# alpapad/java-rsync

Measured on AMD Instinct MI355X. Metric: GiB/s device-resident rolling+MD5 scan (Generator block sums + Sender match scan; bytes read), higher is better.
Workload: dtype u8

## Files before the change

include/rsync_hip_debug.h:

```cpp
#ifndef RSYNC_HIP_DEBUG_H
#define RSYNC_HIP_DEBUG_H

#include <stdint.h>

#include "rsync_hip.h"

#ifdef __cplusplus
extern "C" {
#endif

int rsh_debug_set_option(const char* name, int64_t value);
int rsh_debug_get_option(const char* name, int64_t* value);
void rsh_debug_reset_options(void);

int rsh_debug_kernel_ms(rsh_ctx* ctx, int32_t which, double* ms);

int rsh_debug_generation(rsh_ctx* ctx, int32_t set, int32_t* gen);

int rsh_debug_streams_busy(rsh_ctx* ctx, int32_t* mask);

int rsh_debug_k1_clock(rsh_ctx* ctx, const void* d_data, int64_t n, int32_t block_length, int32_t reps,
                       double* clock_ghz);

int rsh_debug_multi_selftest(const int64_t* bytes, int32_t njobs, int32_t nparts, int32_t fail_part, int32_t* part_out,
                             int32_t* order_out, int32_t* status_out);

int rsh_debug_tokens_selftest(const uint8_t* src, int64_t n, const rsh_event* ev, int64_t n_ev,
                              const uint8_t file_md5[16], int64_t from, uint8_t* out, int64_t len, int64_t span,
                              int64_t* n_desc);

int rsh_debug_sums_selftest(int32_t unframe, const rsh_header* h, int32_t* weak, uint8_t* strong, uint8_t* wire,
                            int64_t len, int64_t span, int64_t* n_desc);

typedef struct {
    int64_t pos;
    int32_t kind;
    int32_t value;
    int64_t count;
} rsh_token_run;
int rsh_debug_tokens_scan_selftest(rsh_ctx* ctx, const uint8_t* tokens, int64_t tokens_len, int64_t from,
                                   rsh_token_run* runs, int64_t cap, int64_t* n_runs, int64_t* pos, int32_t* status);

int rsh_debug_untokens_selftest(rsh_ctx* ctx, const uint8_t* tokens, int64_t tokens_len, int64_t pos, int32_t T,
                                int64_t count, uint8_t* out, int64_t span, int64_t* n_desc, int64_t* lo, int64_t* hi);

#ifdef __cplusplus
}
#endif
#endif
```

java-rsync_amd/csrc/batch.cpp:

```cpp
#include "batch.h"

namespace rsh {

void destroy_batch_state(BatchState* b) { delete b; }
hipError_t clear_batch_abort_words(BatchState* b) {
    if (!b) return hipSuccess;
    hipError_t e = b->file_abort ? hipMemset(b->file_abort, 0, (size_t)b->file_abort_cap * 4) : hipSuccess;
    if (e == hipSuccess && b->chain_map.p) e = hipMemset(b->chain_map.p, 0, b->chain_map.cap);
    return e;
}

namespace batch {
namespace {

#define RSH_HTRY(call) do { const hipError_t e_ = (call); if (e_ != hipSuccess) return e_; } while (0)
#define RSH_STEP(call) do { const int rc_ = (call); if (rc_ != RSH_OK) return rc_; } while (0)

struct K1Set {
    std::vector<K1Plan> plans;
    std::vector<K1Lane> lanes;
    int lane_align = 16;
    bool partial = tail_gather_on();
    uint32_t ngroups = 0;
    void plan(const std::vector<K1File>& kf) {
        ngroups = plan_block_sums_files(kf.data(), (int32_t)kf.size(), &plans, &lanes, &lane_align, &partial);
    }
};

hipError_t stage_k1(K1Staging& k, std::initializer_list<const K1Set*> sets, hipStream_t st) {
    if (!k.ev) RSH_HTRY(hipEventCreateWithFlags(&k.ev, hipEventDisableTiming));
    if (k.pending) RSH_HTRY(hipEventSynchronize(k.ev));
    k.pending = false;
    size_t np = 0, nl = 0, ng = 0;
    for (const K1Set* s : sets) np += s->plans.size(), nl += s->lanes.size(), ng += s->ngroups;
    RSH_HTRY(k.ensure(np, ng, nl));
    K1Plan* hp = k.h_plans.as<K1Plan>();
    K1Lane* hl = k.h_lanes.as<K1Lane>();
    for (const K1Set* s : sets) {
        hp = std::copy(s->plans.begin(), s->plans.end(), hp);
        hl = std::copy(s->lanes.begin(), s->lanes.end(), hl);
    }
    if (np > 0) RSH_HTRY(hipMemcpyAsync(k.plans.p, k.h_plans.p, np * sizeof(K1Plan), hipMemcpyHostToDevice, st));
    size_t p0 = 0, g0 = 0;
    for (const K1Set* s : sets) {
        RSH_HTRY(launch_expand_groups(k.plans.as<K1Plan>() + p0, (uint32_t)s->plans.size(), s->ngroups,
                                      k.groups.as<K1Group>() + g0, st));
        p0 += s->plans.size(), g0 += s->ngroups;
    }
    if (nl > 0) RSH_HTRY(hipMemcpyAsync(k.lanes.p, k.h_lanes.p, nl * sizeof(K1Lane), hipMemcpyHostToDevice, st));
    RSH_HTRY(hipEventRecord(k.ev, st));
    k.pending = true;
    return hipSuccess;
}

struct SegmentLayout {
    int32_t NF = 0;
    int64_t tw = 0, ts = 0, tna = 0, tas = 0, tnf = 0, tns = 0, thit = 0, tw0 = 0, maxC = 0;
    bool chain_on = false;
    bool two_phase = false;
    bool map_on = false;
    int32_t chain_events = 0;
    K1Set whole, a, b;
    std::vector<int64_t> lead_at;
    int64_t nlead_all = 0;
    size_t lead_ents_at = 0;
    std::vector<int64_t> map_off;
    int64_t map_end(const FileLayout& fs) const { return std::min<int64_t>(fs.na_a * fs.B, fs.n - fs.B + 1); }
    hipError_t plan(BatchState* S, const std::vector<FileLayout*>& file, hipStream_t st);
};

hipError_t SegmentLayout::plan(BatchState* S, const std::vector<FileLayout*>& file, hipStream_t st) {
    NF = (int32_t)file.size();
    for (FileLayout* p : file) {
        FileLayout& fs = *p;
        fs.na = (fs.n + fs.B - 1) / fs.B;
        fs.nf = std::min<int64_t>(fs.na, fs.C);
        fs.ns = pow2_at_least(2 * (uint64_t)fs.C + 2);
        fs.off_tw = tw, tw += fs.C;
        fs.off_ts = ts, ts += (int64_t)fs.C * fs.dl;
        fs.off_na = tna, tna += fs.na;
        fs.off_as = tas, tas += fs.na * fs.dl;
        fs.off_nf = tnf, tnf += fs.nf;
        fs.off_ns = tns, tns += fs.ns;
        fs.off_hit = thit, thit += pad16(16 + fs.B);
        fs.off_w0 = tw0, tw0 += pad16(std::min<int64_t>(fs.B, fs.n));
        maxC = std::max<int64_t>(maxC, fs.C);
    }
    const size_t nf = (size_t)NF;
    RSH_HTRY(S->h_weak.ensure((size_t)tw * 4 + 4));
    RSH_HTRY(S->h_strong.ensure((size_t)ts + 1));
    RSH_HTRY(S->slots.ensure((size_t)tns * 8));
    RSH_HTRY(S->src_weak.ensure((size_t)tna * 4));
    RSH_HTRY(S->src_strong.ensure((size_t)tas + 1));
    RSH_HTRY(S->flags.ensure((size_t)tnf + 1));
    RSH_HTRY(S->haw.ensure((size_t)tna * 4));
    RSH_HTRY(S->h_aw.ensure((size_t)tna * 4));
    RSH_HTRY(S->h_as.ensure((size_t)tas + 1));
    RSH_HTRY(S->h_fl.ensure((size_t)tnf + 1));
    RSH_HTRY(S->h_files.ensure(nf * sizeof(ScanFile)));
    RSH_HTRY(S->h_hit.ensure((size_t)thit));
    RSH_HTRY(S->h_win0.ensure((size_t)tw0));
    RSH_HTRY(S->first.ensure(nf * sizeof(ProbeOut)));
    RSH_HTRY(S->h_first.ensure(nf * sizeof(ProbeOut)));
    RSH_HTRY(S->bucket.ensure(nf * HIT_BUCKET_INTS * 4));
    RSH_HTRY(S->h_bucket.ensure(nf * HIT_BUCKET_INTS * 4));
    RSH_HTRY(S->h_copies.ensure(2 * nf * sizeof(CopyEnt)));
    RSH_HTRY(S->h_ccopies.ensure(nf * sizeof(CopyEnt) + 3 * nf * sizeof(CopyEnt)));
    RSH_HTRY(S->h_tabents.ensure(nf * sizeof(TableEnt)));
    RSH_HTRY(S->h_flagents.ensure(nf * sizeof(FlagEnt)));
    RSH_HTRY(S->h_flagents_a.ensure(nf * sizeof(FlagEnt)));
    lead_at.assign(nf + 1, 0);
    for (size_t f = 0; f < nf; ++f) lead_at[f + 1] = lead_at[f] + std::min<int64_t>(kLeadWindows, file[f]->nf);
    nlead_all = lead_at[nf];
    lead_ents_at = ((size_t)(nlead_all + 1) * 4 + 63) & ~(size_t)63;
    RSH_HTRY(S->h_lead.ensure(lead_ents_at + (size_t)(nlead_all + 1) * sizeof(GatherEnt)));
    auto k1_file = [&](const FileLayout& fs, int64_t w0, int64_t w1) {
        return K1File{fs.d_src + w0 * fs.B, std::min<int64_t>(fs.n, w1 * fs.B) - w0 * fs.B, (uint32_t)fs.B, (uint32_t)fs.dl,
                      (uint32_t)(w1 - w0), S->src_weak.as<int32_t>() + fs.off_na + w0,
                      S->src_strong.as<uint8_t>() + fs.off_as + w0 * fs.dl};
    };
    std::vector<K1File> k1;
    for (const FileLayout* fs : file) k1.push_back(k1_file(*fs, 0, fs->na));
    whole.plan(k1);
    RSH_HTRY(S->ensure_file_abort(NF));
    for (K1Plan& pl : whole.plans) pl.abort = S->file_abort + pl.file;
    chain_on = opt(OPT_BATCH_CHAIN) != 0;
    chain_events = (int32_t)std::clamp<int64_t>(
        kChainEventBytes / ((int64_t)std::max<int32_t>(NF, 1) * (int64_t)sizeof(rsh_event)), 256, kChainEventsMax);
    for (FileLayout* fs : file) fs->na_a = fs->na;
    if (const int64_t pre = opt(OPT_BATCH_CHAIN_PREFIX); chain_on && pre != 0) {
        const int64_t P = pre > 0 ? pre : 16 * std::max<int64_t>(1, kWaveSlots / std::max<int32_t>(NF, 1));
        for (FileLayout* fs : file) {
            fs->na_a = std::min(fs->na, P);
            two_phase = two_phase || fs->na_a < fs->na;
        }
    }
    if (two_phase) {
        std::vector<K1File> ka, kb;
        std::vector<int32_t> b_file;
        for (int32_t f = 0; f < NF; ++f) {
            const FileLayout& fs = *file[(size_t)f];
            ka.push_back(k1_file(fs, 0, fs.na_a));
            if (fs.na_a == fs.na) continue;
            kb.push_back(k1_file(fs, fs.na_a, fs.na));
            b_file.push_back(f);
        }
        a.plan(ka);
        b.plan(kb);
        for (K1Plan& pl : a.plans) pl.abort = nullptr;
        for (K1Plan& pl : b.plans) pl.abort = S->file_abort + b_file[(size_t)pl.file];
        for (const K1Lane& ln : b.lanes) {
            const int64_t lo = (int64_t)ln.c_first * ln.B, hi = std::min<int64_t>(ln.n, lo + (int64_t)ln.nchunks * ln.B);
            file[(size_t)b_file[(size_t)ln.file]]->lane_b_bytes += std::max<int64_t>(0, hi - lo);
        }
    }
    RSH_HTRY(S->spec_k1.ensure(std::max(whole.plans.size(), a.plans.size() + b.plans.size()),
                               std::max(whole.ngroups, a.ngroups + b.ngroups),
                               std::max(whole.lanes.size(), a.lanes.size() + b.lanes.size())));
    if (!chain_on) return hipSuccess;
    RSH_HTRY(S->kslots.ensure(kslots_bytes(tns, tw)));
    RSH_HTRY(S->h_kents.ensure(nf * sizeof(ChunkIndexEnt)));
    RSH_HTRY(S->h_chain.ensure(nf * sizeof(ChainFile)));
    RSH_HTRY(S->h_chain_out.ensure(nf * sizeof(ChainOut)));
    RSH_HTRY(S->h_chain_ev.ensure(nf * (size_t)chain_events * sizeof(rsh_event)));
    RSH_HTRY(S->h_early.ensure(4096));
    map_off.assign(nf + 1, 0);
    map_on = two_phase && opt(OPT_CHAIN_HELPERS) != 0;
    for (size_t f = 0; map_on && f < nf; ++f) {
        const FileLayout& fs = *file[f];
        const bool wide = fs.B >= 512 && fs.B % 32 == 0 && CHAIN_TILE / fs.B + 2 <= CHAIN_SEGS;
        const int64_t hend = map_end(fs);
        map_off[f + 1] = map_off[f] + (wide && fs.C > 0 && hend > 0 ? (hend + 31) / 32 : 0);
    }
    map_on = map_on && map_off[nf] > 0 && map_off[nf] * 8 <= opt(OPT_CHAIN_MAP_BYTES);
    if (map_on) {
        if ((size_t)map_off[nf] * 8 > S->chain_map.cap) {
            RSH_HTRY(S->chain_map.ensure((size_t)map_off[nf] * 8));
            RSH_HTRY(hipMemsetAsync(S->chain_map.p, 0, S->chain_map.cap, st));
        }
        RSH_HTRY(S->chain_help.ensure(nf * sizeof(ChainHelp)));
        RSH_HTRY(S->h_chain_help.ensure(nf * sizeof(ChainHelp)));
    }
    return hipSuccess;
}

TableEnt table_ent(const DevBuf& slots, const FileScan& fs) {
    return TableEnt{slots.as<unsigned long long>() + fs.off_ns, fs.d_weak, fs.ns - 1, fs.C};
}
FlagEnt flag_ent(BatchState* S, const FileScan& fs, uint32_t nflag) {
    return FlagEnt{S->src_weak.as<int32_t>() + fs.off_na, S->src_strong.as<uint8_t>() + fs.off_as, fs.d_weak, fs.d_strong,
                   S->flags.as<uint8_t>() + fs.off_nf, nflag, (uint32_t)fs.dl};
}
CopyEnt* table_copies(BatchState* S, const FileScan& fs, CopyEnt* out) {
    if (fs.C == 0) return out;
    *out++ = CopyEnt{reinterpret_cast<const uint8_t*>(fs.d_weak), S->h_weak.as<uint8_t>() + 4 * fs.off_tw, (int64_t)fs.C * 4};
    if (fs.dl > 0) *out++ = CopyEnt{fs.d_strong, S->h_strong.as<uint8_t>() + fs.off_ts, (int64_t)fs.C * fs.dl};
    return out;
}
CopyEnt* spec_copies(BatchState* S, const FileScan& fs, int64_t nal, bool flags, bool sums, CopyEnt* out) {
    const int64_t nfl = std::min(fs.nf, nal);
    if (flags && nfl > 0) *out++ = CopyEnt{S->flags.as<uint8_t>() + fs.off_nf, S->h_fl.as<uint8_t>() + fs.off_nf, nfl};
    if (!sums) return out;
    *out++ = CopyEnt{S->src_weak.as<uint8_t>() + 4 * fs.off_na, S->h_aw.as<uint8_t>() + 4 * fs.off_na, nal * 4};
    if (fs.dl > 0)
        *out++ = CopyEnt{S->src_strong.as<uint8_t>() + fs.off_as, S->h_as.as<uint8_t>() + fs.off_as, nal * fs.dl};
    return out;
}

struct Scan {
    rsh_ctx* const c;
    BatchState* const S;
    rsh_scan_job* const jobs;
    const uint8_t* const seed;
    const std::chrono::steady_clock::time_point t0 = std::chrono::steady_clock::now();
    const bool trace = opt(OPT_SCAN_TRACE) != 0;
    const hipStream_t st, aux;
    std::vector<FileScan> files;
    SegmentLayout L;
    std::shared_ptr<Batch> bp = std::make_shared<Batch>();
    Batch& b = *bp;
    RoundCtl ctl;
    int gen = 0;
    bool tentative = false;
    bool k1_launched = false, spec_launched = false;
    bool skip_rest = false;
    std::vector<char> early;
    hipError_t early_err = hipSuccess;
    uint32_t n_help = 0;
    int spec_rc = RSH_OK;
    int32_t nwait = 0, left = 0;
    int rounds = 0;
    double enq_ms = 0, setup_ms = 0, resolve_ms = 0;

    Scan(rsh_ctx* c_, BatchState* S_, rsh_scan_job* jobs_, const uint8_t* seed_)
        : c(c_), S(S_), jobs(jobs_), seed(seed_), st(c_->stream), aux(c_->aux) {}
    int32_t NF() const { return L.NF; }
    ChainOut* chain_out() const { return S->h_chain_out.as<ChainOut>(); }
    rsh_event* chain_ev(int32_t f) const { return S->h_chain_ev.as<rsh_event>() + (int64_t)f * L.chain_events; }

    int lay_out(const std::vector<int32_t>& which);
    void prepare_files();
    int enqueue_prep();
    int begin_speculation();
    int launch_spec_k1();
    int launch_spec();
    int enqueue_walks();
    void prepare_walks();
    int walk_phase0();
    int walk_rest();
    hipError_t await_walks();
    hipError_t early_resolve(int32_t f);
    void take_walk(int32_t f, bool prefix_only);
    int await_setup();
    int take_walks();
    int hand_over();
    void report_walks();
    int lead_check();
    hipError_t run_rounds();
    int cancel_unlanded();
    void return_events();
    void add_stats(rsh_scan_stats* agg);
};

int Scan::lay_out(const std::vector<int32_t>& which) {
    files.resize(which.size());
    std::vector<FileLayout*> lay;
    for (size_t f = 0; f < which.size(); ++f) {
        FileScan& fs = files[f];
        const rsh_scan_job& j = jobs[which[f]];
        fs.job = which[f];
        fs.d_src = static_cast<const uint8_t*>(j.d_src);
        fs.d_weak = static_cast<const int32_t*>(j.d_weak);
        fs.d_strong = static_cast<const uint8_t*>(j.d_strong);
        fs.n = j.n;
        fs.B = j.h.block_length;
        fs.C = j.h.chunk_count;
        fs.dl = j.h.digest_length;
        lay.push_back(&fs);
    }
    RSH_BHIP(L.plan(S, lay, st));
    early.assign(files.size(), 0);
    return RSH_OK;
}

void Scan::prepare_files() {
    ScanFile* F = S->h_files.as<ScanFile>();
    b.files = &files;
    for (int32_t f = 0; f < NF(); ++f) {
        FileScan& fs = files[(size_t)f];
        const rsh_scan_job& j = jobs[fs.job];
        fs.table.chunk_count = fs.C;
        fs.table.block_length = (int32_t)fs.B;
        fs.table.remainder = j.h.remainder;
        fs.table.digest_length = fs.dl;
        fs.table.weak = S->h_weak.as<int32_t>() + fs.off_tw;
        fs.table.strong = S->h_strong.as<uint8_t>() + fs.off_ts;
        BatchBackend& be = fs.be;
        be.b = &b;
        be.f = f;
        be.na = fs.na;
        be.aw = S->h_aw.as<int32_t>() + fs.off_na;
        be.as = S->h_as.as<uint8_t>() + fs.off_as;
        be.fl = S->h_fl.as<uint8_t>() + fs.off_nf;
        be.win0 = S->h_win0.as<uint8_t>() + fs.off_w0;
        be.w0 = std::min<int64_t>(fs.B, fs.n);
        be.hit = S->h_hit.as<uint8_t>() + fs.off_hit;
        be.bucket = S->h_bucket.as<int32_t>() + (int64_t)f * HIT_BUCKET_INTS;
        be.n = fs.n;
        be.B = fs.B;
        memcpy(be.seed, seed, 4);
        be.table = &fs.table;
        be.haw_ready.assign((size_t)fs.na, 0);
        F[f] = ScanFile{};
        F[f].data = fs.d_src;
        F[f].n = fs.n;
        F[f].B = (uint32_t)fs.B;
        F[f].out = S->first.as<ProbeOut>() + f;
        F[f].table_weak = fs.d_weak;
        F[f].C = fs.C;
        F[f].bucket = S->bucket.as<int32_t>() + (int64_t)f * HIT_BUCKET_INTS;
        F[f].hit = S->h_hit.as<uint8_t>() + fs.off_hit;
        F[f].nwin = 1;
        F[f].aligned_weak = S->haw.as<int32_t>() + fs.off_na;
    }
}

int Scan::enqueue_prep() {
    ScanFile* F = S->h_files.as<ScanFile>();
    RSH_BHIP(hipEventRecord(c->ev_in, st));
    CopyEnt* wc = S->h_ccopies.as<CopyEnt>();
    int64_t max_w0 = 0;
    for (int32_t f = 0; f < NF(); ++f) {
        FileScan& fs = files[(size_t)f];
        const int64_t w0 = std::min<int64_t>(fs.B, fs.n);
        wc[f] = CopyEnt{fs.d_src, S->h_win0.as<uint8_t>() + fs.off_w0, w0};
        max_w0 = std::max(max_w0, w0);
    }
    RSH_BHIP(launch_copy_many(wc, (uint32_t)NF(), max_w0, st));
    if (L.nlead_all > 0 && !L.chain_on) {
        auto* ents = reinterpret_cast<GatherEnt*>(S->h_lead.as<uint8_t>() + L.lead_ents_at);
        for (int32_t f = 0; f < NF(); ++f)
            for (int64_t k = 0; k < L.lead_at[(size_t)f + 1] - L.lead_at[(size_t)f]; ++k)
                ents[L.lead_at[(size_t)f] + k] = GatherEnt{k * files[(size_t)f].B, f, 0};
        RSH_BHIP(launch_window_weak(F, ents, (uint32_t)L.nlead_all, S->h_lead.as<int32_t>(), st));
    }
    RSH_BHIP(hipEventRecord(c->ev_prep, st));
    constexpr bool bg = true;
    if (!L.chain_on) {
        CopyEnt* tc = S->h_copies.as<CopyEnt>();
        CopyEnt* tc_end = tc;
        for (const FileScan& fs : files) tc_end = table_copies(S, fs, tc_end);
        RSH_BHIP(launch_copy_many(tc, (uint32_t)(tc_end - tc), L.maxC * 4, st, bg));
    }
    RSH_BHIP(hipEventRecord(c->ev_tab, st));
    if (!L.chain_on) {
        TableEnt* te = S->h_tabents.as<TableEnt>();
        RSH_BHIP(launch_table_clear(S->slots.as<unsigned long long>(), (uint64_t)L.tns, st, bg));
        for (int32_t f = 0; f < NF(); ++f) te[f] = table_ent(S->slots, files[(size_t)f]);
        RSH_BHIP(launch_table_insert_many(te, (uint32_t)NF(), (int32_t)L.maxC, st, bg));
        return RSH_OK;
    }
    if (!S->ev_fk) RSH_BHIP(hipEventCreateWithFlags(&S->ev_fk, hipEventDisableTiming));
    RSH_BHIP(hipMemsetAsync(S->kslots.p, 0, (size_t)L.tns * 8 + (size_t)L.tw, st));
    ChunkIndexEnt* ke = S->h_kents.as<ChunkIndexEnt>();
    for (int32_t f = 0; f < NF(); ++f) {
        const FileScan& fs = files[(size_t)f];
        ke[f] = ChunkIndexEnt{table_ent(S->kslots, fs), kslots_dup(S, L.tns) + fs.off_tw};
    }
    RSH_BHIP(launch_chunk_index(ke, (uint32_t)NF(), (int32_t)L.maxC, st, bg));
    return RSH_OK;
}

int Scan::begin_speculation() {
    gen = c->next_gen();
    tentative = L.nlead_all > 0 && !L.chain_on;
    return tentative ? launch_spec_k1() : RSH_OK;
}

int Scan::launch_spec_k1() {
    k1_launched = true;
    K1Set& k = L.whole;
    size_t kept = 0;
    k.ngroups = 0;
    for (const K1Plan& pl : k.plans)
        if (!files[(size_t)pl.file].done) {
            k.plans[kept] = pl;
            k.plans[kept++].g0 = k.ngroups;
            k.ngroups += pl.ng;
        }
    k.plans.resize(kept);
    kept = 0;
    for (const K1Lane& ln : k.lanes)
        if (!files[(size_t)ln.file].done) k.lanes[kept++] = ln;
    k.lanes.resize(kept);
    int32_t dropped = 0;
    for (FileScan& fs : files)
        if (fs.done) fs.cancelled = true, ++dropped;
    if (trace)
        fprintf(stderr, "[rsh-batch] speculation launched: %u groups, %d resolved files dropped\n", k.ngroups, dropped);
    RSH_BHIP(stage_k1(S->spec_k1, {&k}, aux));
    RSH_BHIP(hipStreamWaitEvent(aux, L.chain_on ? c->ev_in : c->ev_prep, 0));
    RSH_BHIP(launch_block_sums_batch(S->spec_k1.groups.as<K1Group>(), k.ngroups, S->spec_k1.lanes.as<K1Lane>(),
                                     (uint32_t)k.lanes.size(), k.lane_align, seed_word(seed), aux, c->abort_word, gen,
                                     k.partial));
    return RSH_OK;
}

int Scan::launch_spec() {
    if (!k1_launched) RSH_STEP(launch_spec_k1());
    RSH_BHIP(hipStreamWaitEvent(aux, c->ev_in, 0));
    FlagEnt* fe = S->h_flagents.as<FlagEnt>();
    CopyEnt* const fc = S->h_ccopies.as<CopyEnt>() + NF();
    CopyEnt *fc_end = fc, *const sc = fc + NF(), *sc_end = sc;
    uint32_t max_nf = 0;
    int64_t max_len = 0, max_fl = 0;
    for (int32_t f = 0; f < NF(); ++f) {
        const FileScan& fs = files[(size_t)f];
        const uint32_t nflag = fs.cancelled ? 0u : (uint32_t)fs.nf;
        fe[f] = flag_ent(S, fs, nflag);
        max_nf = std::max<uint32_t>(max_nf, nflag);
        if (fs.cancelled) continue;
        fc_end = spec_copies(S, fs, fs.na, true, false, fc_end);
        sc_end = spec_copies(S, fs, fs.na, false, true, sc_end);
        max_fl = std::max<int64_t>(max_fl, fs.nf);
        max_len = std::max<int64_t>(max_len, fs.na * 4);
    }
    RSH_BHIP(launch_chain_flags_many(fe, (uint32_t)NF(), max_nf, aux));
    if (L.chain_on) RSH_BHIP(hipEventRecord(S->ev_fk, aux));
    if (!L.chain_on) RSH_BHIP(launch_copy_many(fc, (uint32_t)(fc_end - fc), max_fl, aux));
    RSH_BHIP(hipEventRecord(c->ev_flags, aux));
    if (!L.chain_on) RSH_BHIP(launch_copy_many(sc, (uint32_t)(sc_end - sc), max_len, aux));
    RSH_BHIP(hipEventRecord(c->ev_spec, aux));
    return RSH_OK;
}

void Scan::take_walk(int32_t f, bool prefix_only) {
    FileScan& fs = files[(size_t)f];
    const ChainOut& o = chain_out()[f];
    if (o.status == CHAIN_DONE) {
        fs.dev_ev = chain_ev(f);
        fs.dev_n = o.n_ev;
    } else {
        fs.res.ev.assign(chain_ev(f), chain_ev(f) + o.n_ev);
    }
    fs.res.literal = o.literal;
    fs.res.matched = o.matched;
    fs.res.stats.chain_matches += o.chain_matches;
    fs.res.stats.events += o.events;
    fs.res.stats.flushes += o.flushes;
    fs.rs.s = o.s;
    fs.rs.m = o.m;
    fs.rs.pref = o.pref;
    fs.rs.anchor = o.s;
    fs.rs.elo = o.elo;
    fs.rs.ehi = o.ehi;
    fs.rs.clear_from = o.clear_to >= 0 ? o.s : -1;
    fs.rs.clear_to = o.clear_to;
    fs.be.na = (o.aborted || prefix_only) ? fs.na_a : fs.na;
    if (o.md5c_valid) {
        fs.rs.md5c.assign(o.md5c, o.md5c + fs.dl);
        fs.rs.md5c_valid = true;
        fs.rs.dkeys_ready = false;
    }
    if (o.status == CHAIN_DONE) fs.rs.done = fs.done = true;
}

hipError_t Scan::early_resolve(int32_t f) {
    FileScan& fs = files[(size_t)f];
    take_walk(f, true);
    if (fs.done) return hipSuccess;
    const auto te0 = std::chrono::steady_clock::now();
    hipStream_t es = c->phase;
    CopyEnt* ec = S->h_early.as<CopyEnt>();
    TableEnt* et = reinterpret_cast<TableEnt*>(ec + 8);
    const int64_t nal = fs.na_a;
    CopyEnt* ec_end = spec_copies(S, fs, nal, true, true, table_copies(S, fs, ec));
    et[0] = table_ent(S->slots, fs);
    RSH_HTRY(hipStreamWaitEvent(es, S->ev_fa, 0));
    RSH_HTRY(launch_copy_many(ec, (uint32_t)(ec_end - ec), std::max<int64_t>((int64_t)fs.C * 4, nal * 4), es));
    RSH_HTRY(launch_table_clear(S->slots.as<unsigned long long>() + fs.off_ns, fs.ns, es));
    RSH_HTRY(launch_table_insert_many(et, 1, fs.C, es));
    RSH_HTRY(spin_sync(S, es));
    fs.be.head = false;
    b.landed.store(true);
    b.aligned.store(true);
    b.direct = [this, f, es](FileScan&) {
        const hipError_t x = serve_round(c, S, files, std::vector<int32_t>{f}, es);
        if (x != hipSuccess && early_err == hipSuccess) early_err = x;
    };
    resolve_run(fs.n, fs.table, fs.be, &fs.rs, &fs.res, nullptr);
    b.direct = nullptr;
    fs.rs.done = fs.done = true;
    early[(size_t)f] = 1;
    if (trace)
        fprintf(stderr, "[rsh-batch] file %d resolved while the walks ran: %.3f ms, done at %.3f ms\n", f, ms_since(te0),
                ms_since(t0));
    return early_err;
}

hipError_t Scan::await_walks() {
    const ChainOut* co = chain_out();
    std::vector<char> seen((size_t)NF(), 0);
    for (;;) {
        const hipError_t q = hipEventQuery(S->ev_wa);
        if (q != hipErrorNotReady) return q;
        for (int32_t f = 0; f < NF(); ++f) {
            if (seen[(size_t)f] || *reinterpret_cast<const volatile int32_t*>(&co[f].fin) == 0) continue;
            seen[(size_t)f] = 1;
            std::atomic_thread_fence(std::memory_order_acquire);
            if (co[f].status == CHAIN_STOP && co[f].why == CHAIN_WHY_FLUSHED) RSH_HTRY(early_resolve(f));
        }
        _mm_pause();
    }
}

void Scan::prepare_walks() {
    ChainFile* cf = S->h_chain.as<ChainFile>();
    ChainOut* co = chain_out();
    ChainHelp* chh = L.map_on ? S->h_chain_help.as<ChainHelp>() : nullptr;
    for (int32_t f = 0; f < NF(); ++f) {
        const FileScan& fs = files[(size_t)f];
        co[f] = ChainOut{};
        co[f].clear_to = -1;
        const int64_t mw = L.map_on ? L.map_off[(size_t)f + 1] - L.map_off[(size_t)f] : 0;
        const int64_t hend = mw > 0 ? L.map_end(fs) : 0;
        cf[f] = ChainFile{fs.d_src, fs.n, (uint32_t)fs.B, fs.C, fs.dl, jobs[fs.job].h.remainder,
                          fs.ns - 1, S->kslots.as<unsigned long long>() + fs.off_ns, fs.d_weak, fs.d_strong,
                          S->src_weak.as<int32_t>() + fs.off_na, S->src_strong.as<uint8_t>() + fs.off_as,
                          S->flags.as<uint8_t>() + fs.off_nf, fs.na, fs.na_a,
                          L.two_phase ? S->file_abort + f : nullptr, chain_ev(f), L.chain_events,
                          seed_word(seed), co + f,
                          mw > 0 ? S->chain_map.as<unsigned long long>() + L.map_off[(size_t)f] : nullptr, hend,
                          kslots_dup(S, L.tns) + fs.off_tw};
        if (chh) chh[f] = ChainHelp{(int32_t)((hend + CHAIN_MAP_SEG - 1) / CHAIN_MAP_SEG), 0, 1, 0, 0, 0, 0, 0, INT64_MAX, 0, 0, 0,
                                    kChainHelpTiles};
    }
    const int64_t helpers_opt = opt(OPT_CHAIN_HELPERS);
    n_help = !L.map_on ? 0u
             : helpers_opt > 0 ? (uint32_t)helpers_opt
                               : (uint32_t)std::max<int64_t>(0, (int64_t)c->n_cu - NF());
}

int Scan::enqueue_walks() {
    if (!L.chain_on) return RSH_OK;
    prepare_walks();
    if (trace) {
        for (hipEvent_t* e : {&S->ev_ch0, &S->ev_ch1})
            if (!*e) RSH_BHIP(hipEventCreate(e));
    }
    if (L.two_phase) RSH_STEP(walk_phase0());
    RSH_STEP(walk_rest());
    if (trace) RSH_BHIP(hipEventRecord(S->ev_ch1, st));
    return RSH_OK;
}

int Scan::walk_phase0() {
    const ChainFile* cf = S->h_chain.as<ChainFile>();
    const K1Staging& k = S->spec_k1;
    if (!S->ev_fa) RSH_BHIP(hipEventCreateWithFlags(&S->ev_fa, hipEventDisableTiming));
    if (!S->ev_wa) RSH_BHIP(hipEventCreate(&S->ev_wa));
    RSH_BHIP(stage_k1(S->spec_k1, {&L.a, &L.b}, aux));
    RSH_BHIP(hipStreamWaitEvent(aux, c->ev_in, 0));
    RSH_BHIP(launch_block_sums_batch(k.groups.as<K1Group>(), L.a.ngroups, k.lanes.as<K1Lane>(), (uint32_t)L.a.lanes.size(),
                                     L.a.lane_align, seed_word(seed), aux, c->abort_word, gen, L.a.partial));
    RSH_BHIP(hipStreamWaitEvent(aux, c->ev_in, 0));
    FlagEnt* fa = S->h_flagents_a.as<FlagEnt>();
    uint32_t max_na = 0;
    for (int32_t f = 0; f < NF(); ++f) {
        const FileScan& fs = files[(size_t)f];
        const uint32_t nflag = (uint32_t)std::min(fs.na_a, fs.nf);
        fa[f] = flag_ent(S, fs, nflag);
        max_na = std::max(max_na, nflag);
    }
    RSH_BHIP(launch_chain_flags_many(fa, (uint32_t)NF(), max_na, aux));
    RSH_BHIP(hipEventRecord(S->ev_fa, aux));
    if (L.map_on)
        RSH_BHIP(hipMemcpyAsync(S->chain_help.p, S->h_chain_help.p, (size_t)NF() * sizeof(ChainHelp), hipMemcpyHostToDevice, st));
    RSH_BHIP(hipStreamWaitEvent(st, S->ev_fa, 0));
    const int gen_b = c->next_gen();
    if (trace) RSH_BHIP(hipEventRecord(S->ev_ch0, st));
    RSH_BHIP(launch_chain_advance(cf, (uint32_t)NF(), st, 0, gen_b, L.map_on ? S->chain_help.as<ChainHelp>() : nullptr,
                                  n_help, trace));
    RSH_BHIP(hipEventRecord(S->ev_wa, st));
    RSH_BHIP(await_walks());
    const ChainOut* co = chain_out();
    skip_rest = true;
    for (int32_t f = 0; f < NF() && skip_rest; ++f)
        skip_rest = co[f].status == CHAIN_DONE || co[f].aborted || (co[f].status == CHAIN_STOP && co[f].md5c_valid);
    if (!skip_rest) {
        RSH_BHIP(hipStreamWaitEvent(aux, S->ev_wa, 0));
        RSH_BHIP(launch_block_sums_batch(k.groups.as<K1Group>() + L.a.ngroups, L.b.ngroups,
                                         k.lanes.as<K1Lane>() + L.a.lanes.size(), (uint32_t)L.b.lanes.size(), L.b.lane_align,
                                         seed_word(seed), aux, c->abort_word, gen_b, L.b.partial));
        k1_launched = true;
    }
    if (trace)
        fprintf(stderr, "[rsh-batch] two-phase speculation: prefix %u groups, rest %u groups%s\n", L.a.ngroups, L.b.ngroups,
                skip_rest ? " (skipped: no walk reached the prefix's end)" : "");
    return RSH_OK;
}

int Scan::walk_rest() {
    if (!skip_rest) {
        RSH_STEP(launch_spec());
        spec_launched = true;
        RSH_BHIP(hipStreamWaitEvent(st, S->ev_fk, 0));
        if (trace && !L.two_phase) RSH_BHIP(hipEventRecord(S->ev_ch0, st));
        RSH_BHIP(launch_chain_advance(S->h_chain.as<ChainFile>(), (uint32_t)NF(), st, L.two_phase ? 1 : 0, 0, nullptr, 0, trace));
    } else {
        RSH_BHIP(hipEventRecord(c->ev_flags, st));
        RSH_BHIP(hipEventRecord(c->ev_spec, st));
        RSH_BHIP(hipEventRecord(S->ev_fk, st));
        spec_launched = true;
    }
    return RSH_OK;
}

int Scan::await_setup() {
    enq_ms = ms_since(t0);
    RSH_BHIP(hipEventSynchronize(c->ev_tab));
    RSH_BHIP(spin_sync(S, st));
    setup_ms = ms_since(t0);
    return RSH_OK;
}

int Scan::take_walks() {
    if (!L.chain_on) return RSH_OK;
    for (int32_t f = 0; f < NF(); ++f) {
        if (early[(size_t)f]) continue;
        take_walk(f, skip_rest);
        if (!files[(size_t)f].done) ++left;
    }
    b.landed.store(true);
    if (left > 0) RSH_STEP(hand_over());
    if (trace) report_walks();
    return RSH_OK;
}

int Scan::hand_over() {
    CopyEnt* tc = S->h_copies.as<CopyEnt>();
    CopyEnt* tc_end = tc;
    TableEnt* te = S->h_tabents.as<TableEnt>();
    uint32_t ntl = 0;
    int64_t mt = 0;
    for (const FileScan& fs : files) {
        if (fs.done || fs.C == 0) continue;
        tc_end = table_copies(S, fs, tc_end);
        mt = std::max<int64_t>(mt, (int64_t)fs.C * 4);
        te[ntl++] = table_ent(S->slots, fs);
    }
    RSH_BHIP(launch_copy_many(tc, (uint32_t)(tc_end - tc), mt, st));
    RSH_BHIP(launch_table_clear(S->slots.as<unsigned long long>(), (uint64_t)L.tns, st));
    RSH_BHIP(launch_table_insert_many(te, ntl, (int32_t)L.maxC, st));
    CopyEnt* lc = S->h_ccopies.as<CopyEnt>() + NF();
    CopyEnt* lc_end = lc;
    int64_t mx = 0;
    for (const FileScan& fs : files) {
        if (fs.done) continue;
        lc_end = spec_copies(S, fs, fs.be.na, true, true, lc_end);
        mx = std::max(mx, fs.be.na * 4);
    }
    RSH_BHIP(hipStreamWaitEvent(st, c->ev_spec, 0));
    RSH_BHIP(launch_copy_many(lc, (uint32_t)(lc_end - lc), mx, st));
    RSH_BHIP(spin_sync(S, st));
    b.aligned.store(true);
    for (FileScan& fs : files) fs.be.head = false;
    return RSH_OK;
}

void Scan::report_walks() {
    const ChainOut* co = chain_out();
    float kms = 0.f, wams = 0.f;
    if (S->ev_ch0 && S->ev_ch1) (void)hipEventElapsedTime(&kms, S->ev_ch0, S->ev_ch1);
    if (L.two_phase && S->ev_ch0 && S->ev_wa) (void)hipEventElapsedTime(&wams, S->ev_ch0, S->ev_wa);
    int64_t tsum = 0, esum = 0, dsum = 0, psum = 0, asum = 0, msum = 0;
    int32_t tmax = 0, emax = 0, fmax = 0;
    for (int32_t f = 0; f < NF(); ++f) {
        tsum += co[f].tiles;
        msum += co[f].mapped;
        if (co[f].tiles > tmax) tmax = co[f].tiles, fmax = f;
        esum += co[f].events;
        dsum += co[f].digests;
        psum += co[f].md5c_valid;
        asum += co[f].aborted;
        emax = std::max<int32_t>(emax, (int32_t)co[f].events);
    }
    fprintf(stderr, "[rsh-batch] chain walks done at %.3f ms (walks %.3f ms, phase 0 %.3f ms; tiles %lld (%lld from the hit "
            "map), max %d per file; events %lld, max %d; %lld windows digested, %lld files poisoned, %lld speculations "
            "stopped at the prefix): %d of %d files left to the resolvers\n", ms_since(t0), kms, wams, (long long)tsum,
            (long long)msum, tmax, (long long)esum, emax,
            (long long)dsum, (long long)psum, (long long)asum, left, NF());
    const ChainOut& x = co[fmax];
    for (int32_t f = 0; f < NF(); ++f)
        if (co[f].status != CHAIN_DONE)
            fprintf(stderr, "[rsh-batch]   file %d: left at s %lld (why %d, events %lld, tiles %d, poisoned %d, searched to "
                    "%lld, phase 1 %d, walk %.1f us)\n", f, (long long)co[f].s, co[f].why, (long long)co[f].events,
                    co[f].tiles, co[f].md5c_valid, (long long)co[f].clear_to, co[f].spec_full, co[f].t_total / 100.0);
    fprintf(stderr, "[rsh-batch]   file %d: walk %.1f us = tiles %.1f (table checks %.1f; %d of %d tiles from the hit map,"
            " the first at tile %d) + events %.1f (buckets %.1f; %d digests: %.1f) + key set %.1f + steps (1)/(1') %.1f +"
            " event drains %.1f + other\n", fmax, x.t_total / 100.0,
            x.t_tiles / 100.0, x.t_check / 100.0, x.mapped, x.tiles, x.first_mapped, x.t_event / 100.0,
            x.t_evb / 100.0, x.digests, x.t_digest / 100.0, x.t_kset / 100.0, x.t_chain / 100.0, x.t_drain / 100.0);
    if (!S->chain_help.p || !L.two_phase) return;
    std::vector<ChainHelp> hh((size_t)NF());
    if (hipMemcpy(hh.data(), S->chain_help.p, (size_t)NF() * sizeof(ChainHelp), hipMemcpyDeviceToHost) != hipSuccess) return;
    int64_t segs = 0, joins = 0, files_helped = 0;
    for (const ChainHelp& q : hh) {
        segs += q.mapped;
        joins += q.joins;
        files_helped += q.joins > 0;
    }
    const ChainHelp& q = hh[(size_t)fmax];
    fprintf(stderr, "[rsh-batch]   hit map: %lld segments mapped over %lld files (%lld key sets built); file %d: %d "
            "segments (%d whole), %d key sets (%.1f us each), claims %d of %d, first whole segment %.1f us after "
            "the walk's start\n", (long long)segs, (long long)files_helped, (long long)joins, fmax, q.mapped,
            q.whole, q.joins, q.joins ? q.t_kset / 100.0 / q.joins : 0.0, q.claim, q.nseg,
            q.t_first == INT64_MAX ? -1.0 : (q.t_first - q.t_start) / 100.0);
}

int Scan::lead_check() {
    if (!tentative) return RSH_OK;
    const int32_t* lead_w = S->h_lead.as<int32_t>();
    for (int32_t f = 0; f < NF(); ++f) {
        FileScan& fs = files[(size_t)f];
        const int64_t a = L.lead_at[(size_t)f], nl = L.lead_at[(size_t)f + 1] - a;
        int64_t lead = 0;
        while (lead < nl && lead_w[a + lead] == fs.table.weak[lead]) ++lead;
        fs.wait_spec = nl > 0 && lead == nl && (nl >= kLeadWindows || nl == fs.nf);
        nwait += fs.wait_spec;
    }
    if (nwait > 0) {
        spec_rc = launch_spec();
        if (spec_rc != RSH_OK) return spec_rc;
        spec_launched = true;
    } else {
        RSH_BHIP(hipMemsetD32Async(reinterpret_cast<hipDeviceptr_t>(S->file_abort), gen, (size_t)NF(), st));
        RSH_BHIP(hipStreamWaitEvent(st, S->spec_k1.ev, 0));
        gen = c->next_gen();
        k1_launched = false;
    }
    if (trace) fprintf(stderr, "[rsh-batch] lead check: %d of %d files wait for the speculation\n", nwait, NF());
    return RSH_OK;
}

hipError_t Scan::run_rounds() {
    ctl.launch_spec = [this] { return launch_spec(); };
    ctl.spec_launched = &spec_launched;
    ctl.spec_rc = &spec_rc;
    ctl.k1_launched = k1_launched;
    ctl.gen = gen;
    ctl.trace = trace;
    ctl.t0 = t0;
    const hipError_t err = run_resolvers(c, S, bp, files, st, ctl, &rounds);
    const double rounds_end_ms = ms_since(t0);
    resolve_ms = ms_since(t0) - setup_ms;
    if (trace) {
        HostTimes tt;
        for (const HostTimes& x : b.times) {
            tt.bucket_ms += x.bucket_ms;
            tt.sort_ms += x.sort_ms;
            tt.dkeys_ms += x.dkeys_ms;
            tt.md5_ms += x.md5_ms;
        }
        fprintf(stderr, "[rsh-batch] host totals (cumulative per thread): bucket %.3f sort %.3f dkeys %.3f md5 %.3f ms\n",
                tt.bucket_ms, tt.sort_ms, tt.dkeys_ms, tt.md5_ms);
        fprintf(stderr, "[rsh-batch] %d files: enqueued %.3f, tables+hashes ready %.3f, rounds done %.3f, joined %.3f ms\n",
                NF(), enq_ms, setup_ms, rounds_end_ms, ms_since(t0));
    }
    return err;
}

int Scan::cancel_unlanded() {
    if (!spec_launched) return RSH_OK;
    if (!b.landed.load() && hipEventQuery(c->ev_flags) == hipSuccess) b.landed.store(true);
    if (b.landed.load()) return RSH_OK;
    for (int32_t f = 0; f < NF(); ++f) {
        FileScan& fs = files[(size_t)f];
        if (fs.cancelled) continue;
        fs.cancelled = true;
        RSH_BHIP(hipStreamWriteValue32(st, S->file_abort + f, (uint32_t)gen, 0));
    }
    if (trace) fprintf(stderr, "[rsh-batch] scan done before the speculation landed: stopped\n");
    RSH_BHIP(hipStreamWriteValue32(st, c->abort_word, (uint32_t)gen, 0));
    RSH_BHIP(hipStreamWaitEvent(st, c->ev_spec, 0));
    return RSH_OK;
}

void Scan::return_events() {
    std::vector<int32_t> copy_files;
    int64_t copy_bytes = 0;
    for (int32_t f = 0; f < NF(); ++f) {
        FileScan& fs = files[(size_t)f];
        rsh_scan_job& j = jobs[fs.job];
        j.literal = fs.res.literal;
        j.matched = fs.res.matched;
        j.n_ev = fs.dev_ev ? fs.dev_n : (int64_t)fs.res.ev.size();
        if (j.n_ev > j.ev_cap || (!j.ev && j.n_ev > 0)) {
            j.status = RSH_E_NOSPACE;
        } else {
            if (j.n_ev > 0) {
                copy_files.push_back(f);
                copy_bytes += j.n_ev * (int64_t)sizeof(rsh_event);
            }
            j.status = RSH_OK;
        }
    }
    auto copy_range = [&](size_t i0, size_t i1) {
        for (size_t i = i0; i < i1; ++i) {
            FileScan& fs = files[(size_t)copy_files[i]];
            rsh_scan_job& j = jobs[fs.job];
            memcpy(j.ev, fs.dev_ev ? fs.dev_ev : fs.res.ev.data(), (size_t)j.n_ev * sizeof(rsh_event));
        }
    };
    const int nct = copy_bytes > (1 << 20) ? std::min<int>(8, std::max(1, call_cores())) : 1;
    if (nct > 1 && copy_files.size() > 1) {
        const size_t per = (copy_files.size() + (size_t)nct - 1) / (size_t)nct;
        const int parts = (int)((copy_files.size() + per - 1) / per);
        S->pool.ensure(parts - 1);
        const std::function<void(int)> part = [&](int k) {
            copy_range((size_t)k * per, std::min(copy_files.size(), (size_t)(k + 1) * per));
        };
        S->pool.run(parts, part);
    } else {
        copy_range(0, copy_files.size());
    }
}

void Scan::add_stats(rsh_scan_stats* agg) {
    for (const FileScan& fs : files) {
        const rsh_scan_stats& s = fs.res.stats;
        agg->chain_matches += s.chain_matches;
        agg->events += s.events;
        agg->host_md5_windows += s.host_md5_windows;
        agg->flushes += s.flushes;
        agg->table_ms += s.table_ms + fs.table.sort_ms;
        int64_t spec_bytes = (spec_launched && b.landed.load() && !fs.cancelled) ? fs.n : 0;
        if (spec_bytes > 0 && fs.be.na < fs.na)
            spec_bytes = std::min<int64_t>(fs.n, fs.be.na * fs.B) + (skip_rest ? 0 : fs.lane_b_bytes);
        agg->device_bytes += fs.be.bytes_read + spec_bytes;
        agg->phase_matches += s.phase_matches;
    }
    agg->probe_launches += rounds;
    agg->device_ms += setup_ms;
    agg->resolver_ms += resolve_ms;
    agg->speculation_aborted = spec_launched ? (b.landed.load() ? 0 : 1) : 2;
}

int scan_batch(rsh_ctx* c, rsh_scan_job* jobs, const std::vector<int32_t>& which, const uint8_t seed[4],
               rsh_scan_stats* agg) {
    BatchState* S = state_of(c);
    if (!S) return RSH_E_NOMEM;
    Scan s(c, S, jobs, seed);
    RSH_STEP(s.lay_out(which));
    s.prepare_files();
    RSH_STEP(s.enqueue_prep());
    RSH_STEP(s.begin_speculation());
    RSH_STEP(s.enqueue_walks());
    RSH_STEP(s.await_setup());
    RSH_STEP(s.take_walks());
    RSH_STEP(s.lead_check());
    const hipError_t err = s.run_rounds();
    RSH_STEP(s.cancel_unlanded());
    if (s.spec_rc != RSH_OK) return s.spec_rc;
    if (err != hipSuccess) return RSH_E_DEVICE;
    s.return_events();
    if (agg) s.add_stats(agg);
    return RSH_OK;
}

}
}
}

using namespace rsh;

namespace rsh {
using namespace batch;

hipError_t batch_warm(rsh_ctx* c, int32_t nfiles, int64_t n, int64_t B, int32_t dl) {
    if (nfiles <= 0) return hipSuccess;
    BatchState* S = state_of(c);
    if (!S) return hipErrorOutOfMemory;
    FileLayout shape;
    shape.d_src = reinterpret_cast<const uint8_t*>(uintptr_t{4096});
    shape.n = n, shape.B = B, shape.C = (int32_t)((n + B - 1) / B), shape.dl = dl;
    std::vector<FileLayout> shapes((size_t)std::min<int32_t>(nfiles, kMaxLive), shape);
    std::vector<FileLayout*> lay;
    for (FileLayout& sh : shapes) lay.push_back(&sh);
    SegmentLayout L;
    RSH_HTRY(L.plan(S, lay, c->stream));
    hipError_t e = hipSuccess;
    auto ok = [&](hipError_t x) {
        if (e == hipSuccess) e = x;
    };
    S->pool.ensure(7);
    for (PinnedBuf* pb : {&S->h_fjobs, &S->h_fout, &S->h_rcp, &S->h_req, &S->h_gw, &S->h_gb, &S->h_ow, &S->h_ob, &S->h_win,
                          &S->h_dkeys})
        ok(pb->ensure(64 << 10));
    for (PinnedBuf* pb : {&S->h_fgw, &S->h_iv, &S->h_tiles, &S->h_segs, &S->h_ptiles}) ok(pb->ensure(512 << 10));
    for (DevBuf* db : {&S->fc_dev, &S->partials, &S->dslots, &S->d_probe}) ok(db->ensure(64 << 10));
    for (hipEvent_t* ev : {&S->ev_fk, &S->ev_fa, &S->spec_k1.ev, &S->ev_sync, &S->gen_k1.ev})
        if (!*ev) ok(hipEventCreateWithFlags(ev, hipEventDisableTiming));
    if (!S->ev_wa) ok(hipEventCreate(&S->ev_wa));
    ok(S->gen_k1.ensure(L.whole.plans.size(), L.whole.ngroups, L.whole.lanes.size()));
    return e;
}

int block_sums_batch_claimed(rsh_ctx* ctx, const rsh_block_job* jobs, int32_t njobs, const uint8_t seed[4]) {
    if (!ctx || !seed || njobs < 0 || (njobs > 0 && !jobs)) return RSH_E_INVAL;
    std::vector<K1File> files;
    for (int32_t i = 0; i < njobs; ++i) {
        const rsh_block_job& j = jobs[i];
        const int rc = check_generator_header(j.n, &j.h);
        if (rc != RSH_OK) return rc;
        if (j.h.chunk_count == 0) continue;
        if (!j.d_data || !j.d_weak || (!j.d_strong && j.h.digest_length > 0)) return RSH_E_INVAL;
        files.push_back(K1File{static_cast<const uint8_t*>(j.d_data), j.n, (uint32_t)j.h.block_length,
                               (uint32_t)j.h.digest_length, (uint32_t)j.h.chunk_count, static_cast<int32_t*>(j.d_weak),
                               static_cast<uint8_t*>(j.d_strong)});
    }
    if (files.empty()) return RSH_OK;
    BatchState* S = state_of(ctx);
    if (!S) return RSH_E_NOMEM;
    RSH_BHIP(hipSetDevice(ctx->device));
    K1Set k;
    k.plan(files);
    RSH_BHIP(stage_k1(S->gen_k1, {&k}, ctx->stream));
    RSH_BHIP(launch_block_sums_batch(S->gen_k1.groups.as<K1Group>(), k.ngroups, S->gen_k1.lanes.as<K1Lane>(),
                                     (uint32_t)k.lanes.size(), k.lane_align, seed_word(seed), ctx->stream, nullptr, 0,
                                     k.partial));
    return RSH_OK;
}

int match_scan_batch_claimed(rsh_ctx* ctx, rsh_scan_job* jobs, int32_t njobs, const uint8_t seed[4],
                             rsh_scan_stats* stats) {
    if (!ctx || !seed || njobs < 0 || (njobs > 0 && !jobs)) return RSH_E_INVAL;
    if (stats) *stats = rsh_scan_stats{};
    std::vector<int32_t> scan;
    for (int32_t i = 0; i < njobs; ++i) {
        rsh_scan_job& j = jobs[i];
        j.n_ev = j.literal = j.matched = 0;
        j.status = RSH_OK;
        if (j.n < 0) {
            j.status = RSH_E_INVAL;
            continue;
        }
        const int v = rsh_header_validate(&j.h);
        if (v != RSH_OK) {
            j.status = v;
            continue;
        }
        if (j.h.block_length == 0 || j.n == 0) {
            ResolveResult r;
            if (j.h.block_length == 0) skip_events(j.n, &r);
            j.literal = r.literal;
            j.n_ev = (int64_t)r.ev.size();
            if (j.n_ev > j.ev_cap || (!j.ev && j.n_ev > 0)) j.status = RSH_E_NOSPACE;
            else if (j.n_ev > 0) memcpy(j.ev, r.ev.data(), r.ev.size() * sizeof(rsh_event));
            continue;
        }
        if (!j.d_src || (j.h.chunk_count > 0 && (!j.d_weak || (!j.d_strong && j.h.digest_length > 0)))) {
            j.status = RSH_E_INVAL;
            continue;
        }
        if ((j.n + j.h.block_length - 1) / j.h.block_length > 2147483647LL) {
            j.status = RSH_E_OVERFLOW;
            continue;
        }
        scan.push_back(i);
    }
    if (!scan.empty()) {
        auto fail_from = [&](size_t k, int rc) {
            for (size_t q = k; q < scan.size(); ++q) jobs[scan[q]].status = rc;
            return rc;
        };
        if (hipSetDevice(ctx->device) != hipSuccess) return fail_from(0, RSH_E_DEVICE);
        for (size_t k = 0; k < scan.size(); k += kMaxLive) {
            const std::vector<int32_t> part(scan.begin() + (ptrdiff_t)k,
                                            scan.begin() + (ptrdiff_t)std::min(scan.size(), k + kMaxLive));
            const int rc = scan_batch(ctx, jobs, part, seed, stats);
            if (rc != RSH_OK) return fail_from(k, rc);
        }
    }
    for (int32_t i = 0; i < njobs; ++i)
        if (jobs[i].status != RSH_OK) return jobs[i].status;
    return RSH_OK;
}

}

extern "C" {

int rsh_block_sums_batch_device(rsh_ctx* ctx, const rsh_block_job* jobs, int32_t njobs, const uint8_t seed[4]) {
    if (!ctx) return RSH_E_INVAL;
    RSH_CLAIM(ctx);
    return rsh::block_sums_batch_claimed(ctx, jobs, njobs, seed);
}

int rsh_match_scan_batch_device(rsh_ctx* ctx, rsh_scan_job* jobs, int32_t njobs, const uint8_t seed[4],
                                rsh_scan_stats* stats) {
    if (!ctx) return RSH_E_INVAL;
    RSH_CLAIM(ctx);
    return rsh::match_scan_batch_claimed(ctx, jobs, njobs, seed, stats);
}

}
```

java-rsync_amd/csrc/batch.h:

```cpp
#pragma once
#include <sched.h>
#include <ucontext.h>

#include <condition_variable>
#include <functional>
#include <memory>
#include <mutex>
#include <thread>

#include <immintrin.h>

#include "ctx.h"
#include "host_md5.h"
#include "options.h"
#include "resolver.h"

namespace rsh {

struct HostPool {
    std::mutex mu;
    std::condition_variable cv_work, cv_done;
    std::vector<std::thread> th;
    const std::function<void(int)>* job = nullptr;
    int njobs = 0, next = 0, done = 0;
    uint64_t gen = 0;
    bool quit = false;
    void ensure(int n) {
        while ((int)th.size() < n) th.emplace_back([this] { work(); });
    }
    void work() {
        uint64_t seen = 0;
        std::unique_lock<std::mutex> l(mu);
        for (;;) {
            cv_work.wait(l, [&] { return quit || gen != seen; });
            if (quit) return;
            seen = gen;
            while (next < njobs) {
                const int i = next++;
                l.unlock();
                (*job)(i);
                l.lock();
                if (++done == njobs) cv_done.notify_one();
            }
        }
    }
    void run(int n, const std::function<void(int)>& f) {
        if (n <= 0) return;
        std::unique_lock<std::mutex> l(mu);
        job = &f;
        njobs = n, next = 0, done = 0;
        ++gen;
        cv_work.notify_all();
        while (next < njobs) {
            const int i = next++;
            l.unlock();
            f(i);
            l.lock();
            ++done;
        }
        cv_done.wait(l, [&] { return done == njobs; });
        job = nullptr;
    }
    ~HostPool() {
        {
            std::lock_guard<std::mutex> l(mu);
            quit = true;
        }
        cv_work.notify_all();
        for (std::thread& t : th) t.join();
    }
};

struct K1Staging {
    DevBuf plans, groups, lanes;
    PinnedBuf h_plans, h_lanes;
    hipEvent_t ev = nullptr;
    bool pending = false;
    hipError_t ensure(size_t nplans, size_t ngroups, size_t nlanes) {
        hipError_t e = hipSuccess;
        if (pending && ((nplans + 1) * sizeof(K1Plan) > h_plans.cap || (nlanes + 1) * sizeof(K1Lane) > h_lanes.cap)) {
            e = hipEventSynchronize(ev);
            pending = false;
        }
        if (e == hipSuccess) e = groups.ensure((ngroups + 1) * sizeof(K1Group));
        if (e == hipSuccess) e = plans.ensure((nplans + 1) * sizeof(K1Plan));
        if (e == hipSuccess) e = lanes.ensure((nlanes + 1) * sizeof(K1Lane));
        if (e == hipSuccess) e = h_plans.ensure((nplans + 1) * sizeof(K1Plan));
        if (e == hipSuccess) e = h_lanes.ensure((nlanes + 1) * sizeof(K1Lane));
        return e;
    }
    ~K1Staging() {
        if (ev) {
            if (pending) (void)hipEventSynchronize(ev);
            (void)hipEventDestroy(ev);
        }
        for (DevBuf* b : {&plans, &groups, &lanes}) b->release();
        for (PinnedBuf* b : {&h_plans, &h_lanes}) b->release();
    }
};

struct BatchState {
    HostPool pool;
    K1Staging gen_k1, spec_k1;
    DevBuf slots, dslots, src_weak, src_strong, flags, haw, partials, bucket, first;
    DevBuf d_probe;
    DevBuf fc_dev;
    PinnedBuf h_fgw, h_fjobs, h_fout;
    PinnedBuf h_early;
    PinnedBuf h_rcp;
    PinnedBuf h_weak, h_strong, h_aw, h_as, h_fl, h_files, h_hit, h_win0, h_bucket, h_first, h_iv, h_tiles, h_segs,
        h_ptiles, h_req, h_gw, h_gb, h_ow, h_ob, h_win, h_copies, h_tabents, h_flagents, h_flagents_a, h_dkeys, h_ccopies,
        h_lead;
    int* file_abort = nullptr;
    int64_t file_abort_cap = 0;
    DevBuf kslots;
    PinnedBuf h_kents, h_chain, h_chain_out, h_chain_ev;
    DevBuf chain_help, chain_map;
    PinnedBuf h_chain_help;
    std::vector<std::unique_ptr<char[]>> fiber_stacks;
    hipEvent_t ev_fk = nullptr;
    hipEvent_t ev_sync = nullptr;
    hipEvent_t ev_ch0 = nullptr, ev_ch1 = nullptr;
    hipEvent_t ev_fa = nullptr, ev_wa = nullptr;
    hipError_t ensure_file_abort(int64_t nf) {
        if (nf <= file_abort_cap) return hipSuccess;
        if (file_abort) (void)hipFree(file_abort);
        file_abort = nullptr;
        file_abort_cap = 0;
        const int64_t cap = std::max<int64_t>(nf, 256);
        hipError_t e = hipExtMallocWithFlags(reinterpret_cast<void**>(&file_abort), (size_t)cap * 4,
                                             hipDeviceMallocUncached);
        if (e == hipSuccess) e = hipMemset(file_abort, 0, (size_t)cap * 4);
        if (e == hipSuccess) file_abort_cap = cap;
        return e;
    }
    ~BatchState() {
        if (file_abort) (void)hipFree(file_abort);
        for (hipEvent_t e : {ev_fk, ev_ch0, ev_ch1, ev_fa, ev_wa, ev_sync})
            if (e) (void)hipEventDestroy(e);
        kslots.release();
        for (PinnedBuf* b : {&h_kents, &h_chain, &h_chain_out, &h_chain_ev, &h_chain_help}) b->release();
        chain_help.release();
        chain_map.release();
        for (DevBuf* b : {&d_probe, &fc_dev, &slots, &dslots, &src_weak, &src_strong, &flags, &haw, &partials, &bucket, &first})
            b->release();
        for (PinnedBuf* b : {&h_weak, &h_strong, &h_aw, &h_as, &h_fl, &h_files, &h_hit, &h_win0, &h_bucket, &h_first,
                             &h_iv, &h_tiles, &h_segs, &h_ptiles, &h_req, &h_gw, &h_gb, &h_ow, &h_ob, &h_win, &h_copies,
                             &h_tabents, &h_flagents, &h_flagents_a, &h_dkeys, &h_ccopies, &h_lead, &h_fgw, &h_fjobs,
                             &h_fout, &h_early, &h_rcp})
            b->release();
    }
};
inline size_t kslots_bytes(int64_t tns, int64_t tw) { return (size_t)tns * 8 + (size_t)tw + 8; }
inline uint8_t* kslots_dup(BatchState* S, int64_t tns) {
    return reinterpret_cast<uint8_t*>(S->kslots.as<unsigned long long>() + tns);
}

namespace batch {

constexpr int32_t kMaxLive = 256;
constexpr int kDeferRounds = 2;
constexpr int32_t kChainHelpTiles = 1;
constexpr int kSpinUs = 200;
constexpr int32_t kMaxWorkers = 32;
constexpr size_t kFiberStack = 512 * 1024;
constexpr int32_t kEagerSortChunks = 1 << 16;
constexpr int64_t kPad = 16;
constexpr int64_t kWaveSlots = 2 * 4 * 256;
constexpr size_t kProbeUpload = 2048;
constexpr int32_t kChainEventsMax = 4096;
constexpr int64_t kChainEventBytes = 64ll << 20;

inline int64_t pad16(int64_t v) { return (v + kPad - 1) / kPad * kPad; }

inline BatchState* state_of(rsh_ctx* c) {
    if (!c->batch) c->batch = new (std::nothrow) BatchState();
    return c->batch;
}

template <class T>
hipError_t pin(PinnedBuf& b, int64_t count, T** out) {
    const hipError_t e = b.ensure((size_t)std::max<int64_t>(count, 1) * sizeof(T));
    *out = b.as<T>();
    return e;
}

#define RSH_BHIP(call)                                  \
    do {                                                \
        hipError_t e_ = (call);                         \
        if (e_ != hipSuccess) {                         \
            note_error(e_, __LINE__, __FILE__);         \
            return RSH_E_DEVICE;                        \
        }                                               \
    } while (0)

struct Req {
    enum Kind { WEAK, BYTES, WIN, PROBE, WAIT, FLUSH, FCHAIN } kind = WEAK;
    const int64_t* pos = nullptr;
    int64_t count = 0;
    const int64_t* pos2 = nullptr;
    int64_t count2 = 0;
    uint8_t* out_b2 = nullptr;
    int32_t* out_w = nullptr;
    uint8_t* out_b = nullptr;
    int64_t p = 0, w = 0;
    const uint8_t* win = nullptr;
    const ProbeInterval* iv = nullptr;
    int64_t niv = 0;
    const std::vector<int32_t>* keys = nullptr;
    bool head = false;
    int64_t result = -1;
    const ProbeOut* out = nullptr;
    FlushChain fchain;
    int64_t npre = 0;
    uint32_t* chain_out = nullptr;
};

struct Batch;

class BatchBackend : public ScanBackend {
  public:
    Batch* b = nullptr;
    int32_t f = 0;
    bool head = true;
    int64_t na = 0;
    const int32_t* aw = nullptr;
    const uint8_t* as = nullptr;
    const uint8_t* fl = nullptr;
    const uint8_t* win0 = nullptr;
    int64_t w0 = 0;
    const uint8_t* hit = nullptr;
    const int32_t* bucket = nullptr;
    int64_t n = 0, B = 0;
    uint8_t seed[4];
    ChunkTable* table = nullptr;
    std::vector<uint8_t> haw_ready;
    int64_t win_pos[HIT_WINDOWS] = {-1, -1, -1, -1};
    int64_t t_pos = -1;
    int32_t t_val = 0;
    HitCache cache;

    int64_t aligned_count() override;
    int64_t flags_count() override { return head ? 0 : na; }
    int64_t max_batch() override { return head ? 4 : 4096; }
    const int32_t* aligned_weak() override { return aw; }
    const uint8_t* aligned_strong() override { return as; }
    const uint8_t* chain_flags() override { return fl; }
    void weak_many(const int64_t* pos, int64_t count, int32_t* out) override;
    void bytes_many(const int64_t* pos, int64_t count, uint8_t* out) override;
    void flush_gather(const int64_t* tpos, int64_t nt, int32_t* tv, const int64_t* bpos, int64_t nb,
                      uint8_t* bv) override;
    void md5_at(int64_t p, uint8_t out[16]) override;
    int64_t first_hit(const ProbeInterval* iv, int64_t count, const std::vector<int32_t>* keys) override;
    int64_t flush_probe(const ProbeInterval* pre, int64_t npre, const FlushChain& q, std::vector<FlushStep>* steps,
                        std::vector<ProbeInterval>* ivs, const std::vector<int32_t>* keys) override;
  private:
    int64_t probe_answer(const ProbeInterval* iv, int64_t count, const std::vector<int32_t>* keys);
};

struct FileLayout {
    const uint8_t* d_src = nullptr;
    int64_t n = 0, B = 0, na = 0, nf = 0;
    int64_t na_a = 0;
    int64_t lane_b_bytes = 0;
    int32_t C = 0, dl = 0;
    uint32_t ns = 0;
    int64_t off_tw = 0, off_ts = 0, off_na = 0, off_as = 0, off_nf = 0, off_ns = 0, off_hit = 0, off_w0 = 0;
};

struct FileScan : FileLayout {
    int32_t job = 0;
    const int32_t* d_weak = nullptr;
    const uint8_t* d_strong = nullptr;
    const rsh_event* dev_ev = nullptr;
    int64_t dev_n = 0;
    ChunkTable table;
    ResolveState rs;
    ResolveResult res;
    BatchBackend be;
    Req req;
    bool pending = false;
    bool done = false;
    bool started = false;
    bool cancelled = false;
    bool wait_spec = false;
    int32_t worker = 0;
    ucontext_t uc;
    char* stack = nullptr;
};

struct Batch {
    std::mutex mu;
    std::condition_variable cv_coord, cv_work;
    std::atomic<int32_t> idle{0};
    std::atomic<int32_t> nworkers{0};
    std::atomic<uint64_t> gen{0};
    std::atomic<bool> quit{false};
    std::atomic<bool> landed{false};
    std::atomic<bool> aligned{false};
    std::vector<FileScan>* files = nullptr;
    std::vector<ucontext_t> worker_uc;
    std::vector<double> busy_ms, max_fiber_ms;
    std::vector<HostTimes> times;

    std::function<void(FileScan&)> direct;
    void post(FileScan& fs) {
        if (direct) {
            direct(fs);
            return;
        }
        fs.pending = true;
        swapcontext(&fs.uc, &worker_uc[(size_t)fs.worker]);
    }
};
// ... 40 lines not shown
```

java-rsync_amd/csrc/capi.cpp:

```cpp
#include <hip/hip_runtime.h>
#include <immintrin.h>
#include <stdio.h>
#include <stdlib.h>
#include <string.h>

#include <algorithm>
#include <atomic>
#include <chrono>
#include <functional>
#include <thread>
#include <vector>

#include "device.h"
#include "host_md5.h"
#include "resolver.h"
#include "rsync_hip.h"

#include "ctx.h"
#include "options.h"
#include "rsync_hip_debug.h"

namespace {
int warm_calls(rsh_ctx* c) {
    const uint8_t seed[4] = {1, 2, 3, 4};
    constexpr int64_t n5 = 8 << 20, B5 = 131072, n4 = 1 << 20, B4 = 8192;
    const int64_t bytes = 2 * n5 + 4 * n4;
    void* d = nullptr;
    if (hipMalloc(&d, (size_t)bytes + 4096) != hipSuccess) return RSH_E_DEVICE;
    uint8_t* src5 = static_cast<uint8_t*>(d);
    uint8_t* bas5 = src5 + n5;
    uint8_t* src4 = bas5 + n5;
    uint8_t* bas4 = src4 + 2 * n4;
    int rc = RSH_OK;
    auto fill_pair = [&](uint8_t* src, uint8_t* bas, int64_t n, int64_t B, uint64_t key) {
        if (rc == RSH_OK && (rsh_fill_splitmix_device(c, src, n, key, 0) != RSH_OK ||
                             rsh_fill_splitmix_device(c, bas, n, key ^ 0xED17, 0) != RSH_OK ||
                             hipMemcpy2DAsync(bas, (size_t)(2 * B), src, (size_t)(2 * B), (size_t)B, (size_t)(n / (2 * B)),
                                              hipMemcpyDeviceToDevice, c->stream) != hipSuccess))
            rc = RSH_E_DEVICE;
    };
    fill_pair(src5, bas5, n5, B5, 0x5EED5EED00000005ull);
    fill_pair(src4, bas4, 2 * n4, B4, 0x5EED5EED00000004ull);
    rsh_header h5{}, h4{};
    if (rc == RSH_OK) rc = rsh_header_make((int32_t)B5, 4, n5, &h5);
    if (rc == RSH_OK) rc = rsh_header_make((int32_t)B4, 3, n4, &h4);
    const int64_t C5 = h5.chunk_count, C4 = h4.chunk_count;
    void* t = nullptr;
    if (rc == RSH_OK && hipMalloc(&t, (size_t)(C5 * 8 + 2 * C4 * 8) + 256) != hipSuccess) rc = RSH_E_DEVICE;
    int32_t* w5 = static_cast<int32_t*>(t);
    uint8_t* s5 = reinterpret_cast<uint8_t*>(w5 + C5);
    int32_t* w4 = reinterpret_cast<int32_t*>(s5 + C5 * 4);
    uint8_t* s4 = reinterpret_cast<uint8_t*>(w4 + 2 * C4);
    std::vector<rsh_event> ev((size_t)(4 * (C5 + C4) + 64));
    int64_t n_ev = 0, lit = 0, mat = 0;
    if (rc == RSH_OK) rc = rsh_block_sums_device(c, bas5, n5, &h5, seed, w5, s5);
    if (rc == RSH_OK)
        rc = rsh_match_scan_device(c, src5, n5, &h5, w5, s5, seed, ev.data(), (int64_t)ev.size(), &n_ev, &lit, &mat,
                                   nullptr);
    if (rc == RSH_OK) {
        rsh_block_job bj[2];
        rsh_scan_job sj[2];
        for (int f = 0; f < 2; ++f) {
            bj[f] = rsh_block_job{bas4 + f * n4, n4, h4, w4 + f * C4, s4 + f * C4 * 3};
            sj[f] = rsh_scan_job{};
            sj[f].d_src = src4 + f * n4;
            sj[f].n = n4;
            sj[f].h = h4;
            sj[f].d_weak = bj[f].d_weak;
            sj[f].d_strong = bj[f].d_strong;
            sj[f].ev = ev.data() + (size_t)f * (ev.size() / 2);
            sj[f].ev_cap = (int64_t)ev.size() / 2;
        }
        rc = rsh_block_sums_batch_device(c, bj, 2, seed);
        if (rc == RSH_OK) rc = rsh_match_scan_batch_device(c, sj, 2, seed, nullptr);
    }
    if (rsh_ctx_sync(c) != RSH_OK && rc == RSH_OK) rc = RSH_E_DEVICE;
    if (t) (void)hipFree(t);
    (void)hipFree(d);
    return rc;
}
}

int rsh_ctx::next_gen() {
    if (gen >= kGenWrapAt) {
        bool ok = hipDeviceSynchronize() == hipSuccess;
        ok = ok && hipMemset(abort_word, 0, 256) == hipSuccess;
        ok = ok && rsh::clear_batch_abort_words(batch) == hipSuccess;
        if (ok) gen = 0;
    }
    return ++gen;
}

extern "C" {

int rsh_abi_version(void) { return RSH_ABI_VERSION; }

const char* rsh_last_error(void) { return g_last_err; }

const char* rsh_strerror(int status) {
    switch (status) {
        case RSH_OK: return "ok";
        case RSH_E_INVAL: return "invalid argument";
        case RSH_E_PROTOCOL: return "checksum header rejected (RsyncProtocolException)";
        case RSH_E_OVERFLOW: return "chunk count is negative or greater than int max (ChunkOverflow)";
        case RSH_E_NOSPACE: return "event buffer too small";
        case RSH_E_DEVICE: return "HIP device error or no gfx950 device";
        case RSH_E_NOMEM: return "out of memory";
        case RSH_E_BUSY: return "context in use by another thread";
        case RSH_E_NOTFOUND: return "file not found (FileViewNotFound)";
        case RSH_E_OPEN: return "file cannot be opened (FileViewOpenFailed)";
        case RSH_E_NOSOURCE: return "the context holds no source from its last scan";
        default: return "unknown status";
    }
}

int rsh_device_count(int* count) {
    int c = 0;
    if (hipGetDeviceCount(&c) != hipSuccess) c = 0;
    if (count) *count = c;
    return c > 0 ? RSH_OK : RSH_E_DEVICE;
}

int rsh_ctx_create(int device, rsh_ctx** out) {
    if (!out) return RSH_E_INVAL;
    *out = nullptr;
    int count = 0;
    if (hipGetDeviceCount(&count) != hipSuccess || device < 0 || device >= count) return RSH_E_DEVICE;
    hipDeviceProp_t prop;
    if (hipGetDeviceProperties(&prop, device) != hipSuccess) return RSH_E_DEVICE;
    if (strncmp(prop.gcnArchName, "gfx950", 6) != 0) return RSH_E_DEVICE;
    RSH_HIP(hipSetDevice(device));
    rsh_ctx* c = new (std::nothrow) rsh_ctx();
    if (!c) return RSH_E_NOMEM;
    c->device = device;
    c->n_cu = prop.multiProcessorCount > 0 ? prop.multiProcessorCount : 256;
    c->abort_word = nullptr;
    if (hipStreamCreateWithFlags(&c->stream, hipStreamNonBlocking) != hipSuccess ||
        hipStreamCreateWithFlags(&c->aux, hipStreamNonBlocking) != hipSuccess ||
        hipStreamCreateWithFlags(&c->phase, hipStreamNonBlocking) != hipSuccess ||
        hipEventCreateWithFlags(&c->ev_in, hipEventDisableTiming) != hipSuccess ||
        hipEventCreateWithFlags(&c->ev_tab, hipEventDisableTiming) != hipSuccess ||
        hipEventCreateWithFlags(&c->ev_spec, hipEventDisableTiming) != hipSuccess ||
        hipEventCreateWithFlags(&c->ev_phase[0], hipEventDisableTiming) != hipSuccess ||
        hipEventCreateWithFlags(&c->ev_phase[1], hipEventDisableTiming) != hipSuccess ||
        hipEventCreateWithFlags(&c->ev_flags, hipEventDisableTiming) != hipSuccess ||
        hipEventCreateWithFlags(&c->ev_prep, hipEventDisableTiming) != hipSuccess ||
        hipEventCreate(&c->ev_k1a) != hipSuccess || hipEventCreate(&c->ev_k1b) != hipSuccess ||
        hipEventCreate(&c->ev_gen_a) != hipSuccess || hipEventCreate(&c->ev_gen_b) != hipSuccess ||
        hipEventCreateWithFlags(&c->ev_rs_tail, hipEventDisableTiming) != hipSuccess ||
        hipEventCreate(&c->ev_pha[0]) != hipSuccess || hipEventCreate(&c->ev_phb[0]) != hipSuccess ||
        hipEventCreate(&c->ev_pha[1]) != hipSuccess || hipEventCreate(&c->ev_phb[1]) != hipSuccess ||
        hipExtMallocWithFlags(reinterpret_cast<void**>(&c->abort_word), 256, hipDeviceMallocUncached) != hipSuccess ||
        hipMemset(c->abort_word, 0, 256) != hipSuccess ||
        hipEventRecord(c->ev_phase[0], c->stream) != hipSuccess || hipEventRecord(c->ev_phase[1], c->stream) != hipSuccess) {
        delete c;
        return RSH_E_DEVICE;
    }
    if (ctx_warm(c) != hipSuccess || warm_calls(c) != RSH_OK) {
        (void)hipStreamSynchronize(c->stream);
        delete c;
        return RSH_E_DEVICE;
    }
    *out = c;
    return RSH_OK;
}
// ... 259 lines not shown
    return o + 4;
}

int rsh_tokens_write(const uint8_t* src, const rsh_event* ev, int64_t n_ev, const uint8_t file_md5[16], uint8_t* out,
                     int64_t cap) {
    if (!out || !file_md5 || (n_ev > 0 && !ev)) return RSH_E_INVAL;
    if (rsh_tokens_size(ev, n_ev) > cap) return RSH_E_NOSPACE;
    uint8_t* o = out;
    for (int64_t i = 0; i < n_ev; ++i) {
        if (ev[i].kind == RSH_EV_LITERAL) {
            if (!src) return RSH_E_INVAL;
            for (int64_t cur = ev[i].offset, end = ev[i].offset + ev[i].length; cur < end;) {
                const int64_t len = std::min<int64_t>(kChunkSize, end - cur);
                o = put_int(o, (int32_t)len);
                memcpy(o, src + cur, (size_t)len);
                o += len;
                cur += len;
            }
        } else {
            for (int32_t j = 0; j < ev[i].count; ++j) o = put_int(o, -(ev[i].index + j + 1));
        }
    }
    o = put_int(o, 0);
    memcpy(o, file_md5, 16);
    return RSH_OK;
}

int64_t rsh_generator_bytes(const rsh_header* h, const int32_t* weak, const uint8_t* strong, uint8_t* out, int64_t cap) {
    if (!h) return RSH_E_INVAL;
    const int64_t size = 16 + (int64_t)h->chunk_count * (4 + h->digest_length);
    if (!out) return size;
    if (cap < size || (h->chunk_count > 0 && (!weak || (!strong && h->digest_length > 0)))) return RSH_E_NOSPACE;
    uint8_t* o = out;
    o = put_int(o, h->chunk_count);
    o = put_int(o, h->block_length);
    o = put_int(o, h->digest_length);
    o = put_int(o, h->remainder);
    for (int32_t i = 0; i < h->chunk_count; ++i) {
        o = put_int(o, weak[i]);
        memcpy(o, strong + (int64_t)i * h->digest_length, (size_t)h->digest_length);
        o += h->digest_length;
    }
    return size;
}

int rsh_dev_alloc(rsh_ctx* ctx, int64_t bytes, void** out) {
    if (!ctx || !out || bytes < 0) return RSH_E_INVAL;
    RSH_HIP(hipSetDevice(ctx->device));
    return hipMalloc(out, (size_t)(bytes ? bytes : 1)) == hipSuccess ? RSH_OK : RSH_E_NOMEM;
}

int rsh_dev_free(rsh_ctx* ctx, void* p) {
    if (!ctx) return RSH_E_INVAL;
    RSH_HIP(hipSetDevice(ctx->device));
    if (p) RSH_HIP(hipFree(p));
    return RSH_OK;
}

int rsh_memcpy_h2d(rsh_ctx* ctx, void* dst, const void* src, int64_t bytes) {
    if (!ctx || bytes < 0 || (bytes > 0 && (!dst || !src))) return RSH_E_INVAL;
    RSH_HIP(hipSetDevice(ctx->device));
    RSH_HIP(hipMemcpyAsync(dst, src, (size_t)bytes, hipMemcpyHostToDevice, ctx->stream));
    RSH_HIP(hipStreamSynchronize(ctx->stream));
    return RSH_OK;
}

int rsh_memcpy_d2h(rsh_ctx* ctx, void* dst, const void* src, int64_t bytes) {
    if (!ctx || bytes < 0 || (bytes > 0 && (!dst || !src))) return RSH_E_INVAL;
    RSH_HIP(hipSetDevice(ctx->device));
    RSH_HIP(hipMemcpyAsync(dst, src, (size_t)bytes, hipMemcpyDeviceToHost, ctx->stream));
    RSH_HIP(hipStreamSynchronize(ctx->stream));
    return RSH_OK;
}

int rsh_debug_set_option(const char* name, int64_t value) {
    const int i = rsh::opt_index(name);
    if (i < 0) return RSH_E_INVAL;
    rsh::opt_table()[i].store(value, std::memory_order_relaxed);
    return RSH_OK;
}

int rsh_debug_get_option(const char* name, int64_t* value) {
    const int i = rsh::opt_index(name);
    if (i < 0 || !value) return RSH_E_INVAL;
    *value = rsh::opt((rsh::Opt)i);
    return RSH_OK;
}

void rsh_debug_reset_options(void) {
    for (int i = 0; i < rsh::OPT_COUNT; ++i) rsh::opt_table()[i].store(rsh::opt_info()[i].def, std::memory_order_relaxed);
}

int rsh_debug_kernel_ms(rsh_ctx* ctx, int32_t which, double* ms) {
    if (!ctx || !ms || which < 0 || which > 2) return RSH_E_INVAL;
    *ms = -1.0;
    const bool timed = which == 0 ? ctx->gen_timed : which == 1 ? ctx->spec_timed : ctx->sums_timed;
    if (!timed) return RSH_OK;
    const hipEvent_t a = which == 0 ? ctx->ev_gen_a : which == 1 ? ctx->ev_k1a : ctx->ev_sums_a;
    const hipEvent_t b = which == 0 ? ctx->ev_gen_b : which == 1 ? ctx->ev_k1b : ctx->ev_sums_b;
    RSH_HIP(hipSetDevice(ctx->device));
    RSH_HIP(hipEventSynchronize(b));
    float f = 0.f;
    RSH_HIP(hipEventElapsedTime(&f, a, b));
    *ms = f;
    return RSH_OK;
}

int rsh_debug_generation(rsh_ctx* ctx, int32_t set, int32_t* gen) {
    if (!ctx || set < -1 || set > rsh_ctx::kGenWrapAt) return RSH_E_INVAL;
    if (set >= 0) ctx->gen = set;
    if (gen) *gen = ctx->gen;
    return RSH_OK;
}

int rsh_debug_streams_busy(rsh_ctx* ctx, int32_t* mask) {
    if (!ctx || !mask) return RSH_E_INVAL;
    RSH_HIP(hipSetDevice(ctx->device));
    *mask = 0;
    const hipStream_t st[3] = {ctx->stream, ctx->aux, ctx->phase};
    for (int i = 0; i < 3; ++i) {
        const hipError_t e = hipStreamQuery(st[i]);
        if (e == hipErrorNotReady) *mask |= 1 << i;
        else if (e != hipSuccess) RSH_HIP(e);
    }
    return RSH_OK;
}

int rsh_debug_k1_clock(rsh_ctx* ctx, const void* d_data, int64_t n, int32_t block_length, int32_t reps,
                       double* clock_ghz) {
    if (!ctx || !d_data || !clock_ghz || reps <= 0 || block_length <= 0 || n <= 0 || block_length % 128 != 0 ||
        n % (64 * (int64_t)block_length) != 0)
        return RSH_E_INVAL;
    RSH_HIP(hipSetDevice(ctx->device));
    const int64_t C = n / block_length;
    void *w = nullptr, *st = nullptr, *clk = nullptr;
    hipError_t e = hipMalloc(&w, (size_t)C * 4);
    if (e == hipSuccess) e = hipMalloc(&st, (size_t)C * 16);
    if (e == hipSuccess) e = hipMalloc(&clk, 16);
    if (e == hipSuccess) e = hipMemsetAsync(clk, 0, 16, ctx->stream);
    for (int32_t r = 0; e == hipSuccess && r < reps; ++r)
        e = rsh::launch_k1_clock(static_cast<const uint8_t*>(d_data), n, (uint32_t)block_length, 16, 0x04030201u,
                                 static_cast<int32_t*>(w), static_cast<uint8_t*>(st),
                                 static_cast<unsigned long long*>(clk), ctx->stream);
    unsigned long long h[2] = {0, 0};
    if (e == hipSuccess) e = hipMemcpyAsync(h, clk, 16, hipMemcpyDeviceToHost, ctx->stream);
    if (e == hipSuccess) e = hipStreamSynchronize(ctx->stream);
    for (void* p : {w, st, clk})
        if (p) (void)hipFree(p);
    RSH_HIP(e);
    *clock_ghz = h[1] ? 0.1 * (double)h[0] / (double)h[1] : 0.0;
    return RSH_OK;
}

int rsh_fill_splitmix_device(rsh_ctx* ctx, void* d_out, int64_t n, uint64_t key, int64_t byte_offset) {
    if (!ctx || (n > 0 && !d_out) || n < 0 || byte_offset < 0) return RSH_E_INVAL;
    RSH_HIP(hipSetDevice(ctx->device));
    RSH_HIP(rsh::launch_fill_splitmix(static_cast<uint8_t*>(d_out), n, key, byte_offset, ctx->stream));
    return RSH_OK;
}

}
```

java-rsync_amd/csrc/device.h:

```cpp
#pragma once
#include <hip/hip_runtime.h>
#include <stdint.h>

#include <vector>

#include "hit_cache.h"
#include "rsync_hip.h"

namespace rsh {

hipError_t launch_block_sums(const uint8_t* d_data, int64_t n, uint32_t B, uint32_t nchunks, uint32_t dl,
                             uint32_t seed_word, int32_t* d_weak, uint8_t* d_strong, hipStream_t s,
                             const int* abort_flag = nullptr, int abort_gen = 0);
void k1_timing_next(hipEvent_t start, hipEvent_t stop);
bool k1_timing_taken();

#ifdef RSH_KBENCH
hipError_t launch_block_sums_variant(int variant, const uint8_t* d_data, int64_t n, uint32_t B, uint32_t nchunks,
                                     uint32_t dl, uint32_t seed_word, int32_t* d_weak, uint8_t* d_strong,
                                     hipStream_t s, const int* abort_flag = nullptr, int abort_gen = 0);
#endif

struct K1File {
    const uint8_t* data;
// ... 111 lines not shown
    uint32_t B;
    uint32_t mask;
    const unsigned long long* slots;
    int32_t* aligned_weak;
    ProbeOut* out;
    const int32_t* table_weak;
    int32_t C;
    int32_t iv0, niv;
    int32_t nwin;
    int32_t* bucket;
    uint8_t* hit;
    int32_t next_sums;
    int32_t nsmall;
    uint32_t small[PROBE_SMALL_KEYS];
};
struct ProbeIv {
    int64_t a, b, anchor;
    uint32_t e_lo, e_hi;
    int32_t file;
    int32_t pad;
};
struct FlushChainJob {
    const int32_t* tv;
    const uint8_t* bv;
    ProbeIv* iv;
    uint32_t* out;
    int64_t f, B, n, last;
    int32_t K, niv;
    uint32_t el, eh;
};
hipError_t launch_flush_chain(const FlushChainJob* jobs, uint32_t njobs, hipStream_t s);
struct ProbeTile {
    int64_t q0;
    int32_t iv;
    int32_t pbase;
};
struct PartialTile {
    int64_t q0;
    int32_t file;
    int32_t pad;
};
struct ProbeArgs {
    const ScanFile* files;
    const ProbeIv* ivs;
    const ProbeTile* tiles;
    int4* partials;
};
constexpr int PROBE_LONG_PPL = 64;
constexpr int64_t PROBE_LONG_SUB = 256 * PROBE_LONG_PPL;
constexpr int64_t PROBE_LONG_PASSES = 8;
constexpr int64_t PROBE_LONG_MIN = 2 * PROBE_LONG_SUB;
constexpr int64_t PROBE_LONG_BIG = 256 * PROBE_LONG_SUB;
constexpr int64_t PROBE_LONG_MAX_B = 16384;
struct ProbeSeg {
    int64_t q0;
    int32_t iv;
    int32_t len;
};
void probe_tiles(int64_t a, int64_t b, int64_t B, int32_t iv, std::vector<ProbeTile>* out);
int64_t probe_seg_len(int64_t full_positions, int64_t B);
int64_t probe_full_positions(int64_t a, int64_t b, int64_t n, int64_t B);
void probe_plan(int64_t a, int64_t b, int64_t n, int64_t B, int32_t iv, int64_t seg_len, std::vector<ProbeTile>* tiles,
                std::vector<ProbeSeg>* segs);
hipError_t launch_probe_long(const ProbeArgs& args, const ProbeSeg* segs, uint32_t nsegs, hipStream_t s);
void probe_partials(std::vector<ProbeTile>* tiles, size_t t0, int64_t B, int32_t file, std::vector<PartialTile>* out);
hipError_t launch_probe_first(const ProbeArgs& args, uint32_t ntiles, const PartialTile* ptiles, uint32_t nptiles,
                              hipStream_t s);
hipError_t launch_hit_window(const ScanFile* files, const ProbeIv* ivs, const int32_t* req, int32_t nreq, int32_t max_C,
                             hipStream_t s);

hipError_t launch_probe_out_reset(ProbeOut* d_out, uint32_t n, hipStream_t s);

struct GatherEnt {
    int64_t p;
    int32_t file;
    int32_t by_block;
};
hipError_t launch_gather_bytes(const ScanFile* files, const GatherEnt* ents, uint32_t n, uint8_t* out, hipStream_t s);
hipError_t launch_window_weak(const ScanFile* files, const GatherEnt* ents, uint32_t n, int32_t* out, hipStream_t s);
struct CopyEnt {
    const uint8_t* src;
    uint8_t* dst;
    int64_t len;
};
hipError_t launch_copy_many(const CopyEnt* ents, uint32_t n, int64_t max_len, hipStream_t s, bool bg = false);
struct CopyFew {
    CopyEnt e[4];
    uint32_t n;
};
hipError_t launch_copy_few(const CopyFew& f, hipStream_t s);
hipError_t launch_copy_few_stamped(const CopyFew& f, int* stamp, int gen, hipStream_t s);
hipError_t launch_copy_to_host(const uint8_t* d_src, int64_t n, uint8_t* h_dst, hipStream_t s);
struct GatherOp {
    const uint8_t* src;
    uint8_t* dst;
    int64_t len;
};
hipError_t launch_gather_ops(const GatherOp* ops, uint32_t n, hipStream_t s, int64_t avg_len = 1 << 20);
#ifdef RSH_KBENCH
hipError_t launch_gather_ops_variant(int v, const GatherOp* ops, uint32_t n, hipStream_t s);
#endif
struct TokSpan;
hipError_t launch_token_frame(const TokSpan* spans, uint32_t n, uint32_t max_len, bool dst_on_host, hipStream_t s);
struct TokRun;
struct TokScanOut;
struct UntokSpan;
hipError_t launch_token_scan(const uint8_t* tokens, int64_t len, int64_t from, TokRun* runs, int64_t cap, TokScanOut* out,
                             hipStream_t s);
hipError_t launch_token_unframe(const UntokSpan* spans, uint32_t n, uint32_t max_len, hipStream_t s);
hipError_t launch_warm_tokens(hipStream_t s);
struct SumsSpan;
hipError_t launch_sums_frame(const SumsSpan* spans, uint32_t n, uint32_t max_len, hipStream_t s);
hipError_t launch_sums_unframe(const SumsSpan* spans, uint32_t n, uint32_t max_len, hipStream_t s);
hipError_t launch_warm_sums(hipStream_t s);
struct TableEnt {
    unsigned long long* slots;
    const int32_t* keys;
    uint32_t mask;
    int32_t nkeys;
};
hipError_t launch_table_insert_many(const TableEnt* ents, uint32_t n, int32_t max_keys, hipStream_t s,
                                    bool bg = false);
struct FlagEnt {
    const int32_t* wsrc;
    const uint8_t* ssrc;
    const int32_t* wbas;
    const uint8_t* sbas;
    uint8_t* flags;
    uint32_t count, dl;
};
hipError_t launch_chain_flags_many(const FlagEnt* ents, uint32_t n, uint32_t max_count, hipStream_t s);
inline uint32_t slot_hash_host(uint32_t key) {
    const uint32_t h = key * 0x9E3779B1u;
    return h ^ (h >> 15);
}

enum { CHAIN_STOP = 0, CHAIN_DONE = 1, CHAIN_MORE = 2 };
constexpr int CHAIN_BUCKET_CAP = 64;
struct ChainOut {
    int64_t s, m;
    int32_t pref, status;
    int32_t n_ev, tiles;
    int64_t literal, matched, chain_matches, events;
    uint8_t md5c[16];
    int32_t md5c_valid, digests;
    int64_t flushes;
    int64_t t_total, t_tiles, t_check, t_event, t_digest;
    int64_t t_kset, t_chain, t_drain;
    int64_t t_evb;
    int32_t spec_full;
    int32_t aborted;
    int32_t mapped, first_mapped;
    int64_t clear_to;
    int32_t why, pad2;
    uint32_t elo, ehi;
    int32_t fin, pad3;
};
enum { CHAIN_WHY_NONE = 0, CHAIN_WHY_EVCAP, CHAIN_WHY_END, CHAIN_WHY_PHASE, CHAIN_WHY_TAIL, CHAIN_WHY_NOKSET,
       CHAIN_WHY_CUT, CHAIN_WHY_FLUSH, CHAIN_WHY_BUCKET, CHAIN_WHY_FLUSHHIT, CHAIN_WHY_DEADCAP, CHAIN_WHY_CLOSED,
       CHAIN_WHY_FLUSHED };
struct ChainHelp {
    int32_t nseg;
    int32_t claim;
    int32_t live;
    int32_t tiles;
    int64_t pos;
    int32_t mapped;
    int32_t joins;
    int64_t t_start, t_first;
    int64_t t_kset;
    int32_t whole;
    int32_t nhelp;
    int32_t help_tiles;
};
constexpr int CHAIN_THREADS = 512;
constexpr int CHAIN_PPT = 32;
constexpr int64_t CHAIN_TILE = (int64_t)CHAIN_THREADS * CHAIN_PPT;
constexpr int CHAIN_SEGS = 64;
constexpr int64_t CHAIN_MAP_SEG = 2 * CHAIN_TILE;

struct ChainFile {
    const uint8_t* data;
    int64_t n;
    uint32_t B;
    int32_t C, dl, rem;
    uint32_t kmask;
    const unsigned long long* kslots;
    const int32_t* table_weak;
    const uint8_t* table_strong;
    const int32_t* aw;
    const uint8_t* as;
    const uint8_t* flags;
    int64_t na;
    int64_t na_a;
    int* abort;
    rsh_event* ev;
    int32_t ev_cap;
    uint32_t seed;
    ChainOut* out;
    unsigned long long* hmap;
    int64_t hend;
    const uint8_t* dup;
};
hipError_t launch_k1_clock(const uint8_t* d_data, int64_t n, uint32_t B, uint32_t dl, uint32_t seed_word,
                           int32_t* d_weak, uint8_t* d_strong, unsigned long long* d_clk, hipStream_t s);
hipError_t launch_chain_advance(const ChainFile* files, uint32_t nfiles, hipStream_t s, int phase = 1,
                                int abort_gen = 0, ChainHelp* help = nullptr, uint32_t helpers = 0, bool timed = false);
struct ChunkIndexEnt {
    TableEnt t;
    uint8_t* dup;
};
hipError_t launch_chunk_index(const ChunkIndexEnt* ents, uint32_t nfiles, int32_t max_keys, hipStream_t s,
                              bool bg = false);

hipError_t launch_fill_splitmix(uint8_t* d_out, int64_t n, uint64_t key, int64_t byte_offset, hipStream_t s);

}
```

java-rsync_amd/csrc/device_chain.hip:

```cpp
#include <hip/hip_runtime.h>

#include "device.h"
#include "device_common.h"
#include "device_roll.h"
#include "md5_core.h"
#include "options.h"

#include <algorithm>
#include <type_traits>

namespace rsh {

constexpr int CHAIN_EV_LDS = 64;
__device__ __forceinline__ int64_t chain_clock(bool timed) {
#ifdef RSH_CHAIN_TIMERS_ALWAYS
    timed = true;
#endif
    return timed ? (int64_t)wall_clock64() : 0;
}

__device__ __forceinline__ bool kslots_has(const unsigned long long* __restrict__ ks, uint32_t mask, uint32_t key) {
    uint32_t h = slot_hash(key) & mask;
    for (;;) {
        const unsigned long long v = ks[h];
        if (v == 0ull) return false;
        if ((uint32_t)(v >> 32) == key) return true;
        h = (h + 1) & mask;
    }
}

constexpr int CHAIN_CK_BUCKETS = 8192;
__host__ __device__ constexpr uint32_t chain_ck_h1(uint32_t k) {
    return (((k ^ (k >> 15)) & 0xFFFFFFu) * 0x9E3779u) >> 19;
}
__host__ __device__ constexpr uint32_t chain_ck_h2(uint32_t k) {
    return CHAIN_CK_BUCKETS + ((((k ^ (k >> 8)) & 0xFFFFFFu) * 0x85EBCBu) >> 19);
}
__host__ __device__ constexpr uint32_t chain_ck_empty(uint32_t i) {
    return (i == chain_ck_h1(0u) || i == chain_ck_h2(0u)) ? 1u : 0u;
}
static_assert(chain_ck_h1(1u) != chain_ck_h1(0u) && chain_ck_h2(1u) != chain_ck_h2(0u), "empty values");
struct ChainKeySet {
    uint2* b;
    int32_t* full;
};
__device__ __forceinline__ void chain_ck_insert(const ChainKeySet& ks, uint32_t k) {
    uint32_t cur = k;
    int w = 0;
    for (int it = 0; it < 128; ++it) {
        const uint32_t bi = w == 0 ? chain_ck_h1(cur) : chain_ck_h2(cur), e = chain_ck_empty(bi);
        uint32_t* slot = reinterpret_cast<uint32_t*>(&ks.b[bi]);
#pragma unroll
        for (int j = 0; j < 2; ++j) {
            const uint32_t old = atomicCAS(slot + j, e, cur);
            if (old == e || old == cur) return;
        }
        const uint32_t old = atomicExch(slot + (it & 1), cur);
        if (old == cur) return;
        cur = old;
        w ^= 1;
    }
    *ks.full = 1;
}
__device__ __forceinline__ bool chain_ck_has(const ChainKeySet& ks, uint32_t k) {
    const uint2 a = ks.b[chain_ck_h1(k)], c = ks.b[chain_ck_h2(k)];
    return a.x == k || a.y == k || c.x == k || c.y == k;
}

__device__ __forceinline__ uint32_t chain_mask16(const ChainKeySet& set, const uint32_t (&keys)[16]) {
    uint32_t m = 0;
#pragma unroll
    for (int i = 0; i < 16; ++i) {
        const uint32_t k = keys[i];
        const uint2 x = set.b[chain_ck_h1(k)], y = set.b[chain_ck_h2(k)];
        m |= (uint32_t)((x.x == k) | (x.y == k) | (y.x == k) | (y.y == k)) << i;
        if ((i & 3) == 3) asm volatile("" ::: "memory");
    }
    return m;
}

__device__ __forceinline__ int chain_first_hit16(const unsigned long long* __restrict__ ks, uint32_t kmask,
                                                 const ChainKeySet& set, const uint32_t (&keys)[PROBE_PPT],
                                                 uint32_t valid) {
    if (*set.full == 0) {
        const uint32_t m = chain_mask16(set, keys) & valid;
        return m ? __builtin_ctz(m) : -1;
    }
    uint32_t hit = 0, need = 0;
    {
        unsigned long long sl[PROBE_PPT];
#pragma unroll
        for (int i = 0; i < PROBE_PPT; ++i) sl[i] = (valid >> i) & 1u ? ks[slot_hash(keys[i]) & kmask] : 0ull;
#pragma unroll
        for (int i = 0; i < PROBE_PPT; ++i) {
            if (sl[i] == 0ull) continue;
            if ((uint32_t)(sl[i] >> 32) == keys[i]) hit |= 1u << i;
            else need |= 1u << i;
        }
    }
    hit &= valid;
    need &= valid & (hit ? (hit & (0u - hit)) - 1u : 0xFFFFFFFFu);
    while (need) {
        const int i = __builtin_ctz(need);
        uint32_t kk = 0;
#pragma unroll
        for (int j = 0; j < PROBE_PPT; ++j)
            if (j == i) kk = keys[j];
        if (kslots_has(ks, kmask, kk)) return i;
        need &= need - 1u;
    }
    return hit ? __builtin_ctz(hit) : -1;
}

constexpr int CHAIN_WIN_BUF = 16384;
__device__ __forceinline__ uint32_t chain_window_stage(const uint8_t* x, uint32_t L, uint32_t seed, uint8_t* buf,
                                                       uint32_t c0) {
    const int t = threadIdx.x;
    const uint32_t len = L - c0 < (uint32_t)CHAIN_WIN_BUF ? L - c0 : (uint32_t)CHAIN_WIN_BUF;
    const bool last = c0 + len == L;
    const uintptr_t xa = reinterpret_cast<uintptr_t>(x) + c0, a0 = xa & ~(uintptr_t)15;
    const int32_t shift = (int32_t)(xa - a0);
    for (int32_t g = 16 * t; g < shift + (int32_t)len; g += 16 * CHAIN_THREADS) {
        const uint4 q = *reinterpret_cast<const uint4*>(a0 + (uintptr_t)g);
        const uint32_t w[4] = {q.x, q.y, q.z, q.w};
#pragma unroll
        for (int k = 0; k < 16; ++k) {
            const int32_t o = g + k - shift;
            if (o >= 0 && o < (int32_t)len) buf[o] = (uint8_t)(w[k >> 2] >> (8 * (k & 3)));
        }
    }
    const uint32_t plen = last ? ((len + 4 + 1 + 8 + 63) & ~63u) : len;
    if (last && (uint32_t)t < plen - len) {
        const uint32_t i = len + (uint32_t)t;
        const uint64_t bits = ((uint64_t)L + 4) * 8;
        uint32_t v = 0;
        if (t < 4) v = (seed >> (8 * t)) & 0xFFu;
        else if (t == 4) v = 0x80u;
        else if (i >= plen - 8) v = (uint32_t)(bits >> (8 * (i - (plen - 8)))) & 0xFFu;
        buf[i] = (uint8_t)v;
    }
    __syncthreads();
    return plen;
}
__device__ __attribute__((noinline)) void chain_window_digest(const uint8_t* x, uint32_t L, uint32_t dl, uint32_t seed,
                                                              uint8_t* buf, uint8_t* dig) {
    const int t = threadIdx.x;
    Md5State st = md5_init();
    for (uint32_t c0 = 0; c0 < L; c0 += CHAIN_WIN_BUF) {
        const uint32_t plen = chain_window_stage(x, L, seed, buf, c0);
        if (t == 0) {
            const uint4* bq = reinterpret_cast<const uint4*>(buf);
            for (uint32_t b = 0; b < plen / 64; ++b) {
                uint32_t m[16];
#pragma unroll
                for (int i = 0; i < 4; ++i) {
                    const uint4 v = bq[4 * b + i];
                    m[4 * i] = v.x, m[4 * i + 1] = v.y, m[4 * i + 2] = v.z, m[4 * i + 3] = v.w;
                }
                md5_compress(st, m);
            }
        }
        __syncthreads();
    }
    if (t == 0) store_digest(dig, st, dl);
    __syncthreads();
}

template <int NB>
__device__ __forceinline__ void chain_digest_load_n(const uint8_t* __restrict__ a, int dl, uint32_t (&w)[4]) {
#pragma unroll
    for (int k = 0; k < 4; ++k) w[k] = 0u;
#pragma unroll
    for (int j = 0; j < NB; ++j) {
        const uint32_t v = a[j < dl ? j : dl - 1];
        w[j >> 2] |= (j < dl ? v : 0u) << (8 * (j & 3));
    }
}
__device__ __forceinline__ void chain_digest_load(const uint8_t* __restrict__ a, int dl, uint32_t (&w)[4]) {
    if (dl <= 4) chain_digest_load_n<4>(a, dl, w);
    else if (dl <= 8) chain_digest_load_n<8>(a, dl, w);
    else chain_digest_load_n<16>(a, dl, w);
}
__device__ __forceinline__ bool chain_digest_eq_reg(const uint32_t (&a)[4], const uint8_t* __restrict__ b, int dl) {
    uint32_t w[4];
    chain_digest_load(b, dl, w);
    return ((a[0] ^ w[0]) | (a[1] ^ w[1]) | (a[2] ^ w[2]) | (a[3] ^ w[3])) == 0u;
}
__device__ __forceinline__ bool chain_digest_eq(const uint8_t* __restrict__ a, const uint8_t* __restrict__ b, int dl) {
    uint32_t w[4];
    chain_digest_load(a, dl, w);
    return chain_digest_eq_reg(w, b, dl);
}

__device__ __forceinline__ void chain_lane_sums(const uint32_t (&xa)[2][4], const uint32_t (&xb)[2][4], uint32_t base,
                                                uint32_t B, int32_t (&pre)[4]) {
    int32_t sa = 0, ja = 0, sb = 0, jb = 0;
#pragma unroll
    for (int hh = 0; hh < 2; ++hh)
#pragma unroll
        for (int d = 0; d < 4; ++d) {
            const int wt = 0x03020100 + 0x04040404 * d + 0x10101010 * hh;
            sa = __builtin_amdgcn_sdot4((int)xa[hh][d], 0x01010101, sa, false);
            ja = __builtin_amdgcn_sdot4((int)xa[hh][d], wt, ja, false);
            sb = __builtin_amdgcn_sdot4((int)xb[hh][d], 0x01010101, sb, false);
            jb = __builtin_amdgcn_sdot4((int)xb[hh][d], wt, jb, false);
        }
    pre[0] = sa;
    pre[1] = (int32_t)(base * (uint32_t)sa) + ja;
    pre[2] = sb;
    pre[3] = (int32_t)((base + B) * (uint32_t)sb) + jb;
}

__device__ __forceinline__ void chain_kset_build(const ChainKeySet& ks, const int32_t* __restrict__ weak, int64_t C) {
    const int t = threadIdx.x;
    for (int i = t; i < 2 * CHAIN_CK_BUCKETS; i += CHAIN_THREADS) {
        const uint32_t e = chain_ck_empty((uint32_t)i);
        ks.b[i] = make_uint2(e, e);
    }
    if (t == 0) *ks.full = 0;
    __syncthreads();
    for (int64_t c = t; c < C; c += CHAIN_THREADS) chain_ck_insert(ks, (uint32_t)weak[c]);
    __syncthreads();
}

__device__ __forceinline__ int32_t chain_ld(const int32_t* p) {
    return __hip_atomic_load(const_cast<int32_t*>(p), __ATOMIC_RELAXED, __HIP_MEMORY_SCOPE_AGENT);
}
__device__ __forceinline__ int64_t chain_ld64(const int64_t* p) {
    return __hip_atomic_load(const_cast<int64_t*>(p), __ATOMIC_RELAXED, __HIP_MEMORY_SCOPE_AGENT);
}
__device__ __forceinline__ void chain_st(int32_t* p, int32_t v) {
    __hip_atomic_store(p, v, __ATOMIC_RELAXED, __HIP_MEMORY_SCOPE_AGENT);
}
__device__ __forceinline__ void chain_st64(int64_t* p, int64_t v) {
    __hip_atomic_store(p, v, __ATOMIC_RELAXED, __HIP_MEMORY_SCOPE_AGENT);
}

struct ChainLds {
    ChainKeySet kset;
    int32_t* sh;
    int32_t (*seg)[4];
    int32_t* hit;
    uint32_t* key;
    int32_t* bk;
    int32_t* nbk;
    int64_t* zero;
    unsigned long long* best;
    int32_t* word;
    int32_t* live;
};

struct ChainTileKeys {
    int64_t p0, kb, o, kb0;
    uint32_t xa[2][4], xb[2][4];
    int32_t head[4], pre[4], To;
};
__device__ __forceinline__ void chain_tile_sums(ChainTileKeys& K, const ChainFile& F, int64_t q0, bool live,
                                                const ChainLds& L) {
    const int64_t n = F.n, B = F.B;
    K.kb0 = q0 / B;
    const int64_t o0 = K.kb0 * B;
#pragma unroll
    for (int v = 0; v < 4; ++v) K.head[v] = 0;
    if (q0 > o0) {
        range_sums(F.data, n, o0, q0, o0, K.head[0], K.head[1]);
        range_sums(F.data, n, o0 + B, q0 + B, o0, K.head[2], K.head[3]);
        block_reduce<4>(K.head, L.sh);
    }
    K.p0 = q0 + (int64_t)threadIdx.x * CHAIN_PPT;
    K.kb = K.p0 / B;
    K.o = K.kb * B;
    load16(F.data, n, K.p0, K.xa[0]);
    load16(F.data, n, K.p0 + 16, K.xa[1]);
    load16(F.data, n, K.p0 + B, K.xb[0]);
    load16(F.data, n, K.p0 + B + 16, K.xb[1]);
    K.To = live ? F.aw[K.kb] : 0;
    chain_lane_sums(K.xa, K.xb, (uint32_t)(K.p0 - q0), (uint32_t)B, K.pre);
    block_exscan<4>(K.pre, L.sh);
    if (K.p0 == K.o) {
#pragma unroll
        for (int v = 0; v < 4; ++v) L.seg[K.kb - K.kb0][v] = K.pre[v];
    }
}
__device__ __forceinline__ void chain_tile_start(const ChainTileKeys& K, int64_t q0, uint32_t B,
                                                 const int32_t (*seg)[4], uint32_t& u1, uint32_t& u2) {
    uint32_t pa, pa2, pb, pb2;
    if (K.o < q0) {
        const uint32_t d = (uint32_t)(q0 - K.o);
        pa = (uint32_t)K.head[0] + (uint32_t)K.pre[0];
        pa2 = (uint32_t)K.head[1] + (uint32_t)K.pre[1] + d * (uint32_t)K.pre[0];
        pb = (uint32_t)K.head[2] + (uint32_t)K.pre[2];
        pb2 = (uint32_t)K.head[3] + (uint32_t)K.pre[3] + d * (uint32_t)K.pre[2];
    } else {
        const int32_t* R = seg[K.kb - K.kb0];
        const uint32_t d = (uint32_t)(K.o - q0);
        pa = (uint32_t)(K.pre[0] - R[0]);
        pa2 = (uint32_t)(K.pre[1] - R[1]) - d * pa;
        pb = (uint32_t)(K.pre[2] - R[2]);
        pb2 = (uint32_t)(K.pre[3] - R[3]) - d * pb;
    }
    const uint32_t s1o = (uint32_t)K.To & 0xFFFFu, s2o = (uint32_t)K.To >> 16;
    const uint32_t P1e = s1o + pb;
    const uint32_t P2e = B * s1o - s2o + pb2;
    u1 = P1e - pa;
    u2 = (uint32_t)(K.p0 + B - K.o) * u1 - (P2e - pa2);
}
__device__ __forceinline__ void chain_tile_half(const ChainTileKeys& K, int hh, uint32_t B, uint32_t& u1, uint32_t& u2,
                                                uint32_t (&keys)[16]) {
    uint32_t wa[4], wb[4];
#pragma unroll
    for (int j = 0; j < 4; ++j) {
        wa[j] = hh ? K.xa[1][j] : K.xa[0][j];
        wb[j] = hh ? K.xb[1][j] : K.xb[0][j];
    }
#pragma unroll
    for (int i = 0; i < 16; ++i) {
        keys[i] = (u1 & 0xFFFFu) | (u2 << 16);
        const int32_t xo = sbyte_of(wa, i), xi = sbyte_of(wb, i);
        u1 += (uint32_t)(xi - xo);
        u2 += u1 - (uint32_t)__mul24((int)B, xo);
    }
}

__device__ void chain_map_tile(const ChainFile& F, int64_t q0, uint32_t gen, const ChainLds& L) {
    const int64_t p0 = q0 + (int64_t)threadIdx.x * CHAIN_PPT, hend = F.hend;
    const bool live = p0 < hend;
    ChainTileKeys K;
    chain_tile_sums(K, F, q0, live, L);
    __syncthreads();
    if (live) {
        uint32_t u1, u2;
        chain_tile_start(K, q0, F.B, L.seg, u1, u2);
        uint32_t bits = 0;
#pragma unroll 1
        for (int hh = 0; hh < 2; ++hh) {
            uint32_t keys[16];
            chain_tile_half(K, hh, F.B, u1, u2, keys);
            bits |= chain_mask16(L.kset, keys) << (16 * hh);
        }
        if (hend - p0 < 32) bits &= (1u << (uint32_t)(hend - p0)) - 1u;
        __hip_atomic_store(&F.hmap[p0 >> 5], ((unsigned long long)gen << 32) | bits, __ATOMIC_RELAXED,
                           __HIP_MEMORY_SCOPE_AGENT);
    }
    __syncthreads();
}

template <bool EARLY>
__device__ __forceinline__ int64_t chain_first_unset_flag(const uint8_t* __restrict__ flags, int64_t k, int64_t nflags,
                                                          int64_t* zero) {
    const int t = threadIdx.x;
    if (t == 0) *zero = nflags;
    __syncthreads();
    const uintptr_t fa = reinterpret_cast<uintptr_t>(flags);
    for (uintptr_t l0 = (fa + (uintptr_t)k) & ~(uintptr_t)15; l0 < fa + (uintptr_t)nflags; l0 += 16u * CHAIN_THREADS) {
        const uintptr_t la = l0 + 16u * (uintptr_t)t;
        const int64_t jb = (int64_t)la - (int64_t)fa;
        int64_t z = -1;
        if (la < fa + (uintptr_t)nflags) {
            uint32_t w[4] = {0x01010101u, 0x01010101u, 0x01010101u, 0x01010101u};
            if (la + 16 <= fa + (uintptr_t)nflags) {
                const uint4 q = *reinterpret_cast<const uint4*>(la);
                w[0] = q.x, w[1] = q.y, w[2] = q.z, w[3] = q.w;
            } else {
                for (int i = 0; i < 16; ++i)
                    if (jb + i >= 0 && jb + i < nflags && flags[jb + i] == 0) w[i >> 2] &= ~(0xFFu << (8 * (i & 3)));
            }
#pragma unroll
            for (int i = 15; i >= 0; --i)
                if (jb + i >= k && jb + i < nflags && ((w[i >> 2] >> (8 * (i & 3))) & 0xFFu) == 0u) z = jb + i;
        }
        if (z >= 0) atomicMin((unsigned long long*)zero, (unsigned long long)z);
        if (EARLY) {
            __syncthreads();
            if (*zero < nflags) break;
        }
    }
    if (!EARLY) __syncthreads();
    const int64_t first = *zero;
    __syncthreads();
    return first;
}

__device__ __forceinline__ bool chain_narrow_search(const ChainFile& F, int64_t a, int64_t stop, int64_t na,
                                                    const ChainLds& L, int32_t& tiles, int64_t& p, uint32_t& key) {
    const int t = threadIdx.x;
    const int64_t n = F.n, B = F.B;
    for (int64_t q0 = (a / B) * B + ((a % B) / PROBE_TILE) * PROBE_TILE; p < 0 && q0 <= stop;) {
        const int64_t kb = q0 / B, o = kb * B;
        if (kb >= na) return true;
        int64_t qend = q0 + PROBE_TILE;
        if (qend > o + B) qend = o + B;
        ++tiles;
        int32_t head[4] = {0, 0, 0, 0};
        if (q0 > o) {
            range_sums(F.data, n, o, q0, o, head[0], head[1]);
            range_sums(F.data, n, o + B, q0 + B, o, head[2], head[3]);
            block_reduce<4>(head, L.sh);
        }
        const int64_t p0 = q0 + (int64_t)t * PROBE_PPT;
        uint32_t xa[4], xb[4];
        load16(F.data, n, p0, xa);
        load16(F.data, n, p0 + B, xb);
        int32_t part[4] = {0, 0, 0, 0};
#pragma unroll
        for (int i = 0; i < PROBE_PPT; ++i) {
            const int32_t va = sbyte_of(xa, i), vb = sbyte_of(xb, i);
            part[0] += va;
            part[1] += (int32_t)((uint32_t)(p0 + i - o) * (uint32_t)va);
            part[2] += vb;
            part[3] += (int32_t)((uint32_t)(p0 + B + i - o) * (uint32_t)vb);
        }
        int32_t pre[4] = {part[0], part[1], part[2], part[3]};
        block_exscan<4>(pre, L.sh);
        if (t == 0) *L.hit = 0x7FFFFFFF;
        __syncthreads();
        uint32_t keys[PROBE_PPT];
        if (t < PROBE_THREADS && p0 < qend && p0 <= stop && p0 + PROBE_PPT > a) {
            const uint32_t pa = (uint32_t)(head[0] + pre[0]), pa2 = (uint32_t)(head[1] + pre[1]);
            const uint32_t pb = (uint32_t)(head[2] + pre[2]), pb2 = (uint32_t)(head[3] + pre[3]);
            const int32_t To = F.aw[kb];
            const uint32_t s1o = (uint32_t)To & 0xFFFFu, s2o = (uint32_t)To >> 16;
            const uint32_t P1e = s1o + pb;
            const uint32_t P2e = (uint32_t)B * s1o - s2o + pb2;
            const uint32_t s1 = P1e - pa;
            const uint32_t s2 = (uint32_t)(p0 + B - o) * s1 - (P2e - pa2);
            int32_t R = (int32_t)((s1 & 0xFFFFu) | (s2 << 16));
#pragma unroll
            for (int i = 0; i < PROBE_PPT; ++i) {
                keys[i] = (uint32_t)R;
                R = roll_add(roll_sub(R, (int32_t)B, sbyte_of(xa, i)), sbyte_of(xb, i));
            }
            uint32_t valid = 0;
#pragma unroll
            for (int i = 0; i < PROBE_PPT; ++i) {
                const int64_t pp = p0 + i;
                if (pp >= a && pp <= stop && pp < qend) valid |= 1u << i;
            }
            const int h = chain_first_hit16(F.kslots, F.kmask, L.kset, keys, valid);
            if (h >= 0) atomicMin(L.hit, (int32_t)(p0 + h - q0));
        }
        __syncthreads();
        const int32_t hoff = *L.hit;
        if (hoff != 0x7FFFFFFF && (hoff >> 4) == t) {
#pragma unroll
            for (int i = 0; i < PROBE_PPT; ++i)
                if (i == (hoff & 15)) *L.key = keys[i];
        }
        __syncthreads();
        if (hoff != 0x7FFFFFFF) {
            p = q0 + hoff;
            key = *L.key;
        }
        __syncthreads();
        q0 = qend;
    }
    return false;
}

__device__ __forceinline__ void chain_bucket_gather(const ChainFile& F, uint32_t key, const ChainLds& L) {
    const int t = threadIdx.x;
    if (t >= 64) return;
    int32_t cnt = 0;
    const unsigned long long* ks = F.kslots;
    uint32_t h = slot_hash(key) & F.kmask;
    for (bool more = true; more; h = (h + 64u) & F.kmask) {
        const unsigned long long v = ks[(h + (uint32_t)t) & F.kmask];
        const unsigned long long empty = __ballot(v == 0ull);
        const int lim = empty ? __builtin_ctzll(empty) : 64;
        const bool mine = t < lim && (uint32_t)(v >> 32) == key;
        const unsigned long long hits = __ballot(mine);
        const int at = cnt + __popcll(hits & ((1ull << t) - 1ull));
        if (mine && at < CHAIN_BUCKET_CAP) L.bk[at] = (int32_t)((uint32_t)v - 1u);
        cnt += __popcll(hits);
        more = empty == 0ull;
    }
    if (t == 0) {
        *L.nbk = cnt;
        for (int i = 1; i < cnt && i < CHAIN_BUCKET_CAP; ++i)
            for (int j = i; j > 0 && L.bk[j - 1] > L.bk[j]; --j) {
                const int32_t x = L.bk[j];
                L.bk[j] = L.bk[j - 1];
                L.bk[j - 1] = x;
            }
    }
}
__device__ __forceinline__ int32_t chain_close_index(const int32_t* bk, int32_t size, int32_t pref) {
    int32_t l = 0, r = size - 1;
    while (l <= r) {
        const int32_t mid = l + (r - l) / 2;
        if (bk[mid] == pref) return mid;
        if (bk[mid] < pref) l = mid + 1;
        else r = mid - 1;
    }
    return l < size - 1 ? l : size - 1;
}

struct ChainTally {
    int64_t lit, mat, chain_matches, events, flushes;
    int32_t tiles, digests, mapped, first_mapped;
    int64_t t_tiles, t_check, t_event, t_digest, t_kset, t_chain, t_drain, t_evb;
};
__device__ __forceinline__ void chain_write_out(const ChainFile& F, int phase, int abort_gen, int64_t s, int64_t m,
                                                int32_t pref, int32_t nev, int32_t status, int32_t why,
                                                int64_t clear_to, uint32_t elo, uint32_t ehi, const uint8_t* stale,
                                                bool dead, const ChainTally& N, int64_t t_total) {
    ChainOut* out = F.out;
    out->s = s;
    out->m = m;
    out->pref = pref;
    out->status = status;
    out->n_ev = nev;
    out->tiles = N.tiles;
    out->digests = N.digests;
    out->flushes = N.flushes;
    out->t_total += t_total;
    out->t_tiles += N.t_tiles;
    out->t_check += N.t_check;
    out->t_event += N.t_event;
    out->t_digest += N.t_digest;
    out->t_kset += N.t_kset;
    out->t_chain += N.t_chain;
    out->t_drain += N.t_drain;
    out->t_evb += N.t_evb;
    out->spec_full = phase == 1;
    out->mapped = N.mapped;
    out->clear_to = clear_to;
    out->why = why;
    out->elo = elo;
    out->ehi = ehi;
    out->first_mapped = N.first_mapped;
    const bool stop_spec = phase == 0 && F.abort && (status == CHAIN_DONE || dead);
    out->aborted = stop_spec;
    if (stop_spec) *(volatile int*)F.abort = abort_gen;
    out->md5c_valid = stale != nullptr;
    if (stale != nullptr)
        for (int j = 0; j < F.dl && j < 16; ++j) out->md5c[j] = stale[j];
    out->literal = N.lit;
    out->matched = N.mat;
    out->chain_matches = N.chain_matches;
    out->events = N.events;
    __threadfence_system();
    *(volatile int32_t*)&out->fin = 1;
}

constexpr int CHAIN_HELP_LEAD = 64;
__device__ __attribute__((noinline)) void chain_help(const ChainFile* __restrict__ files, int nfiles, uint32_t gen,
                                                     ChainHelp* help, const ChainLds L, bool timed) {
    const int t = threadIdx.x;
    int cur = -1;
    ChainFile F = files[0];
    for (;;) {
        if (t == 0) {
            *L.best = 0ull;
            *L.live = 0;
        }
        __syncthreads();
        for (int f = t; f < nfiles; f += CHAIN_THREADS) {
            ChainHelp* h = help + f;
            const int32_t nseg = h->nseg;
            if (nseg == 0) continue;
            const int32_t live = chain_ld(&h->live), tiles = chain_ld(&h->tiles), claim = chain_ld(&h->claim);
            const int32_t nhelp = chain_ld(&h->nhelp);
            const int64_t pos = chain_ld64(&h->pos);
            if (live == 0 || claim >= nseg) continue;
            *L.live = 1;
            if (tiles < h->help_tiles) continue;
            const int64_t lead = (int64_t)claim - pos / CHAIN_MAP_SEG;
            const uint32_t level = lead <= 0 ? 3u : lead <= 4 ? 2u : lead <= 16 ? 1u : 0u;
            const uint32_t few = 255u - (uint32_t)(nhelp < 0 ? 0 : nhelp > 255 ? 255 : nhelp);
            const uint32_t tie = ((uint32_t)f * 0x9E3779B1u) ^ ((uint32_t)blockIdx.x * 0x85EBCA77u);
            const unsigned long long key = ((unsigned long long)(f == cur && lead < CHAIN_HELP_LEAD) << 63) |
                                           ((unsigned long long)level << 61) | ((unsigned long long)few << 53) |
                                           ((unsigned long long)(tie >> 1) << 21) | (uint32_t)f;
            atomicMax(L.best, key);
        }
        __syncthreads();
        const unsigned long long best = *L.best;
        const bool any_live = *L.live != 0;
        __syncthreads();
        if (best == 0ull) {
            if (!any_live) break;
            __builtin_amdgcn_s_sleep(64);
            continue;
        }
        const int f = (int)(best & 0xFFFFFull);
        ChainHelp* h = help + f;
        if (t == 0) {
            atomicMax(&h->claim, (int32_t)(chain_ld64(&h->pos) / CHAIN_MAP_SEG) + 1);
            *L.word = atomicAdd(&h->claim, 1);
        }
        __syncthreads();
        const int32_t seg = *L.word;
        __syncthreads();
        if (seg >= h->nseg) continue;
        if (f != cur) {
            if (t == 0) {
                if (cur >= 0) atomicSub(&help[cur].nhelp, 1);
                atomicAdd(&h->nhelp, 1);
            }
            cur = f;
            const int64_t tb = chain_clock(timed);
            F = files[f];
            chain_kset_build(L.kset, F.table_weak, F.C);
            if (t == 0) {
                atomicAdd((unsigned long long*)&h->t_kset, (unsigned long long)(chain_clock(timed) - tb));
                atomicAdd(&h->joins, 1);
            }
            if (*L.kset.full) {
                if (t == 0) atomicMax(&h->claim, h->nseg);
                __syncthreads();
                continue;
            }
        }
        const int64_t lo = (int64_t)seg * CHAIN_MAP_SEG, hi = lo + CHAIN_MAP_SEG < F.hend ? lo + CHAIN_MAP_SEG : F.hend;
        bool whole = true;
        for (int64_t q0 = lo; q0 < hi; q0 += CHAIN_TILE) {
            if (t == 0) *L.word = chain_ld(&h->live) != 0 && chain_ld64(&h->pos) < q0 + CHAIN_TILE;
            __syncthreads();
            const bool go = *L.word != 0;
            __syncthreads();
            if (!go) {
                whole = false;
                break;
            }
            chain_map_tile(F, q0, gen, L);
        }
        if (t == 0) {
            atomicAdd(&h->mapped, 1);
            if (whole) {
                atomicAdd(&h->whole, 1);
                atomicMin((unsigned long long*)&h->t_first, (unsigned long long)chain_clock(timed));
            }
        }
    }
    if (t == 0 && cur >= 0) atomicSub(&help[cur].nhelp, 1);
}

__global__ __launch_bounds__(CHAIN_THREADS) void chain_advance_kernel(const ChainFile* __restrict__ files, int phase,
                                                                      int abort_gen, ChainHelp* help, int nfiles,
                                                                      int timed) {
    __builtin_amdgcn_s_setprio(3);
    __shared__ int32_t sh[4 * CHAIN_THREADS / 64];
    __shared__ int32_t s_hit;
    __shared__ uint32_t s_key;
    __shared__ int32_t s_sc[4];
    __shared__ int32_t s_bk[CHAIN_BUCKET_CAP];
    __shared__ int32_t s_nbk;
    __shared__ int64_t s_zero;
    __shared__ __attribute__((aligned(16))) uint8_t s_win[CHAIN_WIN_BUF + 128];
    __shared__ int32_t s_any;
    __shared__ int32_t s_seg[CHAIN_SEGS][4];
    __shared__ uint2 s_ck[2 * CHAIN_CK_BUCKETS];
    __shared__ int32_t s_ck_full;
    __shared__ __attribute__((aligned(16))) uint8_t s_dig[16];
    __shared__ rsh_event s_ev[CHAIN_EV_LDS];
    __shared__ unsigned long long s_best;
    __shared__ int32_t s_word, s_live;
    const ChainKeySet kset{s_ck, &s_ck_full};
    ChainLds L;
    L.kset = kset, L.sh = sh, L.seg = s_seg, L.hit = &s_hit, L.key = &s_key, L.bk = s_bk, L.nbk = &s_nbk;
    L.zero = &s_zero, L.best = &s_best, L.word = &s_word, L.live = &s_live;
    if ((int)blockIdx.x >= nfiles) {
        chain_help(files, nfiles, (uint32_t)abort_gen, help, L, timed != 0);
        return;
    }
    const ChainFile F = files[blockIdx.x];
    ChainHelp* const H = (phase == 0 && help != nullptr) ? help + blockIdx.x : nullptr;
    if (H != nullptr && threadIdx.x == 0) chain_st64(&H->t_start, chain_clock(timed));
    const uint32_t map_gen = (H != nullptr && F.hmap != nullptr) ? (uint32_t)abort_gen : 0u;
    ChainOut* out = F.out;
    if (phase == 1 && out->status != CHAIN_MORE) return;
    const int t = threadIdx.x;
    const int64_t n = F.n, B = F.B, C = F.C;
    const int dl = F.dl;
    const int64_t S = F.rem > 0 ? F.rem : B;
    const int64_t last = n - S, nB = n - B;
    const int64_t na = phase == 0 ? F.na_a : F.na, nflags = na < C ? na : C;
    const bool wide = (B % CHAIN_PPT) == 0 && B >= 512 && CHAIN_TILE / B + 2 <= CHAIN_SEGS;
    int64_t s = out->s, m = out->m;
    bool kset_built = true;
    if (s % B == 0 && nflags >= na)
        kset_built = chain_first_unset_flag<false>(F.flags, s / B, nflags, &s_zero) < nflags;
    const int64_t tks0 = chain_clock(timed);
    if (kset_built) chain_kset_build(kset, F.table_weak, C);
    ChainTally N{out->literal, out->matched, out->chain_matches, out->events, out->flushes, out->tiles, out->digests,
                 out->mapped, out->first_mapped, 0, 0, 0, 0, chain_clock(timed) - tks0, 0, 0, 0};
    int32_t pref = out->pref;
    int32_t nev = out->n_ev, status = CHAIN_STOP;
    int32_t poisoned = 0, dead = 0;
    const int64_t tk0 = chain_clock(timed);
    const uint8_t* stale = nullptr;
    uint32_t dg[4] = {0u, 0u, 0u, 0u};
    int64_t clear_to = -1;
    int32_t why = CHAIN_WHY_NONE;
    uint32_t desync_lo = 0, desync_hi = 0;
    int64_t pf_s = -1;
    int32_t pf_pref = -1, pf_aw = 0, pf_tw = 0;
    uint8_t pf_flag = 0;
    rsh_event pend{0, 0, 0, 0, 0, 0};
    bool have = false;
    if (nev > 0) {
        pend = F.ev[nev - 1];
        have = true;
        --nev;
    }
    int32_t nev_w = nev;
    auto drain_ev = [&]() {
        const int64_t tdr0 = chain_clock(timed);
        __syncthreads();
        for (int32_t i = t; i < nev - nev_w; i += CHAIN_THREADS) F.ev[nev_w + i] = s_ev[i];
        nev_w = nev;
        __syncthreads();
        N.t_drain += chain_clock(timed) - tdr0;
    };
    auto flush_pend = [&]() {
        if (have) {
            if (t == 0) s_ev[nev - nev_w] = pend;
            ++nev;
        }
        have = false;
    };
    auto emit_lit = [&](int64_t off, int64_t len) {
        if (len <= 0) return;
        flush_pend();
        pend = rsh_event{off, len, RSH_EV_LITERAL, 0, 0, 0};
        have = true;
        N.lit += len;
    };
    auto emit_match = [&](int64_t off, int64_t len, int32_t idx, int32_t cnt) {
        N.mat += len;
        if (have && pend.kind == RSH_EV_MATCH && pend.index + pend.count == idx && pend.offset + pend.length == off) {
            pend.count += cnt;
            pend.length += len;
            return;
        }
        flush_pend();
        pend = rsh_event{off, len, RSH_EV_MATCH, idx, cnt, 0};
        have = true;
    };

    for (;;) {
        if (nev - nev_w >= CHAIN_EV_LDS - 8) drain_ev();
        if (nev + 3 > F.ev_cap) {
            why = CHAIN_WHY_EVCAP;
            break;
        }
        if (s > last) {
            emit_lit(m, n - m);
            status = CHAIN_DONE;
            why = CHAIN_WHY_END;
            break;
        }
        if (s % B != 0 && !poisoned) {
            why = CHAIN_WHY_PHASE;
            break;
        }
        const int64_t k = s / B;
        const bool al = s % B == 0;
        const bool pf_use = pf_s == s && pf_pref == pref && !poisoned;
        const uint8_t flag_k = pf_use ? pf_flag : (!poisoned && k == pref && k < nflags) ? F.flags[k] : (uint8_t)0;
        const int32_t aw_k = pf_use ? pf_aw : (al && k < na) ? F.aw[k] : 0;
        const int32_t tw_pref = pf_use ? pf_tw : (!poisoned && pref < C && k < na) ? F.table_weak[pref] : 0;
        pf_s = -1;
        const int64_t tch0 = chain_clock(timed);
        if (flag_k) {
            const int64_t j_end = chain_first_unset_flag<true>(F.flags, k, nflags, &s_zero);
            const int64_t t_max = (last - s) / B + 1;
            const int64_t tt = (j_end - k < t_max) ? j_end - k : t_max;
            const int64_t j = k + tt, p = (s + tt * B < n) ? s + tt * B : n;
            emit_lit(m, s - m);
            emit_match(s, p - s, (int32_t)k, (int32_t)(j - k));
            N.chain_matches += j - k;
            s = m = p;
            pref = (int32_t)j;
            N.t_chain += chain_clock(timed) - tch0;
            continue;
        }
        if (!poisoned && pref < C && k < na) {
            int64_t lim = na - k;
            if (C - pref < lim) lim = C - pref;
            if ((last - s) / B + 1 < lim) lim = (last - s) / B + 1;
            int64_t tt = 0;
            if (lim > 0 && aw_k == tw_pref && chain_digest_eq(F.as + k * dl, F.table_strong + (int64_t)pref * dl, dl)) {
                tt = 1;
                while (tt < lim && F.aw[k + tt] == F.table_weak[pref + tt] &&
                       chain_digest_eq(F.as + (k + tt) * dl, F.table_strong + (pref + tt) * dl, dl))
                    ++tt;
            }
            if (tt > 0) {
                const int64_t p = (s + tt * B < n) ? s + tt * B : n;
                emit_lit(m, s - m);
                emit_match(s, p - s, pref, (int32_t)tt);
                s = m = p;
                pref += (int32_t)tt;
                N.t_chain += chain_clock(timed) - tch0;
                continue;
            }
        }
        N.t_chain += chain_clock(timed) - tch0;
        const int64_t f = (m + 10 * B <= n) ? m + 9 * B : INT64_MAX;
        const int64_t stop = f < last ? f : last;
        if (stop > nB) {
            why = CHAIN_WHY_TAIL;
            break;
        }
        if (!kset_built && (s / B < na || s <= (stop < na * B - 1 ? stop : na * B - 1))) {
            why = CHAIN_WHY_NOKSET;
            break;
        }
        int64_t p = -1;
        uint32_t key = 0;
        int64_t a = s;
        if (al && k < na) {
            key = (uint32_t)aw_k;
            if (s_ck_full ? kslots_has(F.kslots, F.kmask, key) : chain_ck_has(kset, key)) p = s;
            else a = s + 1;
        }
        bool sc_hit = false;
        bool cut = false;
        if (wide) {
            const int64_t lim_spec = na * B - 1;
            const int64_t qlast = stop < lim_spec ? stop : lim_spec;
            if (H != nullptr && t == 0) {
                chain_st64(&H->pos, a);
                chain_st(&H->tiles, N.tiles);
            }
            for (int64_t q0 = a & ~(int64_t)(CHAIN_PPT - 1); p < 0 && q0 <= qlast;) {
                ++N.tiles;
                const int64_t tt0 = chain_clock(timed);
                if (map_gen != 0u) {
                    const int64_t pm = q0 + (int64_t)t * CHAIN_PPT;
                    const int64_t lo = a > pm ? a - pm : 0, hi = qlast - pm;
                    const bool need = lo <= 31 && hi >= lo;
                    unsigned long long wv = 0ull;
                    if (need) wv = __hip_atomic_load(&F.hmap[pm >> 5], __ATOMIC_RELAXED, __HIP_MEMORY_SCOPE_AGENT);
                    const bool al_lane = need && pm % B == 0;
                    const int32_t awl = al_lane ? F.aw[pm / B] : 0;
                    const int64_t kl = pm / B, kl1 = kl + 1;
                    int32_t scw[4] = {0, 0, 0, 0};
// ... 164 lines not shown
                pos = it;
            }
            const int32_t c = s_bk[pos];
            const bool eq = (diag && c == kp) ? ((dg[0] ^ dgk[0]) | (dg[1] ^ dgk[1]) | (dg[2] ^ dgk[2]) | (dg[3] ^ dgk[3])) == 0u
                                              : chain_digest_eq_reg(dg, F.table_strong + (int64_t)c * dl, dl);
            if (eq) hit = c;
        }
        __syncthreads();
        N.t_event += chain_clock(timed) - te0;
        if (hit < 0) {
            if (p < f) {
                s = p + 1;
                if (poisoned) continue;
                poisoned = 1;
                stale = md5c;
                if (t == 0) s_any = 0;
                __syncthreads();
                {
                    bool any = false;
                    for (int64_t c = t; c < C; c += 2 * CHAIN_THREADS) {
                        const int64_t c2 = c + CHAIN_THREADS < C ? c + CHAIN_THREADS : c;
                        any |= (int)chain_digest_eq_reg(dg, F.table_strong + c * dl, dl) |
                               (int)chain_digest_eq_reg(dg, F.table_strong + c2 * dl, dl);
                    }
                    if (any) s_any = 1;
                }
                __syncthreads();
                dead = s_any == 0;
                if (dead) {
                    const int64_t nfl = s <= last ? (n - m) / (10 * B) : 0;
                    if (nev + nfl + 3 <= F.ev_cap) {
                        flush_pend();
                        drain_ev();
                        for (int64_t i = t; i < nfl; i += CHAIN_THREADS)
                            F.ev[nev + i] = rsh_event{m + 10 * B * i, 10 * B, RSH_EV_LITERAL, 0, 0, 0};
                        nev += (int32_t)nfl;
                        nev_w = nev;
                        N.lit += 10 * B * nfl;
                        m += 10 * B * nfl;
                        N.flushes += nfl;
                        emit_lit(m, n - m);
                        s = n;
                        status = CHAIN_DONE;
                        poisoned = 0;
                    }
                }
                if (!dead) continue;
                why = status == CHAIN_DONE ? CHAIN_WHY_CLOSED : CHAIN_WHY_DEADCAP;
            } else {
                if (!poisoned) {
                    poisoned = 1;
                    stale = md5c;
                }
                emit_lit(m, p + B - m);
                ++N.flushes;
                const int64_t s2 = p + B;
                s = m = s2;
                if (s2 <= last) {
                    const int32_t jx = (int32_t)(int8_t)F.data[p];
                    uint32_t rlo = (key & 0xFFFFu) - (uint32_t)jx, rhi = (key >> 16) - (uint32_t)B * (uint32_t)jx;
                    if (n - s2 >= B) {
                        rlo += (uint32_t)(int32_t)(int8_t)F.data[s2 + B - 1];
                        rhi += rlo;
                    }
                    uint32_t T2;
                    if (s2 % B == 0 && s2 / B < na) {
                        T2 = (uint32_t)F.aw[s2 / B];
                    } else {
                        const int64_t L2 = n - s2 < B ? n - s2 : B;
                        int32_t w2[2] = {0, 0};
                        range_sums(F.data, n, s2, s2 + L2, s2, w2[0], w2[1]);
                        block_reduce<2>(w2, sh);
                        const uint32_t S1 = (uint32_t)w2[0], S2 = (uint32_t)L2 * S1 - (uint32_t)w2[1];
                        T2 = (S1 & 0xFFFFu) | (S2 << 16);
                    }
                    desync_lo = (rlo - T2) & 0xFFFFu;
                    desync_hi = (rhi - (T2 >> 16)) & 0xFFFFu;
                }
                why = CHAIN_WHY_FLUSHED;
            }
            break;
        }
        emit_lit(m, p - m);
        emit_match(p, w, hit, 1);
        pref = hit + 1;
        s = m = p + w;
        poisoned = 0;
    }
    flush_pend();
    drain_ev();
    if (t == 0)
        chain_write_out(F, phase, abort_gen, s, m, pref, nev, status, why, clear_to, desync_lo, desync_hi,
                        poisoned ? stale : nullptr, dead != 0, N, chain_clock(timed) - tk0);
    if (H != nullptr) {
        if (t == 0) chain_st(&H->live, 0);
        __syncthreads();
        chain_help(files, nfiles, (uint32_t)abort_gen, help, L, timed != 0);
    }
}

hipError_t launch_chain_advance(const ChainFile* files, uint32_t nfiles, hipStream_t s, int phase, int abort_gen,
                                ChainHelp* help, uint32_t helpers, bool timed) {
    if (nfiles == 0) return hipSuccess;
    if (phase != 0 || help == nullptr || nfiles >= (1u << 20)) {
        help = nullptr;
        helpers = 0;
    }
    hipLaunchKernelGGL(chain_advance_kernel, dim3(nfiles + helpers), dim3(CHAIN_THREADS), 0, s, files, phase,
                       abort_gen, help, (int)nfiles, timed ? 1 : 0);
    return hipGetLastError();
}

constexpr int CHUNK_INDEX_MLP = 8;
__global__ void chunk_index_kernel(const ChunkIndexEnt* __restrict__ ents, uint32_t nfiles) {
    const TableEnt e = ents[blockIdx.y].t;
    uint8_t* const dup = ents[blockIdx.y].dup;
    const int64_t stride = (int64_t)gridDim.x * blockDim.x;
    for (int64_t i0 = blockIdx.x * (int64_t)blockDim.x + threadIdx.x; i0 < e.nkeys; i0 += CHUNK_INDEX_MLP * stride) {
        unsigned long long v[CHUNK_INDEX_MLP], got[CHUNK_INDEX_MLP];
        uint32_t h[CHUNK_INDEX_MLP];
#pragma unroll
        for (int j = 0; j < CHUNK_INDEX_MLP; ++j) {
            const int64_t i = i0 + j * stride;
            const uint32_t key = i < e.nkeys ? (uint32_t)e.keys[i] : 0u;
            v[j] = ((unsigned long long)key << 32) | (uint32_t)(i + 1);
            h[j] = slot_hash(key) & e.mask;
        }
#pragma unroll
        for (int j = 0; j < CHUNK_INDEX_MLP; ++j)
            got[j] = i0 + j * stride < e.nkeys ? atomicCAS(&e.slots[h[j]], 0ull, v[j]) : 0ull;
#pragma unroll
        for (int j = 0; j < CHUNK_INDEX_MLP; ++j) {
            unsigned long long g = got[j];
            uint32_t hh = h[j];
            while (g != 0ull) {
                if ((g >> 32) == (v[j] >> 32)) {
                    dup[(uint32_t)v[j] - 1] = 1;
                    dup[(uint32_t)g - 1] = 1;
                }
                hh = (hh + 1) & e.mask;
                g = atomicCAS(&e.slots[hh], 0ull, v[j]);
            }
        }
    }
    (void)nfiles;
}

hipError_t launch_chunk_index(const ChunkIndexEnt* ents, uint32_t nfiles, int32_t max_keys, hipStream_t s, bool bg) {
    if (nfiles == 0 || max_keys <= 0) return hipSuccess;
    const uint32_t gx = (uint32_t)std::min<int64_t>((max_keys + 255) / 256, bg ? 2 : 64);
    hipLaunchKernelGGL(chunk_index_kernel, dim3(gx, nfiles), dim3(256), 0, s, ents, nfiles);
    return hipGetLastError();
}
__global__ void warm_chain_kernel() {}
constexpr int kWarmScratchWords = 160;
__global__ __launch_bounds__(CHAIN_THREADS) void warm_scratch_kernel(int32_t sel, int32_t* out) {
    volatile int32_t a[kWarmScratchWords];
    for (int i = 0; i < kWarmScratchWords; ++i) a[i] = i ^ sel;
    const int32_t v = a[(threadIdx.x + (uint32_t)sel) % kWarmScratchWords];
    if (out && v == 0x7FFFFFFF) out[0] = v;
}
hipError_t launch_warm_chain(hipStream_t s) {
    hipLaunchKernelGGL(warm_chain_kernel, dim3(1), dim3(64), 0, s);
    hipLaunchKernelGGL(warm_scratch_kernel, dim3(256), dim3(CHAIN_THREADS), 0, s, 1, nullptr);
    return hipGetLastError();
}

}
```

java-rsync_amd/csrc/options.h:

```cpp
#pragma once
#include <stdint.h>
#include <string.h>

#include <atomic>

namespace rsh {

enum Opt : int {
    OPT_K1_GATHER,
    OPT_K1_SHIFT,
    OPT_K1_UNALIGNED,
    OPT_SCAN_TRACE,
    OPT_SCAN_SEGMENTED,
    OPT_SCAN_SAMPLES,
    OPT_BATCH_CHAIN,
    OPT_BATCH_CHAIN_PREFIX,
    OPT_HOST_CORES,
    OPT_FILE_TILE,
    OPT_FILE_TILE_ABOVE,
    OPT_PROBE_LONG,
    OPT_SEGMENT_BYTES,
    OPT_MD5_WIDTH,
    OPT_CHAIN_HELPERS,
    OPT_CHAIN_MAP_BYTES,
    OPT_TIME_GEN,
    OPT_BATCH_WARM,
    OPT_FAULT_INJECT,
    OPT_TOKENS_SPAN,
    OPT_TOKENS_PIECE,
    OPT_SUMS_PIECE,
    OPT_TOKENS_RUNS,
    OPT_COUNT
};

struct OptInfo {
    const char* name;
    int64_t def;
};

inline constexpr OptInfo kOpts[OPT_COUNT] = {
    {"k1_gather", 1},           {"k1_shift", 1},        {"k1_unaligned", 1},
    {"scan_trace", 0},          {"scan_segmented", 1},  {"scan_samples", 256},
    {"batch_chain", 1},         {"batch_chain_prefix", -1}, {"host_cores", 0},
    {"file_tile", 4LL << 30},   {"file_tile_above", 32LL << 30}, {"probe_long", 1},
    {"segment_bytes", 16LL << 30}, {"md5_width", 0},    {"chain_helpers", -1},
    {"chain_map_bytes", 1LL << 30}, {"time_gen", 1},    {"batch_warm", 128},
    {"fault_inject", 0},        {"tokens_span", 256LL << 10}, {"tokens_piece", 8LL << 20},
    {"sums_piece", 32LL << 20}, {"tokens_runs", 64LL << 10},
};

inline const OptInfo* opt_info() { return kOpts; }

inline std::atomic<int64_t>* opt_table() {
    static std::atomic<int64_t> v[OPT_COUNT] = {};
    static std::atomic<bool> init{false};
    if (!init.load(std::memory_order_acquire)) {
        static std::atomic_flag once = ATOMIC_FLAG_INIT;
        if (!once.test_and_set()) {
            for (int i = 0; i < OPT_COUNT; ++i) v[i].store(kOpts[i].def, std::memory_order_relaxed);
            init.store(true, std::memory_order_release);
        } else {
            while (!init.load(std::memory_order_acquire)) {
            }
        }
    }
    return v;
}

inline int64_t opt(Opt o) { return opt_table()[o].load(std::memory_order_relaxed); }

inline int opt_index(const char* name) {
    for (int i = 0; i < OPT_COUNT; ++i)
        if (name && strcmp(name, kOpts[i].name) == 0) return i;
    return -1;
}

}
```

java-rsync_amd/rsync_hip.py:

```python
import ctypes
import os
import subprocess

import numpy as np

HERE = os.path.dirname(os.path.abspath(__file__))
LIB_PATH = os.environ.get("RSH_LIB") or os.path.join(HERE, "lib", "librsynchip.so")

RSH_OK, RSH_E_INVAL, RSH_E_PROTOCOL, RSH_E_OVERFLOW, RSH_E_NOSPACE, RSH_E_DEVICE, RSH_E_NOMEM, RSH_E_BUSY = \
    0, -1, -2, -3, -4, -5, -6, -7
RSH_E_NOTFOUND, RSH_E_OPEN, RSH_E_NOSOURCE = -8, -9, -10
EV_LITERAL, EV_MATCH = 1, 2


class ProtocolError(Exception):
    """RsyncProtocolException (Connection.receiveChecksumHeader, Connection.java:28-38)."""


class FileViewNotFound(FileNotFoundError):
    """RSH_E_NOTFOUND (io/FileViewNotFound: new FileView on a missing file, FileView.java:74-75)."""


class FileViewOpenFailed(OSError):
    """RSH_E_OPEN (io/FileViewOpenFailed, FileView.java:76-78)."""


class ContextBusyError(RuntimeError):
    """RSH_E_BUSY: a Context was called from two threads at once (use one Context per thread)."""


class DeviceError(RuntimeError):
    """HIP failure or no gfx950 device."""


class NoSourceError(RuntimeError):
    """RSH_E_NOSOURCE: the context holds no source from its last scan (tiled, trimmed, or its buffers reused since);
    the caller replays the literals from its own copy of the file."""


class Header(ctypes.Structure):
    _fields_ = [("chunk_count", ctypes.c_int32), ("block_length", ctypes.c_int32),
                ("digest_length", ctypes.c_int32), ("remainder", ctypes.c_int32)]

    def as_dict(self):
        return dict(chunk_count=self.chunk_count, block_length=self.block_length,
                    digest_length=self.digest_length, remainder=self.remainder)

    def smallest_chunk_size(self):
        return self.remainder if self.remainder > 0 else self.block_length


class Event(ctypes.Structure):
    _fields_ = [("offset", ctypes.c_int64), ("length", ctypes.c_int64), ("kind", ctypes.c_int32),
                ("index", ctypes.c_int32), ("count", ctypes.c_int32), ("reserved", ctypes.c_int32)]


class ScanStats(ctypes.Structure):
    _fields_ = [("chain_matches", ctypes.c_int64), ("events", ctypes.c_int64), ("probe_launches", ctypes.c_int64),
                ("host_md5_windows", ctypes.c_int64), ("flushes", ctypes.c_int64),
                ("device_ms", ctypes.c_double), ("resolver_ms", ctypes.c_double), ("table_ms", ctypes.c_double),
                ("head_steps", ctypes.c_int64), ("speculation_aborted", ctypes.c_int64),
                ("device_bytes", ctypes.c_int64), ("phase_launches", ctypes.c_int64),
                ("phase_matches", ctypes.c_int64), ("spec_kernel_ms", ctypes.c_double),
                ("phase_kernel_ms", ctypes.c_double), ("phase_guesses", ctypes.c_int64)]

    def as_dict(self):
        return {f: getattr(self, f) for f, _ in self._fields_}


class BlockJob(ctypes.Structure):
    _fields_ = [("d_data", ctypes.c_void_p), ("n", ctypes.c_int64), ("h", Header), ("d_weak", ctypes.c_void_p),
                ("d_strong", ctypes.c_void_p)]


class ScanJob(ctypes.Structure):
    _fields_ = [("d_src", ctypes.c_void_p), ("n", ctypes.c_int64), ("h", Header), ("d_weak", ctypes.c_void_p),
                ("d_strong", ctypes.c_void_p), ("ev", ctypes.c_void_p), ("ev_cap", ctypes.c_int64),
                ("n_ev", ctypes.c_int64), ("literal", ctypes.c_int64), ("matched", ctypes.c_int64),
                ("status", ctypes.c_int32), ("reserved", ctypes.c_int32)]


class CombineResult(ctypes.Structure):
    _fields_ = [("tokens_used", ctypes.c_int64), ("target_len", ctypes.c_int64), ("literal", ctypes.c_int64),
                ("matched", ctypes.c_int64), ("intact", ctypes.c_int32), ("reserved", ctypes.c_int32),
                ("md5", ctypes.c_uint8 * 16)]


class Piece(ctypes.Structure):
    _fields_ = [("data", ctypes.c_void_p), ("len", ctypes.c_int64)]


class CombineJob(ctypes.Structure):
    _fields_ = [("tokens", ctypes.c_void_p), ("tokens_len", ctypes.c_int64), ("h", Header),
                ("replica", ctypes.POINTER(Piece)), ("nreplica", ctypes.c_int32), ("defer_write", ctypes.c_int32),
                ("target", ctypes.c_void_p), ("target_cap", ctypes.c_int64), ("status", ctypes.c_int32),
                ("reserved", ctypes.c_int32), ("res", CombineResult)]


class BlockBatchJob(ctypes.Structure):
    _fields_ = [("pieces", ctypes.POINTER(Piece)), ("npieces", ctypes.c_int32), ("status", ctypes.c_int32),
                ("h", Header), ("weak_out", ctypes.c_void_p), ("strong_out", ctypes.c_void_p)]


class ScanBatchJob(ctypes.Structure):
    _fields_ = [("pieces", ctypes.POINTER(Piece)), ("npieces", ctypes.c_int32), ("status", ctypes.c_int32),
                ("h", Header), ("weak", ctypes.c_void_p), ("strong", ctypes.c_void_p), ("ev", ctypes.c_void_p),
                ("ev_cap", ctypes.c_int64), ("n_ev", ctypes.c_int64), ("literal", ctypes.c_int64),
                ("matched", ctypes.c_int64), ("file_md5", ctypes.c_uint8 * 16)]


class BlockWireJob(ctypes.Structure):
    _fields_ = [("pieces", ctypes.POINTER(Piece)), ("npieces", ctypes.c_int32), ("status", ctypes.c_int32),
                ("h", Header), ("out", ctypes.c_void_p), ("out_cap", ctypes.c_int64), ("out_len", ctypes.c_int64)]


class SendJob(ctypes.Structure):
    _fields_ = [("pieces", ctypes.POINTER(Piece)), ("npieces", ctypes.c_int32), ("status", ctypes.c_int32),
                ("h", Header), ("table", ctypes.c_void_p), ("table_len", ctypes.c_int64), ("ev", ctypes.c_void_p),
                ("ev_cap", ctypes.c_int64), ("n_ev", ctypes.c_int64), ("literal", ctypes.c_int64),
                ("matched", ctypes.c_int64), ("file_md5", ctypes.c_uint8 * 16), ("out", ctypes.c_void_p),
                ("out_cap", ctypes.c_int64), ("out_len", ctypes.c_int64), ("out_status", ctypes.c_int32),
                ("reserved", ctypes.c_int32)]


class TokenJob(ctypes.Structure):
    _fields_ = [("d_src", ctypes.c_void_p), ("n", ctypes.c_int64), ("ev", ctypes.c_void_p), ("n_ev", ctypes.c_int64),
                ("file_md5", ctypes.c_uint8 * 16), ("out", ctypes.c_void_p), ("out_cap", ctypes.c_int64),
                ("out_len", ctypes.c_int64), ("status", ctypes.c_int32), ("reserved", ctypes.c_int32)]


class Md5Job(ctypes.Structure):
    _fields_ = [("pieces", ctypes.POINTER(Piece)), ("npieces", ctypes.c_int32), ("reserved", ctypes.c_int32),
                ("md5", ctypes.c_uint8 * 16)]


class TokenRun(ctypes.Structure):
    _fields_ = [("pos", ctypes.c_int64), ("kind", ctypes.c_int32), ("value", ctypes.c_int32),
                ("count", ctypes.c_int64)]


COMBINE_NO_MD5 = 1
SCAN_MORE, SCAN_END = 0, 1

EVENT_DTYPE = np.dtype([("offset", "<i8"), ("length", "<i8"), ("kind", "<i4"), ("index", "<i4"),
                        ("count", "<i4"), ("reserved", "<i4")])

EXPORTS = ["rsh_abi_version", "rsh_strerror", "rsh_last_error", "rsh_device_count", "rsh_ctx_create", "rsh_ctx_destroy",
           "rsh_ctx_stream", "rsh_block_length_for", "rsh_digest_length_for", "rsh_header_make",
           "rsh_header_validate", "rsh_block_sums", "rsh_block_sums_device", "rsh_ctx_sync", "rsh_ctx_trim", "rsh_match_scan",
           "rsh_match_scan_device", "rsh_match_scan_tiled", "rsh_fetch_events", "rsh_file_md5", "rsh_tokens_size", "rsh_tokens_write", "rsh_generator_bytes",
           "rsh_block_sums_batch_device", "rsh_match_scan_batch_device", "rsh_receiver_combine",
           "rsh_receiver_combine_device", "rsh_receiver_combine_batch", "rsh_block_sums_file", "rsh_match_scan_file", "rsh_block_sums_pieces", "rsh_match_scan_pieces", "rsh_block_sums_batch", "rsh_match_scan_batch", "rsh_block_sums_batch_multi", "rsh_match_scan_batch_multi", "rsh_receiver_combine_batch_multi", "rsh_shard_files", "rsh_file_md5_batch", "rsh_dev_alloc", "rsh_dev_free", "rsh_memcpy_h2d", "rsh_memcpy_d2h", "rsh_fill_splitmix_device",
           "rsh_tokens_write_device", "rsh_tokens_write_kept", "rsh_tokens_write_batch_device",
           "rsh_sums_wire_size", "rsh_header_from_wire", "rsh_sums_frame_device", "rsh_sums_unframe_device",
           "rsh_block_sums_batch_wire", "rsh_match_scan_batch_wire", "rsh_block_sums_batch_wire_multi",
           "rsh_match_scan_batch_wire_multi", "rsh_tokens_frame_device", "rsh_receiver_combine_resident"]
DEBUG_EXPORTS = ["rsh_debug_set_option", "rsh_debug_get_option", "rsh_debug_reset_options", "rsh_debug_k1_clock",
                 "rsh_debug_streams_busy", "rsh_debug_kernel_ms", "rsh_debug_multi_selftest", "rsh_debug_generation",
                 "rsh_debug_tokens_selftest", "rsh_debug_sums_selftest", "rsh_debug_tokens_scan_selftest",
                 "rsh_debug_untokens_selftest"]

_LIB = None


def build(force=False):
    cmd = ["make", "-s", "-C", HERE] + (["-B"] if force else [])
    subprocess.run(cmd, check=True)


def stale_sources():
    import hashlib
    stamp = os.path.splitext(LIB_PATH)[0] + ".srchash"
    if not os.path.exists(stamp):
        return []
    out = []
    for line in open(stamp):
        digest, _, rel = line.strip().partition("  ")
        path = os.path.join(HERE, rel)
        if os.path.exists(path) and hashlib.sha256(open(path, "rb").read()).hexdigest() != digest:
            out.append(rel)
    return out


def lib():
    global _LIB
    if _LIB is not None:
        return _LIB
    if not os.path.exists(LIB_PATH):
        raise DeviceError(f"{LIB_PATH} missing: run rsync_hip.build() (or __graft_entry__.build())")
    stale = stale_sources()
    if stale:
        raise DeviceError(f"{LIB_PATH} was built from other sources than {', '.join(stale)}: rebuild it")
    L = ctypes.CDLL(LIB_PATH)
    P, I32, I64 = ctypes.c_void_p, ctypes.c_int32, ctypes.c_int64
    HP = ctypes.POINTER(Header)
    sig = {
        "rsh_abi_version": ([], ctypes.c_int),
        "rsh_strerror": ([ctypes.c_int], ctypes.c_char_p),
        "rsh_last_error": ([], ctypes.c_char_p),
        "rsh_device_count": ([ctypes.POINTER(ctypes.c_int)], ctypes.c_int),
        "rsh_ctx_create": ([ctypes.c_int, ctypes.POINTER(P)], ctypes.c_int),
        "rsh_ctx_destroy": ([P], None),
        "rsh_ctx_stream": ([P], P),
        "rsh_block_length_for": ([I64], I32),
        "rsh_digest_length_for": ([I64, I32, I32], I32),
        "rsh_header_make": ([I32, I32, I64, HP], ctypes.c_int),
        "rsh_header_validate": ([HP], ctypes.c_int),
        "rsh_block_sums": ([P, P, I64, HP, P, P, P], ctypes.c_int),
        "rsh_block_sums_device": ([P, P, I64, HP, P, P, P], ctypes.c_int),
        "rsh_ctx_sync": ([P], ctypes.c_int),
        "rsh_ctx_trim": ([P], ctypes.c_int),
        "rsh_match_scan": ([P, P, I64, HP, P, P, P, P, I64, ctypes.POINTER(I64), P, ctypes.POINTER(I64),
                            ctypes.POINTER(I64), ctypes.POINTER(ScanStats)], ctypes.c_int),
        "rsh_match_scan_device": ([P, P, I64, HP, P, P, P, P, I64, ctypes.POINTER(I64), ctypes.POINTER(I64),
                                   ctypes.POINTER(I64), ctypes.POINTER(ScanStats)], ctypes.c_int),
        "rsh_match_scan_tiled": ([P, P, I64, HP, P, P, P, I64, P, I64, ctypes.POINTER(I64), P, ctypes.POINTER(I64),
                                  ctypes.POINTER(I64), ctypes.POINTER(ScanStats)], ctypes.c_int),
        "rsh_fetch_events": ([P, P, I64, ctypes.POINTER(I64)], ctypes.c_int),
        "rsh_file_md5": ([P, I64, P], ctypes.c_int),
        "rsh_tokens_size": ([P, I64], I64),
        "rsh_tokens_write": ([P, P, I64, P, P, I64], ctypes.c_int),
        "rsh_generator_bytes": ([HP, P, P, P, I64], I64),
        "rsh_block_sums_batch_device": ([P, ctypes.POINTER(BlockJob), I32, P], ctypes.c_int),
        "rsh_match_scan_batch_device": ([P, ctypes.POINTER(ScanJob), I32, P, ctypes.POINTER(ScanStats)],
                                        ctypes.c_int),
        "rsh_receiver_combine": ([P, P, I64, HP, P, I64, I32, P, I64, ctypes.POINTER(CombineResult)], ctypes.c_int),
        "rsh_receiver_combine_batch": ([P, ctypes.POINTER(CombineJob), I32], ctypes.c_int),
        "rsh_receiver_combine_device": ([P, P, I64, HP, P, I64, I32, P, I64, ctypes.POINTER(CombineResult)],
                                        ctypes.c_int),
        "rsh_block_sums_file": ([P, ctypes.c_char_p, I64, HP, P, P, P, ctypes.POINTER(I32)], ctypes.c_int),
        "rsh_match_scan_file": ([P, ctypes.c_char_p, I64, HP, P, P, P, P, I64, ctypes.POINTER(I64), P,
                                 ctypes.POINTER(I64), ctypes.POINTER(I64), ctypes.POINTER(ScanStats),
                                 ctypes.POINTER(I32)], ctypes.c_int),
        "rsh_block_sums_pieces": ([P, ctypes.POINTER(Piece), I32, HP, P, P, P], ctypes.c_int),
        "rsh_match_scan_pieces": ([P, ctypes.POINTER(Piece), I32, HP, P, P, P, P, I64, ctypes.POINTER(I64), P,
                                   ctypes.POINTER(I64), ctypes.POINTER(I64), ctypes.POINTER(ScanStats)], ctypes.c_int),
        "rsh_block_sums_batch": ([P, ctypes.POINTER(BlockBatchJob), I32, P], ctypes.c_int),
        "rsh_match_scan_batch": ([P, ctypes.POINTER(ScanBatchJob), I32, P, ctypes.POINTER(ScanStats)], ctypes.c_int),
        "rsh_block_sums_batch_multi": ([ctypes.POINTER(P), I32, ctypes.POINTER(BlockBatchJob), I32, P], ctypes.c_int),
        "rsh_match_scan_batch_multi": ([ctypes.POINTER(P), I32, ctypes.POINTER(ScanBatchJob), I32, P,
                                        ctypes.POINTER(ScanStats)], ctypes.c_int),
        "rsh_receiver_combine_batch_multi": ([ctypes.POINTER(P), I32, ctypes.POINTER(CombineJob), I32], ctypes.c_int),
        "rsh_shard_files": ([P, I32, I32, P], ctypes.c_int),
        "rsh_file_md5_batch": ([ctypes.POINTER(Md5Job), I32, I32], ctypes.c_int),
        "rsh_dev_alloc": ([P, I64, ctypes.POINTER(P)], ctypes.c_int),
        "rsh_dev_free": ([P, P], ctypes.c_int),
        "rsh_memcpy_h2d": ([P, P, P, I64], ctypes.c_int),
        "rsh_memcpy_d2h": ([P, P, P, I64], ctypes.c_int),
        "rsh_fill_splitmix_device": ([P, P, I64, ctypes.c_uint64, I64], ctypes.c_int),
        "rsh_debug_set_option": ([ctypes.c_char_p, I64], ctypes.c_int),
        "rsh_debug_get_option": ([ctypes.c_char_p, ctypes.POINTER(I64)], ctypes.c_int),
        "rsh_debug_reset_options": ([], None),
        "rsh_debug_k1_clock": ([P, P, I64, I32, I32, ctypes.POINTER(ctypes.c_double)], ctypes.c_int),
        "rsh_debug_streams_busy": ([P, ctypes.POINTER(ctypes.c_int32)], ctypes.c_int),
        "rsh_debug_generation": ([P, I32, ctypes.POINTER(ctypes.c_int32)], ctypes.c_int),
        "rsh_debug_kernel_ms": ([P, I32, ctypes.POINTER(ctypes.c_double)], ctypes.c_int),
        "rsh_debug_multi_selftest": ([P, I32, I32, I32, P, P, P], ctypes.c_int),
        "rsh_tokens_write_device": ([P, P, I64, P, I64, P, I64, P, I64], ctypes.c_int),
        "rsh_tokens_write_kept": ([P, P, I64, P, I64, P, I64], ctypes.c_int),
        "rsh_tokens_write_batch_device": ([P, ctypes.POINTER(TokenJob), I32], ctypes.c_int),
        "rsh_debug_tokens_selftest": ([P, I64, P, I64, P, I64, P, I64, I64, ctypes.POINTER(I64)], ctypes.c_int),
        "rsh_sums_wire_size": ([HP], I64),
        "rsh_header_from_wire": ([P, HP], ctypes.c_int),
        "rsh_sums_frame_device": ([P, HP, P, P, P, I64], ctypes.c_int),
        "rsh_sums_unframe_device": ([P, HP, P, I64, P, P], ctypes.c_int),
        "rsh_block_sums_batch_wire": ([P, ctypes.POINTER(BlockWireJob), I32, P], ctypes.c_int),
        "rsh_match_scan_batch_wire": ([P, ctypes.POINTER(SendJob), I32, P, ctypes.POINTER(ScanStats)], ctypes.c_int),
        "rsh_block_sums_batch_wire_multi": ([ctypes.POINTER(P), I32, ctypes.POINTER(BlockWireJob), I32, P],
                                            ctypes.c_int),
        "rsh_match_scan_batch_wire_multi": ([ctypes.POINTER(P), I32, ctypes.POINTER(SendJob), I32, P,
                                             ctypes.POINTER(ScanStats)], ctypes.c_int),
        "rsh_debug_sums_selftest": ([I32, HP, P, P, P, I64, I64, ctypes.POINTER(I64)], ctypes.c_int),
        "rsh_tokens_frame_device": ([P, P, I64, P, I64, P, I64, P, I64], ctypes.c_int),
        "rsh_receiver_combine_resident": ([P, P, I64, HP, P, I64, I32, P, I64, I32, ctypes.POINTER(CombineResult)],
                                          ctypes.c_int),
        "rsh_debug_tokens_scan_selftest": ([P, P, I64, I64, ctypes.POINTER(TokenRun), I64, ctypes.POINTER(I64),
                                            ctypes.POINTER(I64), ctypes.POINTER(I32)], ctypes.c_int),
        "rsh_debug_untokens_selftest": ([P, P, I64, I64, I32, I64, P, I64, ctypes.POINTER(I64), ctypes.POINTER(I64),
                                         ctypes.POINTER(I64)], ctypes.c_int),
    }
    for name, (args, res) in sig.items():
        fn = getattr(L, name)
        fn.argtypes = args
        fn.restype = res
    _LIB = L
    return L


def _check(rc):
    if rc == RSH_OK:
        return
    msg = lib().rsh_strerror(rc).decode()
    if rc == RSH_E_INVAL:
        raise ValueError(msg)
    if rc == RSH_E_PROTOCOL:
        raise ProtocolError(msg)
    if rc == RSH_E_OVERFLOW:
        raise OverflowError(msg)
    if rc == RSH_E_NOMEM:
        raise MemoryError(msg)
    if rc == RSH_E_BUSY:
        raise ContextBusyError(msg)
    if rc == RSH_E_NOTFOUND:
        raise FileViewNotFound(msg)
    if rc == RSH_E_OPEN:
        raise FileViewOpenFailed(msg)
    if rc == RSH_E_NOSOURCE:
        raise NoSourceError(msg)
    detail = lib().rsh_last_error().decode()
    raise DeviceError(f"{msg}: {detail}" if detail else msg)


def _ptr(a):
    return None if a is None else ctypes.c_void_p(a.ctypes.data)


def _u8(data):
    if isinstance(data, np.ndarray):
        return np.ascontiguousarray(data.view(np.uint8).reshape(-1))
    return np.frombuffer(bytes(data), dtype=np.uint8)


def block_length_for(n):
    return lib().rsh_block_length_for(n)


def digest_length_for(n, blen, min_digest=2):
    return lib().rsh_digest_length_for(n, blen, min_digest)


def header_make(blen, dlen, n):
    h = Header()
    _check(lib().rsh_header_make(blen, dlen, n, ctypes.byref(h)))
    return h


def header_validate(h):
    _check(lib().rsh_header_validate(ctypes.byref(h)))


def file_md5(data):
    a = _u8(data)
    out = np.zeros(16, np.uint8)
    _check(lib().rsh_file_md5(_ptr(a), a.size, _ptr(out)))
    return out.tobytes()


def _piece_list(pieces):
    arrs = [_u8(p) for p in pieces]
    pl = (Piece * max(len(arrs), 1))()
    for i, a in enumerate(arrs):
        pl[i].data, pl[i].len = (a.ctypes.data if a.size else None), a.size
    return arrs, pl, sum(a.size for a in arrs)


def file_md5_batch(files, threads=0):
    keep, jobs = [], (Md5Job * max(len(files), 1))()
    for i, pieces in enumerate(files):
        arrs, pl, _ = _piece_list(pieces)
        keep.append((arrs, pl))
        jobs[i].pieces, jobs[i].npieces = ctypes.cast(pl, ctypes.POINTER(Piece)), len(arrs)
    _check(lib().rsh_file_md5_batch(jobs, len(files), threads))
    return [bytes(jobs[i].md5) for i in range(len(files))]


def scan_event_cap(n, h):
    if h.block_length <= 0:
        return n // 8192 + 2
    return 2 * (n // h.block_length + 1) + n // (10 * h.block_length) + 4


def events_as_tuples(ev, block_length):
    out = []
    for e in ev:
        if e["kind"] == EV_LITERAL:
            out.append((EV_LITERAL, int(e["offset"]), int(e["length"]), 0))
        else:
            off, left, cnt = int(e["offset"]), int(e["length"]), int(e["count"])
            for j in range(cnt):
                w = left if j == cnt - 1 else block_length
                out.append((EV_MATCH, off, w, int(e["index"]) + j))
                off += w
                left -= w
    return out


def tokens(src, ev, file_md5_bytes):
    a = _u8(src)
    ev = np.ascontiguousarray(ev, dtype=EVENT_DTYPE)
    n = ev.size
    size = lib().rsh_tokens_size(_ptr(ev) if n else None, n)
    out = np.zeros(size, np.uint8)
    fm = np.frombuffer(file_md5_bytes, np.uint8).copy()
    _check(lib().rsh_tokens_write(_ptr(a), _ptr(ev) if n else None, n, _ptr(fm), _ptr(out), size))
    return out.tobytes()


def tokens_size(ev):
    ev = np.ascontiguousarray(ev, dtype=EVENT_DTYPE)
    return lib().rsh_tokens_size(_ptr(ev) if ev.size else None, ev.size)


def tokens_selftest(src, ev, file_md5_bytes, start=0, length=None, span=0, out=None):
    a = _u8(src)
    ev = np.ascontiguousarray(ev, dtype=EVENT_DTYPE)
    fm = np.frombuffer(file_md5_bytes, np.uint8).copy()
    if length is None:
        length = tokens_size(ev) - start
    if out is None:
        out = np.zeros(max(length, 1), np.uint8)
    nd = ctypes.c_int64()
    _check(lib().rsh_debug_tokens_selftest(_ptr(a) if a.size else None, a.size, _ptr(ev) if ev.size else None, ev.size,
                                           _ptr(fm), start, _ptr(out), length, span, ctypes.byref(nd)))
    return out[:max(length, 0)].tobytes(), nd.value


def _addr(x):
    if isinstance(x, np.ndarray):
        return ctypes.c_void_p(x.ctypes.data)
    if isinstance(x, DeviceBuffer):
        return x.ptr
    return ctypes.c_void_p(x or None)


def tokens_scan_selftest(tokens, length, start=0, cap=1 << 16, ctx=None):
    runs = (TokenRun * cap)()
    n, pos, st = ctypes.c_int64(), ctypes.c_int64(), ctypes.c_int32()
    _check(lib().rsh_debug_tokens_scan_selftest(None if ctx is None else ctx.handle, _addr(tokens), length, start, runs,
                                                cap, ctypes.byref(n), ctypes.byref(pos), ctypes.byref(st)))
    return [(r.pos, r.kind, r.value, r.count) for r in runs[:n.value]], pos.value, st.value


def untokens_selftest(tokens, length, pos, T, count, out, span=0, ctx=None):
    nd, lo, hi = ctypes.c_int64(), ctypes.c_int64(), ctypes.c_int64()
    _check(lib().rsh_debug_untokens_selftest(None if ctx is None else ctx.handle, _addr(tokens), length, pos, T, count,
                                             _addr(out), span, ctypes.byref(nd), ctypes.byref(lo), ctypes.byref(hi)))
    return nd.value, lo.value, hi.value


def sums_wire_size(h):
    return lib().rsh_sums_wire_size(ctypes.byref(h))


def header_from_wire(wire):
    a = _u8(wire)
    if a.size != 16:
        raise ValueError("a checksum header is 16 bytes")
    h = Header()
    _check(lib().rsh_header_from_wire(_ptr(a), ctypes.byref(h)))
    return h


def sums_selftest(h, weak=None, strong=None, wire=None, span=0, unframe=False):
    nd = ctypes.c_int64()
    _check(lib().rsh_debug_sums_selftest(int(bool(unframe)), ctypes.byref(h), _ptr(weak) if weak is not None and weak.size else None,
                                         _ptr(strong) if strong is not None and strong.size else None,
                                         _ptr(wire) if wire is not None and wire.size else None,
                                         0 if wire is None else wire.size, span, ctypes.byref(nd)))
    return nd.value


def set_option(name, value):
    _check(lib().rsh_debug_set_option(name.encode(), int(value)))


def get_option(name):
    v = ctypes.c_int64()
    _check(lib().rsh_debug_get_option(name.encode(), ctypes.byref(v)))
    return v.value


def reset_options():
    lib().rsh_debug_reset_options()


class option:

    def __init__(self, name, value):
        self.name, self.value = name, value

    def __enter__(self):
        self.old = get_option(self.name)
        set_option(self.name, self.value)
        return self

    def __exit__(self, *a):
        set_option(self.name, self.old)


def device_count():
    c = ctypes.c_int(0)
    rc = lib().rsh_device_count(ctypes.byref(c))
    return c.value if rc == RSH_OK else 0


class Context:

    def __init__(self, device=0):
        self._p = ctypes.c_void_p()
        _check(lib().rsh_ctx_create(device, ctypes.byref(self._p)))

    def close(self):
        if self._p:
            lib().rsh_ctx_destroy(self._p)
            self._p = ctypes.c_void_p()

    def __enter__(self):
        return self

    def __exit__(self, *a):
        self.close()

    def __del__(self):
        try:
            self.close()
        except Exception:
            pass

    @property
    def handle(self):
        return self._p

    def kernel_ms(self, which):
        ms = ctypes.c_double(-1.0)
        _check(lib().rsh_debug_kernel_ms(self._p, which, ctypes.byref(ms)))
        return ms.value

    def generation(self, set_to=-1):
        g = ctypes.c_int32(0)
        _check(lib().rsh_debug_generation(self._p, set_to, ctypes.byref(g)))
        return g.value

    def streams_busy(self):
        m = ctypes.c_int32(-1)
        _check(lib().rsh_debug_streams_busy(self._p, ctypes.byref(m)))
        return m.value

    def sync(self):
        _check(lib().rsh_ctx_sync(self._p))

    def _block_batch(self, jobs, n, seed):
        return lib().rsh_block_sums_batch(self._p, jobs, n, seed)

    def _scan_batch(self, jobs, n, seed, stats):
        return lib().rsh_match_scan_batch(self._p, jobs, n, seed, stats)

    def _combine_batch(self, jobs, n):
        return lib().rsh_receiver_combine_batch(self._p, jobs, n)

    def _block_batch_wire(self, jobs, n, seed):
        return lib().rsh_block_sums_batch_wire(self._p, jobs, n, seed)

    def _scan_batch_wire(self, jobs, n, seed, stats):
        return lib().rsh_match_scan_batch_wire(self._p, jobs, n, seed, stats)

    def trim(self):
        _check(lib().rsh_ctx_trim(self._p))

    def alloc(self, nbytes):
        return DeviceBuffer(self, nbytes)

    def block_sums(self, data, h, seed):
        a = _u8(data)
        s = np.frombuffer(bytes(seed), np.uint8).copy()
        weak = np.zeros(max(h.chunk_count, 1), np.int32)
        strong = np.zeros(max(h.chunk_count * h.digest_length, 1), np.uint8)
        _check(lib().rsh_block_sums(self._p, _ptr(a), a.size, ctypes.byref(h), _ptr(s), _ptr(weak), _ptr(strong)))
        return weak[:h.chunk_count], strong[:h.chunk_count * h.digest_length]

    def match_scan(self, src, h, weak, strong, seed, ev_cap=None):
        a = _u8(src)
        s = np.frombuffer(bytes(seed), np.uint8).copy()
        w = np.ascontiguousarray(weak, dtype=np.int32)
        st = np.ascontiguousarray(strong, dtype=np.uint8)
        cap = ev_cap if ev_cap is not None else int(a.size // max(10 * h.block_length, 1) + 2 * h.chunk_count + 64)
        ev = np.zeros(max(cap, 1), EVENT_DTYPE)
        n_ev, lit, mat = ctypes.c_int64(), ctypes.c_int64(), ctypes.c_int64()
        fm = np.zeros(16, np.uint8)
        stats = ScanStats()
        rc = lib().rsh_match_scan(self._p, _ptr(a), a.size, ctypes.byref(h), _ptr(w) if w.size else None,
                                  _ptr(st) if st.size else None, _ptr(s), _ptr(ev), cap, ctypes.byref(n_ev),
                                  _ptr(fm), ctypes.byref(lit), ctypes.byref(mat), ctypes.byref(stats))
        if rc == RSH_E_NOSPACE and ev_cap is None:
            ev = np.zeros(n_ev.value, EVENT_DTYPE)
            rc = lib().rsh_fetch_events(self._p, _ptr(ev), n_ev.value, ctypes.byref(n_ev))
        _check(rc)
        return ev[:n_ev.value], fm.tobytes(), lit.value, mat.value, stats.as_dict()

    def match_scan_tiled(self, src, h, weak, strong, seed, tile_bytes=0, digest=True, ev_cap=None):
        a = _u8(src)
        s = np.frombuffer(bytes(seed), np.uint8).copy()
        w = np.ascontiguousarray(weak, dtype=np.int32)
        st = np.ascontiguousarray(strong, dtype=np.uint8)
        cap = ev_cap if ev_cap is not None else int(a.size // max(10 * h.block_length, 1) + 2 * h.chunk_count + 64)
        ev = np.zeros(max(cap, 1), EVENT_DTYPE)
        n_ev, lit, mat = ctypes.c_int64(), ctypes.c_int64(), ctypes.c_int64()
        fm = np.zeros(16, np.uint8)
        stats = ScanStats()
        rc = lib().rsh_match_scan_tiled(self._p, _ptr(a), a.size, ctypes.byref(h), _ptr(w) if w.size else None,
                                        _ptr(st) if st.size else None, _ptr(s), tile_bytes, _ptr(ev), cap,
                                        ctypes.byref(n_ev), _ptr(fm) if digest else None, ctypes.byref(lit),
                                        ctypes.byref(mat), ctypes.byref(stats))
        if rc == RSH_E_NOSPACE and ev_cap is None:
            ev = np.zeros(n_ev.value, EVENT_DTYPE)
            rc = lib().rsh_fetch_events(self._p, _ptr(ev), n_ev.value, ctypes.byref(n_ev))
        _check(rc)
        return ev[:n_ev.value], (fm.tobytes() if digest else None), lit.value, mat.value, stats.as_dict()

    @staticmethod
    def _pieces(pieces):
        return _piece_list(pieces)

    def block_sums_batch(self, files, seed, statuses=None):
        s = np.frombuffer(bytes(seed), np.uint8).copy()
        jobs = (BlockBatchJob * max(len(files), 1))()
        keep, outs = [], []
        for i, (pieces, h) in enumerate(files):
            arrs, pl, _ = _piece_list(pieces)
            w = np.zeros(max(h.chunk_count, 1), np.int32)
            st = np.zeros(max(h.chunk_count * h.digest_length, 1), np.uint8)
            keep.append((arrs, pl))
            outs.append((w, st, h))
            jobs[i].pieces, jobs[i].npieces, jobs[i].h = ctypes.cast(pl, ctypes.POINTER(Piece)), len(arrs), h
            jobs[i].weak_out, jobs[i].strong_out = w.ctypes.data, st.ctypes.data
        rc = self._block_batch(jobs, len(files), _ptr(s))
        if statuses is not None:
            statuses[:] = [rc] + [jobs[i].status for i in range(len(files))]
        else:
            _check(rc)
        return [(w[:h.chunk_count], st[:h.chunk_count * h.digest_length]) for w, st, h in outs]

    def match_scan_batch(self, files, seed, ev_caps=None, statuses=None):
        s = np.frombuffer(bytes(seed), np.uint8).copy()
        jobs = (ScanBatchJob * max(len(files), 1))()
        keep, evs = [], []
        for i, (pieces, h, weak, strong) in enumerate(files):
            arrs, pl, n = _piece_list(pieces)
            w = np.ascontiguousarray(weak, dtype=np.int32)
            st = np.ascontiguousarray(strong, dtype=np.uint8)
            cap = ev_caps[i] if ev_caps is not None else scan_event_cap(n, h)
            ev = np.zeros(max(cap, 1), EVENT_DTYPE)
            keep.append((arrs, pl, w, st))
            evs.append(ev)
            j = jobs[i]
            j.pieces, j.npieces, j.h = ctypes.cast(pl, ctypes.POINTER(Piece)), len(arrs), h
            j.weak, j.strong = (w.ctypes.data if w.size else None), (st.ctypes.data if st.size else None)
            j.ev, j.ev_cap = ev.ctypes.data, cap
        stats = ScanStats()
        rc = self._scan_batch(jobs, len(files), _ptr(s), ctypes.byref(stats))
        if statuses is not None:
            statuses[:] = [rc]
        elif rc != RSH_E_NOSPACE:
            _check(rc)
        out = []
        for i in range(len(files)):
            j = jobs[i]
            ev = evs[i][:j.n_ev] if j.status == RSH_OK else evs[i][:0]
            out.append((ev, bytes(j.file_md5), j.literal, j.matched, j.status))
        return out, stats.as_dict()

    def block_sums_pieces(self, pieces, h, seed):
        arrs, pl, _ = self._pieces(pieces)
        s = np.frombuffer(bytes(seed), np.uint8).copy()
        weak = np.zeros(max(h.chunk_count, 1), np.int32)
        strong = np.zeros(max(h.chunk_count * h.digest_length, 1), np.uint8)
        _check(lib().rsh_block_sums_pieces(self._p, pl, len(arrs), ctypes.byref(h), _ptr(s), _ptr(weak), _ptr(strong)))
        return weak[:h.chunk_count], strong[:h.chunk_count * h.digest_length]

    def match_scan_pieces(self, pieces, h, weak, strong, seed):
        arrs, pl, n = self._pieces(pieces)
        s = np.frombuffer(bytes(seed), np.uint8).copy()
        w = np.ascontiguousarray(weak, dtype=np.int32)
        st = np.ascontiguousarray(strong, dtype=np.uint8)
        cap = int(n // max(10 * h.block_length, 1) + 2 * h.chunk_count + 64) if h.block_length else n // 8192 + 2
        ev = np.zeros(max(cap, 1), EVENT_DTYPE)
        n_ev, lit, mat = ctypes.c_int64(), ctypes.c_int64(), ctypes.c_int64()
        fm = np.zeros(16, np.uint8)
        stats = ScanStats()
        rc = lib().rsh_match_scan_pieces(self._p, pl, len(arrs), ctypes.byref(h), _ptr(w) if w.size else None,
                                         _ptr(st) if st.size else None, _ptr(s), _ptr(ev), cap, ctypes.byref(n_ev),
                                         _ptr(fm), ctypes.byref(lit), ctypes.byref(mat), ctypes.byref(stats))
        if rc == RSH_E_NOSPACE:
            ev = np.zeros(n_ev.value, EVENT_DTYPE)
            rc = lib().rsh_fetch_events(self._p, _ptr(ev), n_ev.value, ctypes.byref(n_ev))
        _check(rc)
        return ev[:n_ev.value], fm.tobytes(), lit.value, mat.value, stats.as_dict()

    def block_sums_file(self, path, size, h, seed):
        s = np.frombuffer(bytes(seed), np.uint8).copy()
# ... 292 lines not shown
```

Measured before the change: 5198.

## Prebuild chain key-set images in a side kernel and load them in walks

Adds a kernel that builds the cuckoo key-set hash image for each file ahead of time, after first checking a few lead windows to see whether the file is likely to match. The chain walk and its helpers then copy this prebuilt image into LDS instead of rebuilding the key set in every block. When imaging is on, chunk indexing and the window copy move to the phase stream so they can overlap the image kernel. The cost is an extra kernel launch, device memory for one image per file, and a cross-stream event dependency.

After: 5199 (median of 2 runs). No clear change (+0.0%).

```diff
diff --git a/include/rsync_hip_debug.h b/include/rsync_hip_debug.h
--- a/include/rsync_hip_debug.h
+++ b/include/rsync_hip_debug.h
@@ -44,6 +44,11 @@
 int rsh_debug_untokens_selftest(rsh_ctx* ctx, const uint8_t* tokens, int64_t tokens_len, int64_t pos, int32_t T,
                                 int64_t count, uint8_t* out, int64_t span, int64_t* n_desc, int64_t* lo, int64_t* hi);
 
+int rsh_debug_chain_kset_image(rsh_ctx* ctx, const void* d_weak, int64_t C, void* image_out, int32_t* full_out);
+
+int rsh_debug_chain_kset_check(const void* image, const int32_t* weak, int64_t C, int32_t full, uint32_t key,
+                               int32_t buckets_out[2]);
+
 #ifdef __cplusplus
 }
 #endif
diff --git a/java-rsync_amd/csrc/batch.cpp b/java-rsync_amd/csrc/batch.cpp
--- a/java-rsync_amd/csrc/batch.cpp
+++ b/java-rsync_amd/csrc/batch.cpp
@@ -59,6 +59,7 @@
     bool chain_on = false;
     bool two_phase = false;
     bool map_on = false;
+    bool kset_on = false;
     int32_t chain_events = 0;
     K1Set whole, a, b;
     std::vector<int64_t> lead_at;
@@ -164,6 +165,11 @@
     RSH_HTRY(S->h_chain_out.ensure(nf * sizeof(ChainOut)));
     RSH_HTRY(S->h_chain_ev.ensure(nf * (size_t)chain_events * sizeof(rsh_event)));
     RSH_HTRY(S->h_early.ensure(4096));
+    kset_on = opt(OPT_CHAIN_KSET_IMAGE) != 0;
+    if (kset_on) {
+        RSH_HTRY(S->kset_img.ensure(nf * (size_t)CHAIN_CK_IMAGE_BYTES));
+        RSH_HTRY(S->h_ksetents.ensure(nf * sizeof(KsetImageEnt)));
+    }
     map_off.assign(nf + 1, 0);
     map_on = two_phase && opt(OPT_CHAIN_HELPERS) != 0;
     for (size_t f = 0; map_on && f < nf; ++f) {
@@ -237,6 +243,7 @@
     int32_t NF() const { return L.NF; }
     ChainOut* chain_out() const { return S->h_chain_out.as<ChainOut>(); }
     rsh_event* chain_ev(int32_t f) const { return S->h_chain_ev.as<rsh_event>() + (int64_t)f * L.chain_events; }
+    uint32_t* kset_image(int32_t f) const { return S->kset_img.as<uint32_t>() + (int64_t)f * (CHAIN_CK_IMAGE_BYTES / 4); }
 
     int lay_out(const std::vector<int32_t>& which);
     void prepare_files();
@@ -328,6 +335,16 @@
 int Scan::enqueue_prep() {
     ScanFile* F = S->h_files.as<ScanFile>();
     RSH_BHIP(hipEventRecord(c->ev_in, st));
+    if (L.chain_on && L.kset_on) {
+        KsetImageEnt* ie = S->h_ksetents.as<KsetImageEnt>();
+        const bool all = opt(OPT_CHAIN_KSET_IMAGE) == 2;
+        for (int32_t f = 0; f < NF(); ++f) {
+            const FileScan& fs = files[(size_t)f];
+            ie[f] = KsetImageEnt{fs.d_weak, fs.C, all ? 0 : (int32_t)std::min<int64_t>(kKsetLeadWindows, fs.nf), fs.d_src, fs.n,
+                                 (uint32_t)fs.B, 0u, kset_image(f)};
+        }
+        RSH_BHIP(launch_chain_kset_images(ie, (uint32_t)NF(), st));
+    }
     CopyEnt* wc = S->h_ccopies.as<CopyEnt>();
     int64_t max_w0 = 0;
     for (int32_t f = 0; f < NF(); ++f) {
@@ -336,7 +353,8 @@
         wc[f] = CopyEnt{fs.d_src, S->h_win0.as<uint8_t>() + fs.off_w0, w0};
         max_w0 = std::max(max_w0, w0);
     }
-    RSH_BHIP(launch_copy_many(wc, (uint32_t)NF(), max_w0, st));
+    const bool beside = L.chain_on && L.kset_on;
+    if (!beside) RSH_BHIP(launch_copy_many(wc, (uint32_t)NF(), max_w0, st));
     if (L.nlead_all > 0 && !L.chain_on) {
         auto* ents = reinterpret_cast<GatherEnt*>(S->h_lead.as<uint8_t>() + L.lead_ents_at);
         for (int32_t f = 0; f < NF(); ++f)
@@ -361,13 +379,21 @@
         return RSH_OK;
     }
     if (!S->ev_fk) RSH_BHIP(hipEventCreateWithFlags(&S->ev_fk, hipEventDisableTiming));
-    RSH_BHIP(hipMemsetAsync(S->kslots.p, 0, (size_t)L.tns * 8 + (size_t)L.tw, st));
+    const hipStream_t xs = beside ? c->phase : st;
+    if (beside) RSH_BHIP(hipStreamWaitEvent(xs, c->ev_in, 0));
+    RSH_BHIP(hipMemsetAsync(S->kslots.p, 0, (size_t)L.tns * 8 + (size_t)L.tw, xs));
     ChunkIndexEnt* ke = S->h_kents.as<ChunkIndexEnt>();
     for (int32_t f = 0; f < NF(); ++f) {
         const FileScan& fs = files[(size_t)f];
         ke[f] = ChunkIndexEnt{table_ent(S->kslots, fs), kslots_dup(S, L.tns) + fs.off_tw};
     }
-    RSH_BHIP(launch_chunk_index(ke, (uint32_t)NF(), (int32_t)L.maxC, st, bg));
+    RSH_BHIP(launch_chunk_index(ke, (uint32_t)NF(), (int32_t)L.maxC, xs, bg));
+    if (beside) {
+        RSH_BHIP(launch_copy_many(wc, (uint32_t)NF(), max_w0, xs));
+        if (!S->ev_ix) RSH_BHIP(hipEventCreateWithFlags(&S->ev_ix, hipEventDisableTiming));
+        RSH_BHIP(hipEventRecord(S->ev_ix, xs));
+        RSH_BHIP(hipStreamWaitEvent(st, S->ev_ix, 0));
+    }
     return RSH_OK;
 }
 
@@ -531,9 +557,9 @@
                           L.two_phase ? S->file_abort + f : nullptr, chain_ev(f), L.chain_events,
                           seed_word(seed), co + f,
                           mw > 0 ? S->chain_map.as<unsigned long long>() + L.map_off[(size_t)f] : nullptr, hend,
-                          kslots_dup(S, L.tns) + fs.off_tw};
+                          kslots_dup(S, L.tns) + fs.off_tw, L.kset_on && fs.C > 0 ? kset_image(f) : nullptr};
         if (chh) chh[f] = ChainHelp{(int32_t)((hend + CHAIN_MAP_SEG - 1) / CHAIN_MAP_SEG), 0, 1, 0, 0, 0, 0, 0, INT64_MAX, 0, 0, 0,
-                                    kChainHelpTiles};
+                                    kChainHelpTiles, 0};
     }
     const int64_t helpers_opt = opt(OPT_CHAIN_HELPERS);
     n_help = !L.map_on ? 0u
@@ -698,23 +724,29 @@
                     co[f].tiles, co[f].md5c_valid, (long long)co[f].clear_to, co[f].spec_full, co[f].t_total / 100.0);
     fprintf(stderr, "[rsh-batch]   file %d: walk %.1f us = tiles %.1f (table checks %.1f; %d of %d tiles from the hit map,"
             " the first at tile %d) + events %.1f (buckets %.1f; %d digests: %.1f) + key set %.1f + steps (1)/(1') %.1f +"
-            " event drains %.1f + other\n", fmax, x.t_total / 100.0,
+            " event drains %.1f + other; key set: %s\n", fmax, x.t_total / 100.0,
             x.t_tiles / 100.0, x.t_check / 100.0, x.mapped, x.tiles, x.first_mapped, x.t_event / 100.0,
-            x.t_evb / 100.0, x.digests, x.t_digest / 100.0, x.t_kset / 100.0, x.t_chain / 100.0, x.t_drain / 100.0);
+            x.t_evb / 100.0, x.digests, x.t_digest / 100.0, x.t_kset / 100.0, x.t_chain / 100.0, x.t_drain / 100.0,
+            x.kset == 2 ? "loaded" : x.kset == 1 ? "built" : "none");
+    int32_t wl = 0, wb = 0;
+    for (int32_t f = 0; f < NF(); ++f) wl += co[f].kset == 2, wb += co[f].kset == 1;
+    fprintf(stderr, "[rsh-batch]   key sets of the walks: %d loaded, %d built\n", wl, wb);
     if (!S->chain_help.p || !L.two_phase) return;
     std::vector<ChainHelp> hh((size_t)NF());
     if (hipMemcpy(hh.data(), S->chain_help.p, (size_t)NF() * sizeof(ChainHelp), hipMemcpyDeviceToHost) != hipSuccess) return;
-    int64_t segs = 0, joins = 0, files_helped = 0;
+    int64_t segs = 0, joins = 0, loads = 0, files_helped = 0;
     for (const ChainHelp& q : hh) {
         segs += q.mapped;
         joins += q.joins;
-        files_helped += q.joins > 0;
+        loads += q.loads;
+        files_helped += q.joins + q.loads > 0;
     }
     const ChainHelp& q = hh[(size_t)fmax];
-    fprintf(stderr, "[rsh-batch]   hit map: %lld segments mapped over %lld files (%lld key sets built); file %d: %d "
-            "segments (%d whole), %d key sets (%.1f us each), claims %d of %d, first whole segment %.1f us after "
-            "the walk's start\n", (long long)segs, (long long)files_helped, (long long)joins, fmax, q.mapped,
-            q.whole, q.joins, q.joins ? q.t_kset / 100.0 / q.joins : 0.0, q.claim, q.nseg,
+    fprintf(stderr, "[rsh-batch]   hit map: %lld segments mapped over %lld files (%lld key sets built, %lld loaded); file "
+            "%d: %d segments (%d whole), %d key sets built and %d loaded (%.1f us each), claims %d of %d, first whole "
+            "segment %.1f us after the walk's start\n", (long long)segs, (long long)files_helped, (long long)joins,
+            (long long)loads, fmax, q.mapped, q.whole, q.joins, q.loads,
+            q.joins + q.loads ? q.t_kset / 100.0 / (q.joins + q.loads) : 0.0, q.claim, q.nseg,
             q.t_first == INT64_MAX ? -1.0 : (q.t_first - q.t_start) / 100.0);
 }
 
@@ -899,7 +931,7 @@
         ok(pb->ensure(64 << 10));
     for (PinnedBuf* pb : {&S->h_fgw, &S->h_iv, &S->h_tiles, &S->h_segs, &S->h_ptiles}) ok(pb->ensure(512 << 10));
     for (DevBuf* db : {&S->fc_dev, &S->partials, &S->dslots, &S->d_probe}) ok(db->ensure(64 << 10));
-    for (hipEvent_t* ev : {&S->ev_fk, &S->ev_fa, &S->spec_k1.ev, &S->ev_sync, &S->gen_k1.ev})
+    for (hipEvent_t* ev : {&S->ev_fk, &S->ev_ix, &S->ev_fa, &S->spec_k1.ev, &S->ev_sync, &S->gen_k1.ev})
         if (!*ev) ok(hipEventCreateWithFlags(ev, hipEventDisableTiming));
     if (!S->ev_wa) ok(hipEventCreate(&S->ev_wa));
     ok(S->gen_k1.ensure(L.whole.plans.size(), L.whole.ngroups, L.whole.lanes.size()));
diff --git a/java-rsync_amd/csrc/batch.h b/java-rsync_amd/csrc/batch.h
--- a/java-rsync_amd/csrc/batch.h
+++ b/java-rsync_amd/csrc/batch.h
@@ -10,6 +10,7 @@
 
 #include <immintrin.h>
 
+#include "chain_kset.h"
 #include "ctx.h"
 #include "host_md5.h"
 #include "options.h"
@@ -115,10 +116,13 @@
     int64_t file_abort_cap = 0;
     DevBuf kslots;
     PinnedBuf h_kents, h_chain, h_chain_out, h_chain_ev;
+    DevBuf kset_img;
+    PinnedBuf h_ksetents;
     DevBuf chain_help, chain_map;
     PinnedBuf h_chain_help;
     std::vector<std::unique_ptr<char[]>> fiber_stacks;
     hipEvent_t ev_fk = nullptr;
+    hipEvent_t ev_ix = nullptr;
     hipEvent_t ev_sync = nullptr;
     hipEvent_t ev_ch0 = nullptr, ev_ch1 = nullptr;
     hipEvent_t ev_fa = nullptr, ev_wa = nullptr;
@@ -136,10 +140,11 @@
     }
     ~BatchState() {
         if (file_abort) (void)hipFree(file_abort);
-        for (hipEvent_t e : {ev_fk, ev_ch0, ev_ch1, ev_fa, ev_wa, ev_sync})
+        for (hipEvent_t e : {ev_fk, ev_ix, ev_ch0, ev_ch1, ev_fa, ev_wa, ev_sync})
             if (e) (void)hipEventDestroy(e);
         kslots.release();
-        for (PinnedBuf* b : {&h_kents, &h_chain, &h_chain_out, &h_chain_ev, &h_chain_help}) b->release();
+        kset_img.release();
+        for (PinnedBuf* b : {&h_kents, &h_chain, &h_chain_out, &h_chain_ev, &h_chain_help, &h_ksetents}) b->release();
         chain_help.release();
         chain_map.release();
         for (DevBuf* b : {&d_probe, &fc_dev, &slots, &dslots, &src_weak, &src_strong, &flags, &haw, &partials, &bucket, &first})
@@ -160,6 +165,7 @@
 
 constexpr int32_t kMaxLive = 256;
 constexpr int kDeferRounds = 2;
+constexpr int32_t kKsetLeadWindows = 8;
 constexpr int32_t kChainHelpTiles = 1;
 constexpr int kSpinUs = 200;
 constexpr int32_t kMaxWorkers = 32;
diff --git a/java-rsync_amd/csrc/capi.cpp b/java-rsync_amd/csrc/capi.cpp
--- a/java-rsync_amd/csrc/capi.cpp
+++ b/java-rsync_amd/csrc/capi.cpp
@@ -11,6 +11,7 @@
 #include <thread>
 #include <vector>
 
+#include "chain_kset.h"
 #include "device.h"
 #include "host_md5.h"
 #include "resolver.h"
@@ -576,6 +577,43 @@
     return RSH_OK;
 }
 
+int rsh_debug_chain_kset_image(rsh_ctx* ctx, const void* d_weak, int64_t C, void* image_out, int32_t* full_out) {
+    if (!ctx || !image_out || !full_out || C < 0 || C > 0x7FFFFFFF || (C > 0 && !d_weak)) return RSH_E_INVAL;
+    RSH_HIP(hipSetDevice(ctx->device));
+    constexpr size_t kGuard = 256, kImage = (size_t)rsh::CHAIN_CK_IMAGE_BYTES;
+    uint8_t* d = nullptr;
+    rsh::KsetImageEnt* ent = nullptr;
+    std::vector<uint8_t> h(kImage + 2 * kGuard);
+    hipError_t e = hipMalloc(reinterpret_cast<void**>(&d), h.size());
+    if (e == hipSuccess) e = hipHostMalloc(reinterpret_cast<void**>(&ent), sizeof(*ent), hipHostMallocDefault);
+    if (e == hipSuccess) e = hipMemsetAsync(d, 0xA5, h.size(), ctx->stream);
+    if (e == hipSuccess) {
+        *ent = rsh::KsetImageEnt{static_cast<const int32_t*>(d_weak), (int32_t)C, 0, nullptr, 0, 0u, 0u,
+                                 reinterpret_cast<uint32_t*>(d + kGuard)};
+        e = rsh::launch_chain_kset_images(ent, 1, ctx->stream);
+    }
+    if (e == hipSuccess) e = hipMemcpyAsync(h.data(), d, h.size(), hipMemcpyDeviceToHost, ctx->stream);
+    if (e == hipSuccess) e = hipStreamSynchronize(ctx->stream);
+    if (d) (void)hipFree(d);
+    if (ent) (void)hipHostFree(ent);
+    RSH_HIP(e);
+    for (size_t i = 0; i < kGuard; ++i)
+        if (h[i] != 0xA5 || h[kGuard + kImage + i] != 0xA5) return RSH_E_DEVICE;
+    memcpy(image_out, h.data() + kGuard, 4 * (size_t)rsh::CHAIN_CK_WORDS);
+    memcpy(full_out, h.data() + kGuard + 4 * (size_t)rsh::CHAIN_CK_WORDS, 4);
+    return RSH_OK;
+}
+
+int rsh_debug_chain_kset_check(const void* image, const int32_t* weak, int64_t C, int32_t full, uint32_t key,
+                               int32_t buckets_out[2]) {
+    if (C < 0 || (C > 0 && !weak)) return RSH_E_INVAL;
+    if (buckets_out) {
+        buckets_out[0] = (int32_t)rsh::chain_ck_h1(key);
+        buckets_out[1] = (int32_t)rsh::chain_ck_h2(key);
+    }
+    return image ? rsh::chain_kset_check(static_cast<const uint32_t*>(image), weak, C, full) : 0;
+}
+
 int rsh_fill_splitmix_device(rsh_ctx* ctx, void* d_out, int64_t n, uint64_t key, int64_t byte_offset) {
     if (!ctx || (n > 0 && !d_out) || n < 0 || byte_offset < 0) return RSH_E_INVAL;
     RSH_HIP(hipSetDevice(ctx->device));
diff --git a/java-rsync_amd/csrc/chain_kset.h b/java-rsync_amd/csrc/chain_kset.h
--- /dev/null
+++ b/java-rsync_amd/csrc/chain_kset.h
@@ -0,0 +1,44 @@
+#pragma once
+#include <stdint.h>
+
+#include <algorithm>
+#include <vector>
+
+#if defined(__HIPCC__)
+#define RSH_CK_HD __host__ __device__ constexpr
+#else
+#define RSH_CK_HD constexpr
+#endif
+
+namespace rsh {
+
+constexpr int CHAIN_CK_BUCKETS = 8192;
+constexpr int64_t CHAIN_CK_WORDS = 4 * (int64_t)CHAIN_CK_BUCKETS;
+constexpr int64_t CHAIN_CK_IMAGE_BYTES = 4 * CHAIN_CK_WORDS + 16;
+constexpr int CHAIN_CK_INSERT_BOUND = 128;
+RSH_CK_HD uint32_t chain_ck_h1(uint32_t k) { return (((k ^ (k >> 15)) & 0xFFFFFFu) * 0x9E3779u) >> 19; }
+RSH_CK_HD uint32_t chain_ck_h2(uint32_t k) {
+    return CHAIN_CK_BUCKETS + ((((k ^ (k >> 8)) & 0xFFFFFFu) * 0x85EBCBu) >> 19);
+}
+RSH_CK_HD uint32_t chain_ck_empty(uint32_t i) { return (i == chain_ck_h1(0u) || i == chain_ck_h2(0u)) ? 1u : 0u; }
+static_assert(chain_ck_h1(1u) != chain_ck_h1(0u) && chain_ck_h2(1u) != chain_ck_h2(0u), "empty values");
+
+inline int chain_kset_check(const uint32_t* image, const int32_t* weak, int64_t C, int32_t full) {
+    std::vector<uint32_t> keys(weak, weak + (C > 0 ? C : 0));
+    std::sort(keys.begin(), keys.end());
+    for (uint32_t b = 0; b < 2u * CHAIN_CK_BUCKETS; ++b)
+        for (int j = 0; j < 2; ++j) {
+            const uint32_t v = image[2 * b + j];
+            if (v == chain_ck_empty(b)) continue;
+            if ((b < (uint32_t)CHAIN_CK_BUCKETS ? chain_ck_h1(v) : chain_ck_h2(v)) != b) return 1;
+            if (!std::binary_search(keys.begin(), keys.end(), v)) return 3;
+        }
+    if (full != 0) return 0;
+    for (const uint32_t k : keys) {
+        const uint32_t a = chain_ck_h1(k), c = chain_ck_h2(k);
+        if (image[2 * a] != k && image[2 * a + 1] != k && image[2 * c] != k && image[2 * c + 1] != k) return 2;
+    }
+    return 0;
+}
+
+}
diff --git a/java-rsync_amd/csrc/device.h b/java-rsync_amd/csrc/device.h
--- a/java-rsync_amd/csrc/device.h
+++ b/java-rsync_amd/csrc/device.h
@@ -287,7 +287,8 @@
     int32_t aborted;
     int32_t mapped, first_mapped;
     int64_t clear_to;
-    int32_t why, pad2;
+    int32_t why;
+    int32_t kset;
     uint32_t elo, ehi;
     int32_t fin, pad3;
 };
@@ -307,6 +308,7 @@
     int32_t whole;
     int32_t nhelp;
     int32_t help_tiles;
+    int32_t loads;
 };
 constexpr int CHAIN_THREADS = 512;
 constexpr int CHAIN_PPT = 32;
@@ -336,6 +338,7 @@
     unsigned long long* hmap;
     int64_t hend;
     const uint8_t* dup;
+    const uint32_t* kimg;
 };
 hipError_t launch_k1_clock(const uint8_t* d_data, int64_t n, uint32_t B, uint32_t dl, uint32_t seed_word,
                            int32_t* d_weak, uint8_t* d_strong, unsigned long long* d_clk, hipStream_t s);
@@ -348,6 +351,17 @@
 hipError_t launch_chunk_index(const ChunkIndexEnt* ents, uint32_t nfiles, int32_t max_keys, hipStream_t s,
                               bool bg = false);
 
+struct KsetImageEnt {
+    const int32_t* keys;
+    int32_t nkeys;
+    int32_t lead;
+    const uint8_t* data;
+    int64_t n;
+    uint32_t B, pad;
+    uint32_t* image;
+};
+hipError_t launch_chain_kset_images(const KsetImageEnt* ents, uint32_t nfiles, hipStream_t s);
+
 hipError_t launch_fill_splitmix(uint8_t* d_out, int64_t n, uint64_t key, int64_t byte_offset, hipStream_t s);
 
 }
diff --git a/java-rsync_amd/csrc/device_chain.hip b/java-rsync_amd/csrc/device_chain.hip
--- a/java-rsync_amd/csrc/device_chain.hip
+++ b/java-rsync_amd/csrc/device_chain.hip
@@ -2,6 +2,7 @@
 
 #include "device.h"
 #include "device_common.h"
+#include "chain_kset.h"
 #include "device_roll.h"
 #include "md5_core.h"
 #include "options.h"
@@ -29,17 +30,6 @@
     }
 }
 
-constexpr int CHAIN_CK_BUCKETS = 8192;
-__host__ __device__ constexpr uint32_t chain_ck_h1(uint32_t k) {
-    return (((k ^ (k >> 15)) & 0xFFFFFFu) * 0x9E3779u) >> 19;
-}
-__host__ __device__ constexpr uint32_t chain_ck_h2(uint32_t k) {
-    return CHAIN_CK_BUCKETS + ((((k ^ (k >> 8)) & 0xFFFFFFu) * 0x85EBCBu) >> 19);
-}
-__host__ __device__ constexpr uint32_t chain_ck_empty(uint32_t i) {
-    return (i == chain_ck_h1(0u) || i == chain_ck_h2(0u)) ? 1u : 0u;
-}
-static_assert(chain_ck_h1(1u) != chain_ck_h1(0u) && chain_ck_h2(1u) != chain_ck_h2(0u), "empty values");
 struct ChainKeySet {
     uint2* b;
     int32_t* full;
@@ -47,7 +37,7 @@
 __device__ __forceinline__ void chain_ck_insert(const ChainKeySet& ks, uint32_t k) {
     uint32_t cur = k;
     int w = 0;
-    for (int it = 0; it < 128; ++it) {
+    for (int it = 0; it < CHAIN_CK_INSERT_BOUND; ++it) {
         const uint32_t bi = w == 0 ? chain_ck_h1(cur) : chain_ck_h2(cur), e = chain_ck_empty(bi);
         uint32_t* slot = reinterpret_cast<uint32_t*>(&ks.b[bi]);
 #pragma unroll
@@ -220,6 +210,24 @@
     if (t == 0) *ks.full = 0;
     __syncthreads();
     for (int64_t c = t; c < C; c += CHAIN_THREADS) chain_ck_insert(ks, (uint32_t)weak[c]);
+    __syncthreads();
+}
+__device__ __forceinline__ bool chain_kset_has_image(const uint32_t* __restrict__ img) {
+    return img != nullptr && img[CHAIN_CK_WORDS + 1] != 0u;
+}
+__device__ __forceinline__ void chain_kset_load(const ChainKeySet& ks, const uint32_t* __restrict__ img) {
+    static_assert(CHAIN_CK_WORDS / 4 % (8 * CHAIN_THREADS) == 0, "whole rounds of eight loads per thread");
+    const int t = threadIdx.x;
+    const uint4* src = reinterpret_cast<const uint4*>(img);
+    uint4* dst = reinterpret_cast<uint4*>(ks.b);
+    for (int i0 = t; i0 < (int)(CHAIN_CK_WORDS / 4); i0 += 8 * CHAIN_THREADS) {
+        uint4 v[8];
+#pragma unroll
+        for (int j = 0; j < 8; ++j) v[j] = src[i0 + j * CHAIN_THREADS];
+#pragma unroll
+        for (int j = 0; j < 8; ++j) dst[i0 + j * CHAIN_THREADS] = v[j];
+    }
+    if (t == 0) *ks.full = (int32_t)img[CHAIN_CK_WORDS];
     __syncthreads();
 }
 
@@ -499,6 +507,7 @@
     int64_t lit, mat, chain_matches, events, flushes;
     int32_t tiles, digests, mapped, first_mapped;
     int64_t t_tiles, t_check, t_event, t_digest, t_kset, t_chain, t_drain, t_evb;
+    int32_t kset;
 };
 __device__ __forceinline__ void chain_write_out(const ChainFile& F, int phase, int abort_gen, int64_t s, int64_t m,
                                                 int32_t pref, int32_t nev, int32_t status, int32_t why,
@@ -529,6 +538,7 @@
     out->elo = elo;
     out->ehi = ehi;
     out->first_mapped = N.first_mapped;
+    if (N.kset != 0) out->kset = N.kset;
     const bool stop_spec = phase == 0 && F.abort && (status == CHAIN_DONE || dead);
     out->aborted = stop_spec;
     if (stop_spec) *(volatile int*)F.abort = abort_gen;
@@ -601,10 +611,12 @@
             cur = f;
             const int64_t tb = chain_clock(timed);
             F = files[f];
-            chain_kset_build(L.kset, F.table_weak, F.C);
+            const bool img = chain_kset_has_image(F.kimg);
+            if (img) chain_kset_load(L.kset, F.kimg);
+            else chain_kset_build(L.kset, F.table_weak, F.C);
             if (t == 0) {
                 atomicAdd((unsigned long long*)&h->t_kset, (unsigned long long)(chain_clock(timed) - tb));
-                atomicAdd(&h->joins, 1);
+                atomicAdd(img ? &h->loads : &h->joins, 1);
             }
             if (*L.kset.full) {
                 if (t == 0) atomicMax(&h->claim, h->nseg);
@@ -650,7 +662,7 @@
     __shared__ __attribute__((aligned(16))) uint8_t s_win[CHAIN_WIN_BUF + 128];
     __shared__ int32_t s_any;
     __shared__ int32_t s_seg[CHAIN_SEGS][4];
-    __shared__ uint2 s_ck[2 * CHAIN_CK_BUCKETS];
+    __shared__ __attribute__((aligned(16))) uint2 s_ck[2 * CHAIN_CK_BUCKETS];
     __shared__ int32_t s_ck_full;
     __shared__ __attribute__((aligned(16))) uint8_t s_dig[16];
     __shared__ rsh_event s_ev[CHAIN_EV_LDS];
@@ -682,9 +694,12 @@
     if (s % B == 0 && nflags >= na)
         kset_built = chain_first_unset_flag<false>(F.flags, s / B, nflags, &s_zero) < nflags;
     const int64_t tks0 = chain_clock(timed);
-    if (kset_built) chain_kset_build(kset, F.table_weak, C);
+    const bool kset_img = kset_built && chain_kset_has_image(F.kimg);
+    if (kset_img) chain_kset_load(kset, F.kimg);
+    else if (kset_built) chain_kset_build(kset, F.table_weak, C);
     ChainTally N{out->literal, out->matched, out->chain_matches, out->events, out->flushes, out->tiles, out->digests,
-                 out->mapped, out->first_mapped, 0, 0, 0, 0, chain_clock(timed) - tks0, 0, 0, 0};
+                 out->mapped, out->first_mapped, 0, 0, 0, 0, chain_clock(timed) - tks0, 0, 0, 0,
+                 kset_img ? 2 : kset_built ? 1 : 0};
     int32_t pref = out->pref;
     int32_t nev = out->n_ev, status = CHAIN_STOP;
     int32_t poisoned = 0, dead = 0;
@@ -1155,6 +1170,39 @@
     hipLaunchKernelGGL(chunk_index_kernel, dim3(gx, nfiles), dim3(256), 0, s, ents, nfiles);
     return hipGetLastError();
 }
+
+__global__ __launch_bounds__(CHAIN_THREADS) void chain_kset_image_kernel(const KsetImageEnt* __restrict__ ents) {
+    __shared__ int32_t sh[2 * CHAIN_THREADS / 64];
+    __shared__ __attribute__((aligned(16))) uint2 s_ck[2 * CHAIN_CK_BUCKETS];
+    __shared__ int32_t s_ck_full;
+    const KsetImageEnt e = ents[blockIdx.x];
+    const int t = threadIdx.x;
+    bool need = e.lead == 0;
+    for (int32_t k = 0; !need && k < e.lead; ++k) {
+        const int64_t o = (int64_t)k * e.B, len = e.n - o < (int64_t)e.B ? e.n - o : (int64_t)e.B;
+        int32_t w2[2] = {0, 0};
+        range_sums(e.data, e.n, o, o + len, o, w2[0], w2[1]);
+        block_reduce<2>(w2, sh);
+        const uint32_t S1 = (uint32_t)w2[0], S2 = (uint32_t)len * S1 - (uint32_t)w2[1];
+        need = ((S1 & 0xFFFFu) | (S2 << 16)) != (uint32_t)e.keys[k];
+    }
+    uint4* const hdr = reinterpret_cast<uint4*>(e.image + CHAIN_CK_WORDS);
+    if (!need) {
+        if (t == 0) *hdr = make_uint4(0u, 0u, 0u, 0u);
+        return;
+    }
+    chain_kset_build(ChainKeySet{s_ck, &s_ck_full}, e.keys, e.nkeys);
+    const uint4* src = reinterpret_cast<const uint4*>(s_ck);
+    uint4* img = reinterpret_cast<uint4*>(e.image);
+    for (int i = t; i < (int)(CHAIN_CK_WORDS / 4); i += CHAIN_THREADS) img[i] = src[i];
+    if (t == 0) *hdr = make_uint4((uint32_t)s_ck_full, 1u, 0u, 0u);
+}
+hipError_t launch_chain_kset_images(const KsetImageEnt* ents, uint32_t nfiles, hipStream_t s) {
+    if (nfiles == 0) return hipSuccess;
+    hipLaunchKernelGGL(chain_kset_image_kernel, dim3(nfiles), dim3(CHAIN_THREADS), 0, s, ents);
+    return hipGetLastError();
+}
+
 __global__ void warm_chain_kernel() {}
 constexpr int kWarmScratchWords = 160;
 __global__ __launch_bounds__(CHAIN_THREADS) void warm_scratch_kernel(int32_t sel, int32_t* out) {
diff --git a/java-rsync_amd/csrc/options.h b/java-rsync_amd/csrc/options.h
--- a/java-rsync_amd/csrc/options.h
+++ b/java-rsync_amd/csrc/options.h
@@ -30,6 +30,7 @@
     OPT_TOKENS_PIECE,
     OPT_SUMS_PIECE,
     OPT_TOKENS_RUNS,
+    OPT_CHAIN_KSET_IMAGE,
     OPT_COUNT
 };
 
@@ -47,6 +48,7 @@
     {"chain_map_bytes", 1LL << 30}, {"time_gen", 1},    {"batch_warm", 128},
     {"fault_inject", 0},        {"tokens_span", 256LL << 10}, {"tokens_piece", 8LL << 20},
     {"sums_piece", 32LL << 20}, {"tokens_runs", 64LL << 10},
+    {"chain_kset_image", 1},
 };
 
 inline const OptInfo* opt_info() { return kOpts; }
diff --git a/java-rsync_amd/rsync_hip.py b/java-rsync_amd/rsync_hip.py
--- a/java-rsync_amd/rsync_hip.py
+++ b/java-rsync_amd/rsync_hip.py
@@ -158,7 +158,7 @@
 DEBUG_EXPORTS = ["rsh_debug_set_option", "rsh_debug_get_option", "rsh_debug_reset_options", "rsh_debug_k1_clock",
                  "rsh_debug_streams_busy", "rsh_debug_kernel_ms", "rsh_debug_multi_selftest", "rsh_debug_generation",
                  "rsh_debug_tokens_selftest", "rsh_debug_sums_selftest", "rsh_debug_tokens_scan_selftest",
-                 "rsh_debug_untokens_selftest"]
+                 "rsh_debug_untokens_selftest", "rsh_debug_chain_kset_image", "rsh_debug_chain_kset_check"]
 
 _LIB = None
 
@@ -278,8 +278,12 @@
                                             ctypes.POINTER(I64), ctypes.POINTER(I32)], ctypes.c_int),
         "rsh_debug_untokens_selftest": ([P, P, I64, I64, I32, I64, P, I64, ctypes.POINTER(I64), ctypes.POINTER(I64),
                                          ctypes.POINTER(I64)], ctypes.c_int),
+        "rsh_debug_chain_kset_image": ([P, P, I64, P, ctypes.POINTER(I32)], ctypes.c_int),
+        "rsh_debug_chain_kset_check": ([P, P, I64, I32, ctypes.c_uint32, P], ctypes.c_int),
     }
     for name, (args, res) in sig.items():
+        if os.environ.get("RSH_LIB") and name.startswith("rsh_debug_chain_kset") and not hasattr(L, name):
+            continue
         fn = getattr(L, name)
         fn.argtypes = args
         fn.restype = res
@@ -460,6 +464,23 @@
     return nd.value
 
 
+CHAIN_KSET_SLOTS = 4 * 8192
+
+
+def chain_kset_buckets(key):
+    b = (ctypes.c_int32 * 2)()
+    _check(lib().rsh_debug_chain_kset_check(None, None, 0, 0, int(key) & 0xFFFFFFFF, ctypes.cast(b, ctypes.c_void_p)))
+    return int(b[0]), int(b[1])
+
+
+def chain_kset_check(image, weak, full):
+    image = np.ascontiguousarray(image, np.uint32)
+    weak = np.ascontiguousarray(weak, np.int32)
+    assert image.size == CHAIN_KSET_SLOTS
+    return lib().rsh_debug_chain_kset_check(_addr(image), _addr(weak) if weak.size else None, weak.size, int(full), 0,
+                                            None)
+
+
 def set_option(name, value):
     _check(lib().rsh_debug_set_option(name.encode(), int(value)))
 
@@ -535,6 +556,15 @@
         m = ctypes.c_int32(-1)
         _check(lib().rsh_debug_streams_busy(self._p, ctypes.byref(m)))
         return m.value
+
+    def chain_kset_image(self, d_weak, count, guard=64):
+        buf = np.full(4 * CHAIN_KSET_SLOTS + 2 * guard, 0xA5, np.uint8)
+        full = ctypes.c_int32(-1)
+        _check(lib().rsh_debug_chain_kset_image(self._p, _addr(d_weak), count,
+                                                ctypes.c_void_p(buf.ctypes.data + guard), ctypes.byref(full)))
+        if not ((buf[:guard] == 0xA5).all() and (buf[buf.size - guard:] == 0xA5).all()):
+            raise AssertionError("rsh_debug_chain_kset_image wrote outside its image")
+        return buf[guard:buf.size - guard].view(np.uint32).copy(), full.value
 
     def sync(self):
         _check(lib().rsh_ctx_sync(self._p))
```
